# MrOlm/inStrain

Hardware: AMD Instinct MI355X
Metric: Gbp profiled/s (higher is better)
Workload: dtype u32

## Files before the change

include/instrain_amd.h:

```cpp
#ifndef INSTRAIN_AMD_H
#define INSTRAIN_AMD_H

#include <stdint.h>

#ifdef __cplusplus
extern "C" {
#endif

#define ISX_OK 0
#define ISX_ERR_ARG (-1)
#define ISX_ERR_HIP (-2)
#define ISX_ERR_CAPACITY (-3)
#define ISX_ERR_MM_RANGE (-4)
#define ISX_ERR_IO (-5)
#define ISX_ERR_STATE (-6)

#define ISX_ABI_VERSION 5


typedef struct isx_ctx isx_ctx;
typedef struct isx_batch isx_batch;
typedef struct isx_bam isx_bam;
struct isx_bam_params_s;
struct isx_bam_info_s;

typedef struct {
    uint32_t gpos;
    uint16_t mm;
    uint8_t base;
    uint8_t flags;
} isx_obs;

typedef struct {
    int32_t min_cov;
    int32_t min_snp;
    double min_freq;
    int32_t rarefied_coverage;
    int32_t n_mm_bins;
    int32_t enable_linkage;
    int32_t linkage_mode;
    int32_t window;
    uint64_t seed;
    int32_t layout;
    int32_t reserved;
} isx_params;

#define ISX_LAYOUT_WIDE_RECORDS 1
#define ISX_LAYOUT_NO_SHORT_RECORDS 2
#define ISX_LAYOUT_NO_PACKED_COUNTERS 4
#define ISX_LAYOUT_SEG64_RECORDS 8

#define ISX_LAYOUT_MM_ENTRIES 16

#define ISX_LAYOUT_MM_DELTA_RECORDS 32

#define ISX_LAYOUT_NO_STRIPES 64

typedef struct {
    uint32_t gpos;
    uint16_t mm;
    uint16_t flags;
    uint32_t cnt[4];
    float clon;
    float clon_rarefied;
} isx_entry;

typedef struct {
    uint32_t gpos;
    uint16_t mm;
    uint8_t con_base, var_base;
    uint8_t allele_count;
    uint8_t cls;
    uint8_t cryptic;
    uint8_t ref_base;
    uint32_t cnt[4];
} isx_snv;

typedef struct {
    uint32_t gpos_a, gpos_b;
    uint16_t mm;
    uint8_t allele_A, allele_a, allele_B, allele_b;
    uint16_t pad;
    uint32_t total, countAB, countAb, countaB, countab;
    uint32_t pad2;
    double r2, d_prime;
    double r2_normalized, d_prime_normalized;
} isx_ld;

typedef struct {
    int64_t n_entries;
    int64_t n_snv;
    int64_t n_sites;
    int64_t n_allele_obs;
    int64_t n_increments;
    int64_t n_edges;
    int64_t n_ld;
} isx_sizes;

typedef struct {
    float pileup_ms;
    float sites_ms;
    float allele_ms;
    float group_ms;
    float incr_ms;
    float ld_ms;
    float total_ms;
    int32_t pileup_blocks, pileup_threads, pileup_lds_bytes, pileup_window;
    float mfma_ms;
    int32_t dense_tiles;
    int64_t dense_macs;
    int64_t dense_bytes;
    int32_t record_bytes;
    int32_t pad;
} isx_timings;

const char *isx_last_error(void);
int isx_abi_version(void);

int isx_ctx_create(int device_id, isx_ctx **out);
void isx_ctx_destroy(isx_ctx *ctx);
int isx_ctx_reserve_cus(isx_ctx *ctx, int cus_per_xcd);

int isx_set_null_model(isx_ctx *ctx, const int32_t *lut, int64_t n, int32_t fallback);

int isx_batch_create(isx_ctx *ctx, const isx_params *params, int64_t n_pos, const uint8_t *ref,
                     int32_t n_splits, const int64_t *split_bounds, int64_t n_obs,
                     const isx_obs *obs, const uint32_t *pair, isx_batch **out);
void isx_batch_destroy(isx_batch *b);

int isx_batch_run(isx_batch *b);

int isx_batch_launch(isx_batch *b);
int isx_batch_wait(isx_batch *b);
int isx_batch_sizes(const isx_batch *b, isx_sizes *out);
int isx_batch_timings(const isx_batch *b, isx_timings *out);

int isx_batch_fetch_entries(isx_batch *b, isx_entry *out);
int isx_batch_fetch_dense(isx_batch *b, uint32_t *counts , float *clon ,
                          float *clon_rarefied );
// ... 159 lines not shown
    const isx_sat *lev_sat;
    int64_t n_lev, n_lev_clon, n_lev_rare, n_lev_sat;
    int32_t lev_mask_bytes, lev_cov_bytes, lev_window, n_lev_windows, lev_min_cov, pad_lev;
    uint64_t rows_checksum;
} isx_pipe_result;

int isx_levels_expand(const isx_pipe_result *r, int32_t host_threads, uint32_t *gpos, uint32_t *mm_cov, float *clon, float *clon_rarefied);

int isx_pipe_create(isx_ctx *ctx, const isx_params *params, const isx_pipe_params *pp, isx_pipe **out);
void isx_pipe_destroy(isx_pipe *p);
int isx_pipe_submit(isx_pipe *p, int64_t n_pos, const uint8_t *ref, int32_t n_splits, const int64_t *split_bounds,
                    int64_t n_obs, const isx_obs *obs, const uint32_t *pair, int64_t *ticket);
int isx_pipe_submit_bam(isx_pipe *p, isx_bam *bam, const struct isx_bam_params_s *bp, const int32_t *refs, int32_t n_refs,
                        const uint8_t *ref, int32_t n_splits, const int64_t *split_bounds, struct isx_bam_info_s *info,
                        int64_t *ticket);
int isx_pipe_collect(isx_pipe *p, int64_t ticket, isx_pipe_result *out);
int isx_pipe_release(isx_pipe *p, int64_t ticket);
int isx_pipe_fetch_entries(isx_pipe *p, int64_t ticket, isx_entry *out);
int isx_pipe_fetch_entries_shrunk(isx_pipe *p, int64_t ticket, uint32_t *gpos, uint32_t *mm_cov, float *clon, float *clon_rarefied);


#define ISX_SEG_BASES 150
#define ISX_SEG_WORDS 15
#define ISX_SEG_SKIP_WORD 0x24924924u
#define ISX_DREC_WORDS 8
#define ISX_DREC_EXC 6
#define ISX_DREC_EXC_FULL 3
#define ISX_DREC_DUAL 0x80000000u
#define ISX_DREC_NO_EXC 0x3FFFFFFFu

typedef struct {
    int64_t n_seg;
    const uint32_t *gpos;
    const uint8_t *len;
    const uint8_t *mm;
    const uint32_t *pair;
    const uint32_t *bases;
} isx_segs;

int isx_batch_create_reads(isx_ctx *ctx, const isx_params *params, int64_t n_pos, const uint8_t *ref, int32_t n_splits,
                           const int64_t *split_bounds, const isx_segs *segs, isx_batch **out);
int isx_pipe_submit_reads(isx_pipe *p, int64_t n_pos, const uint8_t *ref, int32_t n_splits, const int64_t *split_bounds,
                          const isx_segs *segs, int64_t *ticket);

typedef struct isx_wire isx_wire;
int isx_pipe_stage_reads(isx_pipe *p, int64_t n_pos, const uint8_t *ref, int32_t n_splits, const int64_t *split_bounds,
                         const isx_segs *segs, isx_wire **out);
int isx_pipe_submit_wire(isx_pipe *p, const isx_wire *wire, int64_t *ticket);
int64_t isx_wire_bytes(const isx_wire *wire);
void isx_wire_free(isx_wire *wire);
int isx_wire_keep_reference(isx_pipe *p, isx_wire *wire);

#define ISX_PLANE_WORDS 8
typedef struct {
    int64_t n_seg;
    const uint32_t *gpos;
    const uint8_t *len;
    const uint32_t *pair;
    const uint64_t *planes;
    const uint8_t *mm;
} isx_read_planes;

typedef struct {
    const uint8_t *plane2;
    const uint8_t *nplane;
    uint64_t key;
} isx_ref_planes;

int isx_pack_ref_planes(const uint8_t *ref, int64_t n_pos, int32_t host_threads, uint8_t *plane2, uint8_t *nplane, int32_t *has_n);
int isx_planes_from_segs(const isx_segs *segs, int32_t host_threads, uint64_t *planes);
int isx_pack_read_planes(int64_t n_reads, const int64_t *ref_start, const int64_t *clip_lo, const int64_t *clip_hi,
                         const uint32_t *cigar, const int64_t *cigar_off, const char *seq, const uint8_t *qual, const int64_t *seq_off,
                         const uint32_t *pair, int32_t min_base_quality, int64_t cap_seg, uint32_t *seg_gpos,
                         uint8_t *seg_len, uint32_t *seg_pair, uint64_t *seg_planes, int64_t *n_seg);
int isx_pipe_submit_planes(isx_pipe *p, int64_t n_pos, const isx_ref_planes *ref, int32_t n_splits, const int64_t *split_bounds,
                           const isx_read_planes *reads, int64_t *ticket);
int isx_pipe_stage_planes(isx_pipe *p, int64_t n_pos, const isx_ref_planes *ref, int32_t n_splits, const int64_t *split_bounds,
                          const isx_read_planes *reads, isx_wire **out);
int isx_pipe_set_reference_budget(isx_pipe *p, int64_t mib);
int isx_host_register(const void *ptr, int64_t bytes);
int isx_host_unregister(const void *ptr);
int isx_encode_planes(const isx_read_planes *reads, const isx_ref_planes *ref, int64_t n_pos, int32_t host_threads, int32_t slack_groups,
                      int64_t cap_rec, int64_t ring_records, uint32_t *rec, uint32_t *gbase, int64_t *n_rec, int64_t *need_slack);
int isx_encode_planes_mm(const isx_read_planes *reads, const isx_ref_planes *ref, int64_t n_pos, int32_t n_mm_bins, int32_t host_threads, int32_t slack_groups,
                         int64_t cap_rec, int64_t ring_records, uint32_t *rec, uint32_t *gbase, int64_t *n_rec, int64_t *need_slack);

int isx_count_read_segs(int64_t n_reads, const uint32_t *cigar, const int64_t *cigar_off, const int64_t *ref_start,
                        const int64_t *clip_lo, const int64_t *clip_hi, int64_t *n_seg);
int isx_pack_reads(int64_t n_reads, const int64_t *ref_start, const int64_t *clip_lo, const int64_t *clip_hi,
                   const uint32_t *cigar, const int64_t *cigar_off, const char *seq, const uint8_t *qual, const int64_t *seq_off,
                   const uint8_t *mm, const uint32_t *pair, int32_t min_base_quality, int64_t cap_seg, uint32_t *seg_gpos,
                   uint8_t *seg_len, uint8_t *seg_mm, uint32_t *seg_pair, uint32_t *seg_bases, int64_t *n_seg);

int isx_encode_segs(const isx_segs *segs, int64_t n_pos, int32_t n_mm_bins, int32_t host_threads, int64_t cap_rec, uint32_t *rec,
                    uint32_t *gbase, uint32_t *pair_out, int64_t *n_rec);
int64_t isx_seg_records_needed(const uint32_t *gpos, int64_t n_seg, int32_t host_threads);
int isx_encode_segs_ring(const isx_segs *segs, int64_t n_pos, int32_t n_mm_bins, int32_t host_threads, int64_t cap_rec, int64_t ring_records,
                         uint32_t *rec, uint32_t *gbase, uint32_t *pair_out, int64_t *n_rec);

int isx_encode_delta(const isx_segs *segs, const uint8_t *ref, int64_t n_pos, int32_t n_mm_bins, int32_t host_threads, int32_t slack_groups,
                     int64_t cap_rec, int64_t ring_records, uint32_t *rec, uint32_t *gbase, uint32_t *pair_out, int64_t *n_rec, int64_t *need_slack);
int64_t isx_delta_records_needed(const uint32_t *gpos, int64_t n_seg, int32_t host_threads, int32_t slack_groups);

int isx_encode_obs(const isx_obs *obs, const uint32_t *pair, int64_t n_obs, int64_t n_pos, int32_t record_bytes,
                   int32_t host_threads, double slack, int64_t cap_rec, void *rec, uint32_t *gbase, uint32_t *pair_out,
                   int64_t *n_rec, int32_t *passes);
int isx_encode_obs_ring(const isx_obs *obs, const uint32_t *pair, int64_t n_obs, int64_t n_pos, int32_t record_bytes,
                        int32_t host_threads, double slack, int64_t cap_rec, int64_t ring_records, void *rec,
                        uint32_t *gbase, uint32_t *pair_out, int64_t *n_rec, int32_t *passes);

typedef struct {
    int64_t in_off;
    int32_t in_len;
    int32_t out_len;
    int64_t out_off;
} isx_bgzf_block;
int isx_bgzf_index(const uint8_t *image, int64_t n_bytes, int64_t cap_blocks, isx_bgzf_block *blocks, int64_t *n_blocks, int64_t *out_bytes);
int isx_bgzf_inflate_device(isx_ctx *ctx, const uint8_t *image, int64_t n_bytes, const isx_bgzf_block *blocks, int64_t n_blocks,
                            uint8_t *out, int64_t out_bytes, float *kernel_ms);
int isx_bgzf_inflate_host(const uint8_t *image, int64_t n_bytes, const isx_bgzf_block *blocks, int64_t n_blocks, uint8_t *out, int64_t out_bytes);
int isx_bgzf_inflate_fast(const uint8_t *image, int64_t n_bytes, const isx_bgzf_block *blocks, int64_t n_blocks, uint8_t *out, int64_t out_bytes);

typedef struct isx_bam_params_s {
    double min_read_ani;
    int32_t min_mapq;
    double max_insert_relative;
    int32_t min_insert;
    int32_t min_base_quality;
    int32_t skip_mm;
    int32_t window_length;
    int32_t pairing_filter;
} isx_bam_params;

typedef struct isx_bam_info_s {
    int32_t n_refs;
    int32_t n_splits;
    int64_t n_reads;
    int64_t n_pos;
    int64_t n_obs;
    int64_t n_pairs;
    int64_t unfiltered_pairs, filtered_pairs;
    int64_t filtered_bases;
    double median_insert;
    int32_t max_mm;
    int32_t pad;
    int64_t unfiltered_reads, unfiltered_singletons, filtered_singletons;
    int64_t n_segs;
} isx_bam_info;

int isx_bam_open(const char *path, isx_bam **out);
void isx_bam_close(isx_bam *bam);
void isx_bam_close_wait(isx_bam *bam);
int isx_bam_set_threads(isx_bam *bam, int32_t threads);
int isx_bam_ref(const isx_bam *bam, int32_t i, const char **name, int64_t *length, int64_t *flat_offset);
int isx_bam_set_priority_reads(isx_bam *bam, int64_t n, const char *names, const int64_t *offs);
int isx_bam_scan(isx_bam *bam, isx_bam_info *info );
int isx_bam_scan_part(isx_bam *bam, int32_t part, int32_t n_parts, isx_bam_info *info );
int isx_bam_set_wanted_refs(isx_bam *bam, const int32_t *refs, int32_t n);
int isx_bam_insert_sizes(isx_bam *bam, int64_t *out, int64_t cap, int64_t *n);
int isx_bam_filter(isx_bam *bam, const isx_bam_params *p, double median_insert , isx_bam_info *info);
int isx_bam_pair_keys(isx_bam *bam, uint64_t *h1, uint64_t *h2, int32_t *tid, int64_t *info4, int64_t cap, int64_t *n);
int isx_bam_set_cross_names(isx_bam *bam, int64_t n, const int64_t *entry, const int64_t *occurrences, const int64_t *info4);
int isx_bam_filter_insert_sizes(isx_bam *bam, int64_t *out, int64_t cap, int64_t *n);
int isx_bam_set_r2m(isx_bam *bam, int32_t ref, int64_t n, const char *names, const int64_t *offs, const int32_t *mm );
int isx_bam_set_mm_cap(isx_bam *bam, int32_t cap);
int isx_bam_mm_levels(const isx_bam *bam, int32_t *levels, int32_t cap, int32_t *n);
// ... 20 lines not shown
```

instrain_amd/_lib.py:

```python
import ctypes as C
import os

import numpy as np

_HERE = os.path.dirname(os.path.abspath(__file__))
LIB_PATH = os.path.join(_HERE, "libinstrain_amd.so")
if os.environ.get("ISX_LIB"):
    LIB_PATH = os.path.abspath(os.environ["ISX_LIB"])

BGZF_BLOCK_DT = np.dtype([("in_off", np.int64), ("in_len", np.int32), ("out_len", np.int32), ("out_off", np.int64)])
OBS_DT = np.dtype([("gpos", "<u4"), ("mm", "<u2"), ("base", "u1"), ("flags", "u1")])
ENTRY_DT = np.dtype([("gpos", "<u4"), ("mm", "<u2"), ("flags", "<u2"), ("cnt", "<u4", (4,)), ("clon", "<f4"),
                     ("clon_rarefied", "<f4")])
SNV_DT = np.dtype([("gpos", "<u4"), ("mm", "<u2"), ("con_base", "u1"), ("var_base", "u1"),
                   ("allele_count", "u1"), ("cls", "u1"), ("cryptic", "u1"), ("ref_base", "u1"),
                   ("cnt", "<u4", (4,))])
LD_DT = np.dtype([("gpos_a", "<u4"), ("gpos_b", "<u4"), ("mm", "<u2"), ("allele_A", "u1"), ("allele_a", "u1"),
                  ("allele_B", "u1"), ("allele_b", "u1"), ("pad", "<u2"), ("total", "<u4"), ("countAB", "<u4"),
                  ("countAb", "<u4"), ("countaB", "<u4"), ("countab", "<u4"), ("pad2", "<u4"),
                  ("r2", "<f8"), ("d_prime", "<f8"), ("r2_normalized", "<f8"), ("d_prime_normalized", "<f8")])
AO_DT = np.dtype([("pair", "<u4"), ("gpos", "<u4"), ("order", "<u4"), ("mm", "<u2"), ("base", "u1"), ("pad", "u1")])
assert AO_DT.itemsize == 16
assert OBS_DT.itemsize == 8 and ENTRY_DT.itemsize == 32 and SNV_DT.itemsize == 28 and LD_DT.itemsize == 72


class Params(C.Structure):
    _fields_ = [("min_cov", C.c_int32), ("min_snp", C.c_int32), ("min_freq", C.c_double),
                ("rarefied_coverage", C.c_int32), ("n_mm_bins", C.c_int32), ("enable_linkage", C.c_int32),
                ("linkage_mode", C.c_int32), ("window", C.c_int32), ("seed", C.c_uint64), ("layout", C.c_int32),
                ("reserved", C.c_int32)]


LAYOUT_WIDE_RECORDS, LAYOUT_NO_SHORT_RECORDS, LAYOUT_NO_PACKED_COUNTERS, LAYOUT_SEG64_RECORDS = 1, 2, 4, 8


class PipeParams(C.Structure):
    _fields_ = [("max_pos", C.c_int64), ("max_obs", C.c_int64), ("max_splits", C.c_int32), ("depth", C.c_int32),
                ("host_threads", C.c_int32), ("pin_threads", C.c_int32), ("jump_slack", C.c_double),
                ("want_counts", C.c_int32), ("ring_kib", C.c_int32), ("stage_async", C.c_int32), ("lean_output", C.c_int32),
                ("max_segs", C.c_int64)]


SEG_BASES, SEG_WORDS, SEG_SKIP_WORD = 150, 15, 0x24924924


class Segs(C.Structure):
    _fields_ = [("n_seg", C.c_int64), ("gpos", C.c_void_p), ("len", C.c_void_p), ("mm", C.c_void_p), ("pair", C.c_void_p),
                ("bases", C.c_void_p)]


PLANE_WORDS = 8
LAYOUT_MM_ENTRIES = 16
LAYOUT_MM_DELTA_RECORDS = 32
ABI_VERSION = 5


class ReadPlanes(C.Structure):
    _fields_ = [("n_seg", C.c_int64), ("gpos", C.c_void_p), ("len", C.c_void_p), ("pair", C.c_void_p), ("planes", C.c_void_p), ("mm", C.c_void_p)]


class RefPlanes(C.Structure):
    _fields_ = [("plane2", C.c_void_p), ("nplane", C.c_void_p), ("key", C.c_uint64)]


RARE_DT = np.dtype([("gpos", "<u4"), ("clon_rarefied", "<f4")])
CLON_DT = np.dtype([("gpos", "<u4"), ("clon", "<f4")])
SAT_DT = np.dtype([("gpos", "<u4"), ("coverage", "<u4")])


class Sizes(C.Structure):
    _fields_ = [(n, C.c_int64) for n in ("n_entries", "n_snv", "n_sites", "n_allele_obs", "n_increments",
                                         "n_edges", "n_ld")]


class Timings(C.Structure):
    _fields_ = [(n, C.c_float) for n in ("pileup_ms", "sites_ms", "allele_ms", "group_ms", "incr_ms", "ld_ms",
                                         "total_ms")] + \
               [(n, C.c_int32) for n in ("pileup_blocks", "pileup_threads", "pileup_lds_bytes", "pileup_window")] + \
               [("mfma_ms", C.c_float), ("dense_tiles", C.c_int32), ("dense_macs", C.c_int64), ("dense_bytes", C.c_int64),
                ("record_bytes", C.c_int32), ("pad", C.c_int32)]


class PipeResult(C.Structure):
    _fields_ = [("ticket", C.c_int64), ("n_pos", C.c_int64), ("n_obs", C.c_int64), ("sizes", Sizes),
                ("coverage16", C.c_void_p), ("clon", C.c_void_p), ("rare", C.c_void_p), ("n_rare", C.c_int64),
                ("n_saturated", C.c_int64), ("counts", C.c_void_p), ("clon_rarefied", C.c_void_p), ("snv", C.c_void_p),
                ("batch", C.c_void_p),
                ("encode_ms", C.c_float), ("h2d_ms", C.c_float), ("kernel_ms", C.c_float), ("d2h_ms", C.c_float),
                ("collect_wait_ms", C.c_float), ("record_bytes", C.c_int32), ("encode_passes", C.c_int32),
                ("h2d_bytes", C.c_int64), ("d2h_bytes", C.c_int64), ("ld", C.c_void_p),
                ("coverage8", C.c_void_p), ("clon_sparse", C.c_void_p), ("n_clon", C.c_int64), ("saturated", C.c_void_p),
                ("coverage4", C.c_void_p), ("cov_rows", C.c_void_p), ("cov_row_window", C.c_void_p), ("n_cov_rows", C.c_int64),
                ("cov_window", C.c_int32), ("pad_cov", C.c_int32),
                ("lev_mask", C.c_void_p), ("lev_cov", C.c_void_p), ("lev_win_off", C.c_void_p), ("lev_clon", C.c_void_p), ("lev_rare", C.c_void_p),
                ("lev_sat", C.c_void_p), ("n_lev", C.c_int64), ("n_lev_clon", C.c_int64), ("n_lev_rare", C.c_int64), ("n_lev_sat", C.c_int64),
                ("lev_mask_bytes", C.c_int32), ("lev_cov_bytes", C.c_int32), ("lev_window", C.c_int32), ("n_lev_windows", C.c_int32),
                ("lev_min_cov", C.c_int32), ("pad_lev", C.c_int32), ("rows_checksum", C.c_uint64)]


class BamParams(C.Structure):
    _fields_ = [("min_read_ani", C.c_double), ("min_mapq", C.c_int32), ("max_insert_relative", C.c_double),
                ("min_insert", C.c_int32), ("min_base_quality", C.c_int32), ("skip_mm", C.c_int32),
                ("window_length", C.c_int32), ("pairing_filter", C.c_int32)]


PAIRING_FILTERS = {"paired_only": 0, "non_discordant": 1, "all_reads": 2}


class BamInfo(C.Structure):
    _fields_ = [("n_refs", C.c_int32), ("n_splits", C.c_int32), ("n_reads", C.c_int64), ("n_pos", C.c_int64),
                ("n_obs", C.c_int64), ("n_pairs", C.c_int64), ("unfiltered_pairs", C.c_int64),
                ("filtered_pairs", C.c_int64), ("filtered_bases", C.c_int64), ("median_insert", C.c_double),
                ("max_mm", C.c_int32), ("pad", C.c_int32), ("unfiltered_reads", C.c_int64),
                ("unfiltered_singletons", C.c_int64), ("filtered_singletons", C.c_int64), ("n_segs", C.c_int64)]


SCAFFOLD_LEVEL_DT = np.dtype([("nonzero", "<i8"), ("sum_cov", "<u8"), ("sumsq_cov", "<u8"), ("median_cov", "<f8"),
                              ("counted", "<i8"), ("sum_clon", "<f8"), ("median_clon", "<f8"),
                              ("counted_rarefied", "<i8"), ("sum_clon_rarefied", "<f8"),
                              ("median_clon_rarefied", "<f8"), ("mm", "<i4"), ("present", "<i4")])
assert SCAFFOLD_LEVEL_DT.itemsize == 88
GENOME_LEVEL_DT = np.dtype([("n", "<i8"), ("sum_cov", "<u8"), ("sumsq_cov", "<u8"), ("median_cov", "<f8"), ("mm", "<i4"), ("pad", "<i4")])
assert GENOME_LEVEL_DT.itemsize == 40


COMPARE_LEVEL_DT = np.dtype([("both", "<i8"), ("either", "<i8"), ("mm", "<i4"), ("present_a", "<i4"),
                             ("present_b", "<i4"), ("pad", "<i4"), ("consensus_snps", "<i8"), ("population_snps", "<i8")])
assert COMPARE_LEVEL_DT.itemsize == 48
COMPARE_SNP_DT = np.dtype([("gpos", "<u4"), ("mm", "<u2"), ("consensus_snp", "u1"), ("population_snp", "u1"),
                           ("has_a", "u1"), ("has_b", "u1"), ("con_a", "u1"), ("ref_a", "u1"), ("var_a", "u1"),
                           ("con_b", "u1"), ("ref_b", "u1"), ("var_b", "u1"), ("cnt_a", "<u4", (4,)), ("cnt_b", "<u4", (4,))])
assert COMPARE_SNP_DT.itemsize == 48


GENE_DT = np.dtype([("start", "<i8"), ("end", "<i8"), ("seq_off", "<i8"), ("strand", "<i4"), ("pad", "<i4")])
GENE_COV_DT = np.dtype([("sum_cov", "<u8"), ("nonzero", "<u4"), ("counted", "<u4"), ("sum_clon", "<f8")])
GENE_SNV_COUNT_DT = np.dtype([(n, "<u4") for n in ("divergent", "sns", "sns_n", "sns_s", "snv", "snv_n", "snv_s")])
GENE_MUTATION_DT = np.dtype([("gene", "<i4"), ("k", "<i4"), ("type", "u1"), ("aa_old", "u1"), ("aa_new", "u1"), ("n_genes", "u1"),
                             ("pad", "<u4")])
assert GENE_DT.itemsize == 32 and GENE_COV_DT.itemsize == 24 and GENE_SNV_COUNT_DT.itemsize == 28 and GENE_MUTATION_DT.itemsize == 16
GENE_LEVEL_PRESENT, GENE_COV_ANY, GENE_CLON_ANY = 1, 2, 4


ERR_CAPACITY = -3


class IsxError(RuntimeError):
    def __init__(self, code, msg):
        super().__init__("libinstrain_amd error %d: %s" % (code, msg))
        self.code = code


SYMBOLS = ["isx_last_error", "isx_abi_version", "isx_ctx_create", "isx_ctx_destroy", "isx_ctx_reserve_cus", "isx_set_null_model",
           "isx_batch_create", "isx_batch_create_reads", "isx_batch_destroy", "isx_batch_run", "isx_batch_launch", "isx_batch_wait", "isx_batch_sizes", "isx_batch_timings",
           "isx_batch_fetch_entries", "isx_batch_fetch_dense", "isx_batch_fetch_snv", "isx_batch_fetch_ld", "isx_batch_fetch_allele_obs",
           "isx_batch_summarize", "isx_batch_summarize_genomes", "isx_compare_coverage", "isx_compare_scaffolds", "isx_compare_fetch_snps",
           "isx_genes_create", "isx_genes_destroy", "isx_genes_sites", "isx_batch_profile_genes", "isx_genes_profile_snvs",
           "isx_pipe_create", "isx_pipe_destroy", "isx_pipe_submit", "isx_pipe_submit_reads", "isx_pipe_stage_reads", "isx_pipe_submit_wire", "isx_wire_bytes", "isx_wire_free", "isx_wire_keep_reference", "isx_pipe_submit_bam", "isx_encode_segs", "isx_encode_segs_ring", "isx_seg_records_needed", "isx_encode_delta", "isx_delta_records_needed", "isx_count_read_segs", "isx_pack_reads", "isx_pipe_collect", "isx_pipe_release", "isx_pipe_fetch_entries", "isx_pipe_fetch_entries_shrunk", "isx_levels_expand", "isx_encode_obs", "isx_encode_obs_ring",
           "isx_pack_ref_planes", "isx_planes_from_segs", "isx_pack_read_planes", "isx_pipe_submit_planes", "isx_pipe_stage_planes", "isx_encode_planes", "isx_encode_planes_mm", "isx_pipe_set_reference_budget", "isx_host_register", "isx_host_unregister",
           "isx_bgzf_index", "isx_bgzf_inflate_device", "isx_bgzf_inflate_host", "isx_bgzf_inflate_fast",
           "isx_bam_open", "isx_bam_close", "isx_bam_close_wait", "isx_bam_set_threads", "isx_bam_ref", "isx_bam_set_priority_reads", "isx_bam_scan", "isx_bam_scan_part",
           "isx_bam_insert_sizes", "isx_bam_set_wanted_refs", "isx_bam_pair_keys", "isx_bam_set_cross_names", "isx_bam_filter_insert_sizes", "isx_bam_filter", "isx_bam_set_r2m", "isx_bam_r2m", "isx_bam_drop_names", "isx_bam_batch_pair_names", "isx_bam_set_mm_cap", "isx_bam_mm_levels", "isx_bam_set_mm_levels", "isx_bam_ref_counts",
           "isx_bam_expand_refs", "isx_bam_segment_refs", "isx_bam_copy_segs", "isx_bam_copy_read_planes", "isx_bam_expand_region", "isx_bam_expand", "isx_bam_copy", "isx_bam_view"]

_lib = None


def load():
    global _lib
    if _lib is not None:
        return _lib
    if not os.path.exists(LIB_PATH):
        raise IsxError(-2, "%s not built: run `python -c 'import __graft_entry__ as g; g.build()'` "
                           "(hipcc --offload-arch=gfx950)" % LIB_PATH)
    lib = C.CDLL(LIB_PATH)
    vp, i32, i64 = C.c_void_p, C.c_int32, C.c_int64
    lib.isx_last_error.restype = C.c_char_p
    lib.isx_abi_version.restype = C.c_int
    if lib.isx_abi_version() != ABI_VERSION:
        raise IsxError(-6, "%s has ABI version %d, this package binds version %d: rebuild it (python -c 'import __graft_entry__ as g; g.build()')"
                       % (LIB_PATH, lib.isx_abi_version(), ABI_VERSION))
    lib.isx_ctx_create.argtypes = [C.c_int, C.POINTER(vp)]
    lib.isx_ctx_destroy.argtypes = [vp]
    lib.isx_ctx_reserve_cus.argtypes = [vp, C.c_int]
    lib.isx_bgzf_index.argtypes = [vp, i64, i64, vp, C.POINTER(i64), C.POINTER(i64)]
    lib.isx_bgzf_inflate_device.argtypes = [vp, vp, i64, vp, i64, vp, i64, C.POINTER(C.c_float)]
    lib.isx_bgzf_inflate_host.argtypes = [vp, i64, vp, i64, vp, i64]
    lib.isx_bgzf_inflate_fast.argtypes = [vp, i64, vp, i64, vp, i64]
    lib.isx_ctx_destroy.restype = None
    lib.isx_set_null_model.argtypes = [vp, vp, i64, i32]
    lib.isx_batch_create.argtypes = [vp, C.POINTER(Params), i64, vp, i32, vp, i64, vp, vp, C.POINTER(vp)]
    lib.isx_batch_create_reads.argtypes = [vp, C.POINTER(Params), i64, vp, i32, vp, C.POINTER(Segs), C.POINTER(vp)]
    lib.isx_pipe_submit_reads.argtypes = [vp, i64, vp, i32, vp, C.POINTER(Segs), C.POINTER(i64)]
    lib.isx_pipe_stage_reads.argtypes = [vp, i64, vp, i32, vp, C.POINTER(Segs), C.POINTER(vp)]
    lib.isx_pipe_submit_wire.argtypes = [vp, vp, C.POINTER(i64)]
    lib.isx_wire_bytes.argtypes = [vp]
    lib.isx_wire_bytes.restype = i64
    lib.isx_wire_free.argtypes = [vp]
    lib.isx_wire_keep_reference.argtypes = [vp, vp]
    lib.isx_wire_free.restype = None
    lib.isx_encode_segs.argtypes = [C.POINTER(Segs), i64, i32, i32, i64, vp, vp, vp, C.POINTER(i64)]
    lib.isx_encode_segs_ring.argtypes = [C.POINTER(Segs), i64, i32, i32, i64, i64, vp, vp, vp, C.POINTER(i64)]
    lib.isx_encode_delta.argtypes = [C.POINTER(Segs), vp, i64, i32, i32, i32, i64, i64, vp, vp, vp, C.POINTER(i64), C.POINTER(i64)]
    lib.isx_delta_records_needed.argtypes = [vp, i64, i32, i32]
    lib.isx_delta_records_needed.restype = i64
    lib.isx_seg_records_needed.argtypes = [vp, i64, i32]
    lib.isx_seg_records_needed.restype = i64
    lib.isx_count_read_segs.argtypes = [i64, vp, vp, vp, vp, vp, C.POINTER(i64)]
    lib.isx_pack_reads.argtypes = [i64, vp, vp, vp, vp, vp, vp, vp, vp, vp, vp, i32, i64, vp, vp, vp, vp, vp, C.POINTER(i64)]
    lib.isx_batch_destroy.argtypes = [vp]
    lib.isx_batch_destroy.restype = None
    lib.isx_batch_run.argtypes = [vp]
    lib.isx_batch_launch.argtypes = [vp]
    lib.isx_batch_wait.argtypes = [vp]
    lib.isx_batch_sizes.argtypes = [vp, C.POINTER(Sizes)]
    lib.isx_batch_timings.argtypes = [vp, C.POINTER(Timings)]
    for f in ("isx_batch_fetch_entries", "isx_batch_fetch_snv", "isx_batch_fetch_ld", "isx_batch_fetch_allele_obs"):
        getattr(lib, f).argtypes = [vp, vp]
    lib.isx_batch_fetch_dense.argtypes = [vp, vp, vp, vp]
    lib.isx_batch_summarize.argtypes = [vp, i32, vp, vp, C.POINTER(C.c_float)]
    lib.isx_batch_summarize_genomes.argtypes = [vp, i32, vp, i32, vp, i32, vp, C.POINTER(C.c_float)]
    lib.isx_compare_coverage.argtypes = [vp, vp, i32, vp, i32, vp, C.POINTER(C.c_float)]
    lib.isx_compare_scaffolds.argtypes = [vp, vp, i32, vp, i32, C.c_double, vp, C.POINTER(i64), C.POINTER(C.c_float)]
    lib.isx_compare_fetch_snps.argtypes = [vp, vp]
    lib.isx_genes_create.argtypes = [vp, i64, vp, C.c_char_p, i64, C.POINTER(vp)]
    lib.isx_genes_destroy.argtypes = [vp]
    lib.isx_genes_destroy.restype = None
    lib.isx_genes_sites.argtypes = [vp, vp, C.POINTER(C.c_float)]
    lib.isx_batch_profile_genes.argtypes = [vp, vp, i32, vp, vp, vp, vp, vp, C.POINTER(C.c_float)]
    lib.isx_genes_profile_snvs.argtypes = [vp, i32, vp, vp, vp, i64, vp, i32, vp, vp, C.POINTER(C.c_float)]
    lib.isx_pipe_create.argtypes = [vp, C.POINTER(Params), C.POINTER(PipeParams), C.POINTER(vp)]
    lib.isx_pipe_destroy.argtypes = [vp]
    lib.isx_pipe_destroy.restype = None
    lib.isx_pipe_submit.argtypes = [vp, i64, vp, i32, vp, i64, vp, vp, C.POINTER(i64)]
    lib.isx_pipe_submit_bam.argtypes = [vp, vp, C.POINTER(BamParams), vp, i32, vp, i32, vp, C.POINTER(BamInfo), C.POINTER(i64)]
    lib.isx_pipe_collect.argtypes = [vp, i64, C.POINTER(PipeResult)]
    lib.isx_pipe_release.argtypes = [vp, i64]
    lib.isx_pipe_fetch_entries.argtypes = [vp, i64, vp]
    lib.isx_pipe_fetch_entries_shrunk.argtypes = [vp, i64, vp, vp, vp, vp]
    lib.isx_levels_expand.argtypes = [C.POINTER(PipeResult), i32, vp, vp, vp, vp]
    lib.isx_encode_obs.argtypes = [vp, vp, i64, i64, i32, i32, C.c_double, i64, vp, vp, vp, C.POINTER(i64), C.POINTER(i32)]
    lib.isx_encode_obs_ring.argtypes = [vp, vp, i64, i64, i32, i32, C.c_double, i64, i64, vp, vp, vp, C.POINTER(i64), C.POINTER(i32)]
    lib.isx_bam_open.argtypes = [C.c_char_p, C.POINTER(vp)]
    lib.isx_bam_close.argtypes = [vp]
    lib.isx_bam_close.restype = None
    lib.isx_bam_close_wait.argtypes = [vp]
    lib.isx_bam_close_wait.restype = None
    lib.isx_bam_expand.argtypes = [vp, C.POINTER(BamParams), C.POINTER(BamInfo)]
    lib.isx_bam_set_threads.argtypes = [vp, i32]
    lib.isx_bam_set_priority_reads.argtypes = [vp, i64, C.c_char_p, vp]
    lib.isx_bam_scan.argtypes = [vp, C.POINTER(BamInfo)]
    lib.isx_bam_scan_part.argtypes = [vp, i32, i32, C.POINTER(BamInfo)]
    lib.isx_bam_set_wanted_refs.argtypes = [vp, vp, i32]
    lib.isx_bam_insert_sizes.argtypes = [vp, vp, i64, C.POINTER(i64)]
    lib.isx_bam_filter_insert_sizes.argtypes = [vp, vp, i64, C.POINTER(i64)]
    lib.isx_bam_pair_keys.argtypes = [vp, vp, vp, vp, vp, i64, C.POINTER(i64)]
    lib.isx_bam_set_cross_names.argtypes = [vp, i64, vp, vp, vp]
    lib.isx_bam_filter.argtypes = [vp, C.POINTER(BamParams), C.c_double, C.POINTER(BamInfo)]
    lib.isx_bam_set_r2m.argtypes = [vp, i32, i64, C.c_char_p, vp, vp]
    lib.isx_bam_drop_names.argtypes = [vp]
    lib.isx_bam_r2m.argtypes = [vp, i32, C.POINTER(i64), C.POINTER(i64), vp, vp, vp]
    lib.isx_bam_batch_pair_names.argtypes = [vp, C.POINTER(i64), C.POINTER(i64), vp, vp]
    lib.isx_bam_set_mm_cap.argtypes = [vp, i32]
    lib.isx_bam_mm_levels.argtypes = [vp, vp, i32, vp]
    lib.isx_bam_set_mm_levels.argtypes = [vp, vp, i32]
    lib.isx_bam_ref_counts.argtypes = [vp, vp, vp]
    lib.isx_bam_expand_region.argtypes = [vp, C.POINTER(BamParams), i32, i64, i64, C.POINTER(BamInfo)]
    lib.isx_bam_expand_refs.argtypes = [vp, C.POINTER(BamParams), vp, i32, C.POINTER(BamInfo)]
    lib.isx_bam_segment_refs.argtypes = [vp, C.POINTER(BamParams), vp, i32, C.POINTER(BamInfo), C.POINTER(i64)]
    lib.isx_bam_copy_segs.argtypes = [vp, vp, vp, vp, vp, vp, vp, vp]
    lib.isx_bam_copy_read_planes.argtypes = [vp, vp]
    lib.isx_pack_ref_planes.argtypes = [vp, i64, i32, vp, vp, C.POINTER(i32)]
    lib.isx_planes_from_segs.argtypes = [C.POINTER(Segs), i32, vp]
    lib.isx_pack_read_planes.argtypes = [i64, vp, vp, vp, vp, vp, vp, vp, vp, vp, i32, i64, vp, vp, vp, vp, C.POINTER(i64)]
    lib.isx_pipe_submit_planes.argtypes = [vp, i64, C.POINTER(RefPlanes), i32, vp, C.POINTER(ReadPlanes), C.POINTER(i64)]
    lib.isx_pipe_set_reference_budget.argtypes = [vp, i64]
    lib.isx_host_register.argtypes = [vp, i64]
    lib.isx_host_unregister.argtypes = [vp]
    lib.isx_pipe_stage_planes.argtypes = [vp, i64, C.POINTER(RefPlanes), i32, vp, C.POINTER(ReadPlanes), C.POINTER(vp)]
    lib.isx_encode_planes.argtypes = [C.POINTER(ReadPlanes), C.POINTER(RefPlanes), i64, i32, i32, i64, i64, vp, vp, C.POINTER(i64), C.POINTER(i64)]
    lib.isx_encode_planes_mm.argtypes = [C.POINTER(ReadPlanes), C.POINTER(RefPlanes), i64, i32, i32, i32, i64, i64, vp, vp, C.POINTER(i64), C.POINTER(i64)]
    lib.isx_bam_ref.argtypes = [vp, i32, C.POINTER(C.c_char_p), C.POINTER(i64), C.POINTER(i64)]
    lib.isx_bam_copy.argtypes = [vp, vp, vp, vp, vp]
    lib.isx_bam_view.argtypes = [vp, C.POINTER(vp), C.POINTER(vp)]
    _lib = lib
    return lib


def check(rc):
    if rc != 0:
        raise IsxError(rc, load().isx_last_error().decode(errors="replace"))
```

instrain_amd/csrc/isx_pipe.hip:

```cpp
#include <atomic>
#include <algorithm>
#include <chrono>
#include <cmath>
#include <condition_variable>
#include <cstring>
#include <deque>
#include <mutex>
#include <memory>
#include <string>
#include <thread>
#include <vector>

#include "bam_front.h"
#include "isx_batch.h"
#include "obs_encode.h"
#include "seg_encode.h"
#include "isx_summary.h"
#include <unordered_map>

namespace {

constexpr size_t ALIGN = 256;
inline size_t up(size_t v, size_t a = ALIGN) { return (v + a - 1) / a * a; }

double now_ms()
{
    return std::chrono::duration<double, std::milli>(std::chrono::steady_clock::now().time_since_epoch()).count();
}

int host_block_alloc(void **p, size_t bytes, bool pinned)
{
    *p = nullptr;
    if (pinned) { HIP_TRY(isx_pin_malloc(p, std::max<size_t>(bytes, 1))); return ISX_OK; }
    if (posix_memalign(p, 4096, std::max<size_t>(bytes, 4096)) != 0) { *p = nullptr; isx_set_error("out of host memory"); return ISX_ERR_ARG; }
    return ISX_OK;
}

void host_block_free(void *p, bool pinned)
{
    if (!p) return;
    if (pinned) isx_pin_free(p); else free(p);
}

static const bool pipe_timing = getenv("ISX_PIPE_TIMING") != nullptr;
#define H2D(p, s) ((s).h2d ? (s).h2d : (p)->s_h2d)
struct Slot {
    isx_batch *b = nullptr;
    hipStream_t h2d = nullptr;
    uint8_t *h_in = nullptr, *d_in = nullptr;
    size_t in_bytes = 0;
    size_t off_bounds = 0, off_win = 0, off_ref = 0, off_gbase = 0, off_ridx = 0, off_rec = 0;
    size_t off_pairs = 0;
    isxenc::PairRun *h_runs = nullptr;
    bool runs_pinned = true;
    uint2 *d_runs = nullptr;
    size_t cap_runs = 0;
    hipEvent_t ev_ring[2] = {nullptr, nullptr};
    bool ring_busy[2] = {false, false};
    uint8_t *h_out = nullptr;
    uint8_t *h_small = nullptr;
    size_t small_bytes = 0;
    bool out_pinned = true;
    size_t out_bytes = 0, o_counts = 0, o_clon = 0, o_clonr = 0, o_snv = 0, o_cov16 = 0, o_rare = 0;
    bool rare_dense = false;
    bool cov8 = false, clon_sparse = false;
    bool cov4 = false;
    size_t cov_rows_off = 0;
    int cov_window = 0;
    std::vector<uint32_t> cov_row_win;
    std::vector<isx_sat> sat_rows;
    bool sat_complete = true;
    void *sort_temp = nullptr;
    size_t sort_temp_bytes = 0;
    std::vector<float> clonr_big;
    std::vector<isx_rare> rare_big;
    std::vector<uint32_t> cmin, cmax, dir_pmax, dir_smin;
    std::vector<uint8_t> cany;
    std::vector<uint2> win;
    size_t o_lmask = 0, o_lwin = 0, o_lcov = 0, o_lclon = 0, o_lrare = 0;
    size_t lcov_room = 0, lclon_room = 0, lrare_room = 0;
    std::vector<uint8_t> lcov_big;
    std::vector<isx_rare> lclon_big, lrare_big;
    std::vector<isx_snv> snv_big;
    std::vector<isx_ld> ld_rows;
    uint64_t rows_checksum = 0;
    hipEvent_t ev_h2d0 = nullptr, ev_h2d1 = nullptr, ev_pass = nullptr, ev_d2h0 = nullptr, ev_d2h1 = nullptr;
    hipEvent_t ev_h2da = nullptr, ev_h2db = nullptr;
    bool h2d_split = false;
    int64_t ticket = -1;
    BamBatch *dead_batch = nullptr;
    bool ref_has_n = false;
    int state = 0;
    int rc = 0;
    std::string err;
    float finish_wait_ms = 0.f;
    float encode_ms = 0.f;
    int encode_passes = 0;
    int64_t h2d_bytes = 0, d2h_bytes = 0;
    uint16_t *d_gpos16 = nullptr;
};

static uint64_t bytes_checksum(const void *p, size_t bytes, uint64_t seed)
{
    const uint8_t *b = static_cast<const uint8_t *>(p);
    uint64_t a[4] = {seed ^ 0x9E3779B97F4A7C15ull, seed + 0xC2B2AE3D27D4EB4Full, seed ^ 0x165667B19E3779F9ull, seed + 0x27D4EB2F165667C5ull};
    const size_t n8 = bytes / 8;
    size_t i = 0;
    for (; i + 4 <= n8; i += 4) {
        uint64_t w[4];
        memcpy(w, b + 8 * i, 32);
        for (int k = 0; k < 4; k++) a[k] = a[k] * 0x100000001B3ull + w[k];
    }
    uint64_t h = (uint64_t)bytes;
    for (; i < n8; i++) { uint64_t w; memcpy(&w, b + 8 * i, 8); h = h * 0x100000001B3ull + w; }
    for (size_t j = n8 * 8; j < bytes; j++) h = h * 0x100000001B3ull + b[j];
    for (int k = 0; k < 4; k++) { h ^= a[k]; h *= 0xFF51AFD7ED558CCDull; h ^= h >> 33; }
    return h;
}

static inline size_t ref2_bytes(int64_t n_pos) { return (((size_t)n_pos + 3) / 4 + 15) & ~(size_t)15; }
static inline size_t refn_bytes(int64_t n_pos) { return (((size_t)n_pos + 7) / 8 + 15) & ~(size_t)15; }

static bool copy_ref_planes(isxenc::HostPool &pool, const isx_ref_planes *rp, int64_t n_pos, uint8_t *plane2, uint8_t *nplane)
{
    const size_t b2 = ((size_t)n_pos + 3) / 4, bn = ((size_t)n_pos + 7) / 8;
    const size_t piece = (size_t)1 << 20;
    const int t2 = (int)((b2 + piece - 1) / piece), tn = rp->nplane ? (int)((bn + piece - 1) / piece) : 0;
    std::atomic<int> any{0};
    pool.run(t2 + tn, [&](int t) {
        if (t < t2) { const size_t a = (size_t)t * piece; memcpy(plane2 + a, rp->plane2 + a, std::min(piece, b2 - a)); return; }
        const size_t a = (size_t)(t - t2) * piece, n = std::min(piece, bn - a);
        const uint8_t *src = rp->nplane + a;
        uint8_t acc = 0;
        for (size_t i = 0; i < n; i++) acc |= src[i];
        memcpy(nplane + a, src, n);
        if (acc) any.store(1, std::memory_order_relaxed);
    });
    return any.load() != 0;
}

static bool plane_any(isxenc::HostPool &pool, const uint8_t *pl, size_t bytes)
{
    const size_t piece = (size_t)1 << 20;
    const int nt = (int)((bytes + piece - 1) / piece);
    std::atomic<int> any{0};
    pool.run(nt, [&](int t) {
        const size_t a = (size_t)t * piece, n = std::min(piece, bytes - a);
        uint64_t acc = 0;
        size_t i = 0;
        for (; i + 8 <= n; i += 8) { uint64_t v; memcpy(&v, pl + a + i, 8); acc |= v; }
        for (; i < n; i++) acc |= pl[a + i];
        if (acc) any.store(1, std::memory_order_relaxed);
    });
    return any.load() != 0;
}

static uint64_t ref_plane_checksum(const uint8_t *plane2, int64_t n_pos)
{
    const size_t words = (((size_t)n_pos + 3) / 4) / 8;
    uint64_t h = 0x9E3779B97F4A7C15ull ^ (uint64_t)n_pos;
    if (!words) { for (size_t i = 0; i < ((size_t)n_pos + 3) / 4; i++) h = (h ^ plane2[i]) * 0x100000001B3ull; return h; }
    const size_t n_s = std::min<size_t>(words, 4096), step = words / n_s;
    for (size_t k = 0; k < n_s; k++) {
        uint64_t w;
        memcpy(&w, plane2 + 8 * (k * step), 8);
        h = (h ^ w) * 0x100000001B3ull;
        h ^= h >> 29;
    }
    return h;
}

int cgroup_cpus()
{
    if (FILE *f = fopen("/sys/fs/cgroup/cpu.max", "r")) {
        char q[64] = {0};
        long period = 0;
        const int n = fscanf(f, "%63s %ld", q, &period);
        fclose(f);
        if (n == 2 && period > 0 && strcmp(q, "max") != 0) return (int)std::max<long>(1, atol(q) / period);
    }
    return 0;
}

int gpu_numa_node(int device)
{
    char bus[64] = {0};
    if (hipDeviceGetPCIBusId(bus, sizeof bus, device) != hipSuccess) return -1;
    std::string id(bus);
    std::transform(id.begin(), id.end(), id.begin(), [](unsigned char ch) { return (char)std::tolower(ch); });
    int node = -1;
    if (FILE *f = fopen(("/sys/bus/pci/devices/" + id + "/numa_node").c_str(), "r")) {
        if (fscanf(f, "%d", &node) != 1) node = -1;
        fclose(f);
    }
    return node;
}

}

struct isx_pipe {
    isx_ctx *ctx = nullptr;
    isx_params prm{};
    isx_pipe_params pp{};
    std::unique_ptr<isxenc::HostPool> pool;
    std::vector<Slot> slots;
    hipStream_t s_h2d = nullptr, s_d2h = nullptr;
    hipStream_t s_h2d2 = nullptr;
    hipStream_t s_fin = nullptr;
    hipStream_t s_fin2 = nullptr;
    int64_t next_ticket = 0;
    int64_t cap_rec = 0;
    int64_t ring_half = 0;
    int rb = 2;
    bool segs = false;
    bool drec = false;
    int64_t dslack = 1;
    uint32_t G = ISX_GROUP16;
    size_t snv_prefix = 0;
    size_t rare_prefix = 0, cap_rare = 0;
    double slack = 0.0;
    std::thread finisher;
    std::thread finisher2;
    std::vector<std::thread> more_finishers;
    std::vector<hipStream_t> extra_fin;
    std::mutex bounce_mu;
    std::mutex mu;
    std::condition_variable cv_work, cv_done;
    std::deque<int64_t> work;
    bool stop = false;
    std::mutex launch_mu;
    uint8_t *bounce[2] = {nullptr, nullptr};
    hipEvent_t bounce_ev[2] = {nullptr, nullptr};
    size_t bounce_bytes = 0;
    std::unique_ptr<isxenc::HostPool> fin_pool;
    struct StageJob {
        int64_t ticket, n_pos;
        const uint8_t *ref;
        std::vector<int64_t> bounds;
        isx_segs segs;
        bool planes = false;
        isx_read_planes reads{};
        isx_ref_planes rp{};
    };
    struct RefEntry { uint8_t *d = nullptr; size_t bytes = 0; int64_t n_pos = 0; bool has_n = false; hipEvent_t ready = nullptr; uint64_t sum = 0; };
    std::unordered_map<uint64_t, RefEntry> ref_cache;
    size_t ref_cache_bytes = 0;
    std::atomic<size_t> ref_cache_budget{(size_t)4096 << 20};
    std::thread stager;
    std::deque<StageJob> stage_q;
    std::condition_variable cv_stage;
    int64_t next_promise = 0;
    bool stage_stop = false;
};

static int bounce_d2h(isx_pipe *p, void *hdst, const void *dsrc, size_t bytes, hipStream_t st)
{
    if (!bytes) return ISX_OK;
    std::lock_guard<std::mutex> bounce_lk(p->bounce_mu);
    const size_t piece = p->bounce_bytes;
    const size_t n_pieces = (bytes + piece - 1) / piece;
    auto issue = [&](size_t k) -> hipError_t {
        const size_t off = k * piece, len = std::min(piece, bytes - off);
        hipError_t e = isx_copy_to_host(p->bounce[k & 1], static_cast<const uint8_t *>(dsrc) + off, len, st);
        return e == hipSuccess ? hipEventRecord(p->bounce_ev[k & 1], st) : e;
    };
    HIP_TRY(issue(0));
    for (size_t k = 0; k < n_pieces; k++) {
        if (k + 1 < n_pieces) HIP_TRY(issue(k + 1));
        HIP_TRY(isx_wait_event(p->bounce_ev[k & 1]));
        const size_t off = k * piece, len = std::min(piece, bytes - off);
        const size_t sub = (size_t)1 << 20;
        const uint8_t *src = p->bounce[k & 1];
        uint8_t *dst = static_cast<uint8_t *>(hdst) + off;
        p->fin_pool->run((int)((len + sub - 1) / sub), [&](int t) {
            const size_t a = (size_t)t * sub;
            memcpy(dst + a, src + a, std::min(sub, len - a));
        });
    }
    return ISX_OK;
}

static void pipe_free(isx_pipe *p)
{
    if (!p) return;
    if (p->stager.joinable()) {
        { std::lock_guard<std::mutex> lk(p->mu); p->stage_stop = true; }
        p->cv_stage.notify_all();
        p->stager.join();
    }
    if (p->finisher.joinable()) {
        { std::lock_guard<std::mutex> lk(p->mu); p->stop = true; }
        p->cv_work.notify_all();
        p->finisher.join();
        if (p->finisher2.joinable()) p->finisher2.join();
        for (auto &t : p->more_finishers) if (t.joinable()) t.join();
    }
    (void)hipSetDevice(p->ctx->device);
    if (p->s_h2d) (void)isx_wait_stream(p->s_h2d);
    if (p->s_h2d2) (void)isx_wait_stream(p->s_h2d2);
    if (p->s_d2h) (void)isx_wait_stream(p->s_d2h);
    if (p->s_fin) (void)isx_wait_stream(p->s_fin);
    if (p->s_fin2) (void)isx_wait_stream(p->s_fin2);
    for (hipStream_t st : p->extra_fin) (void)isx_wait_stream(st);
    for (int i = 0; i < 2; i++) if (p->ctx->pstream[i]) (void)isx_wait_stream(p->ctx->pstream[i]);
    const double t_f0 = now_ms();
    double t_batch = 0, t_dev = 0, t_pin = 0;
    for (Slot &s : p->slots) {
        double t_x = now_ms();
        if (s.b) {
            isx_batch *b = s.b;
            b->d_seg = nullptr; b->d_drec = nullptr;
            b->d_rec = nullptr; b->d_rec32 = nullptr; b->d_rec16 = nullptr; b->d_gbase = nullptr; b->d_pair = nullptr;
            b->d_pair_runs = nullptr; b->d_run_index = nullptr;
            b->d_gpos = nullptr; b->d_gpos16 = nullptr; b->d_cbase = nullptr; b->d_ref = nullptr; b->d_win = nullptr;
            b->d_bounds = nullptr;
            isx_batch_destroy(b);
        }
        t_batch += now_ms() - t_x; t_x = now_ms();
        if (s.sort_temp) isx_dev_free(s.sort_temp);
        if (s.d_gpos16) isx_dev_free(s.d_gpos16);
        if (s.d_in) isx_dev_free(s.d_in);
        if (s.d_runs) isx_dev_free(s.d_runs);
        t_dev += now_ms() - t_x; t_x = now_ms();
        if (s.h_in) isx_pin_free(s.h_in);
        host_block_free(s.h_runs, s.runs_pinned);
        for (hipEvent_t e : s.ev_ring) if (e) (void)hipEventDestroy(e);
        host_block_free(s.h_out, s.out_pinned);
        if (s.h_small) isx_pin_free(s.h_small);
        t_pin += now_ms() - t_x;
        for (hipEvent_t e : {s.ev_h2d0, s.ev_h2d1, s.ev_pass, s.ev_d2h0, s.ev_d2h1, s.ev_h2da, s.ev_h2db}) if (e) (void)hipEventDestroy(e);
    }
    if (pipe_timing)
        fprintf(stderr, "[isx_pipe_destroy] device tables %.1f ms, device arena %.1f ms, pinned staging %.1f ms, total %.1f ms\n", t_batch, t_dev, t_pin, now_ms() - t_f0);
    for (auto &kv : p->ref_cache) { if (kv.second.d) isx_dev_free(kv.second.d); if (kv.second.ready) (void)hipEventDestroy(kv.second.ready); }
    for (int i = 0; i < 2; i++) {
        if (p->bounce[i]) isx_pin_free(p->bounce[i]);
        if (p->bounce_ev[i]) (void)hipEventDestroy(p->bounce_ev[i]);
    }
    if (p->s_h2d) (void)hipStreamDestroy(p->s_h2d);
    if (p->s_h2d2) (void)hipStreamDestroy(p->s_h2d2);
    if (p->s_d2h) (void)hipStreamDestroy(p->s_d2h);
    if (p->s_fin) (void)hipStreamDestroy(p->s_fin);
    if (p->s_fin2) (void)hipStreamDestroy(p->s_fin2);
    for (hipStream_t st : p->extra_fin) (void)hipStreamDestroy(st);
    delete p;
}

static int slot_batch_create(isx_pipe *p, Slot &s, int index)
{
    isx_ctx *c = p->ctx;
    const isx_params *prm = &p->prm;
    const double t_s0 = now_ms();
    isx_batch *b = new isx_batch();
    s.b = b;
    b->ctx = c; b->prm = *prm; b->M = prm->n_mm_bins;
    b->ps = getenv("ISX_ONE_PASS_QUEUE") ? 0 : (index & 1);
    b->cap_pos = p->pp.max_pos; b->cap_obs = p->pp.max_obs; b->arena = true; b->ref_packed = 2;
    b->n_pos = p->pp.max_pos; b->n_obs = p->pp.max_obs;
    b->segs = p->segs; b->drec = p->drec;
    b->lean = p->pp.lean_output != 0 && !p->pp.want_counts;
    b->lev_sparse = b->M > 1 && b->M <= 32 && p->segs && !p->pp.want_counts && !(prm->layout & ISX_LAYOUT_MM_ENTRIES);
    b->spin_us = (p->pp.host_threads > 0 && p->pp.host_threads < 8) ? 200 : 2000;
    const bool dense = b->M == 1;
    batch_pick_block(b);
    const int64_t cap_pos = p->pp.max_pos;
    for (auto &e : b->ev) HIP_TRY(hipEventCreate(&e));
    for (auto &e : b->ev_sum) HIP_TRY(hipEventCreate(&e));
    HIP_TRY(isx_dev_malloc(reinterpret_cast<void **>(&b->d_cursors), (CUR_N + 4) * sizeof(uint32_t)));
    b->d_flags = b->d_cursors + CUR_N;
    HIP_TRY(hipHostMalloc(&b->h_state, (CUR_N + 8) * sizeof(uint32_t), hipHostMallocMapped | hipHostMallocCoherent));
    memset(b->h_state, 0, (CUR_N + 8) * sizeof(uint32_t));
    HIP_TRY(hipHostGetDevicePointer(reinterpret_cast<void **>(&b->d_host_state), b->h_state, 0));
    HIP_TRY(hipMemset(b->d_cursors, 0, (CUR_N + 4) * sizeof(uint32_t)));
    {
        std::vector<uint16_t> thr = build_thresholds(c->h_lut, c->fallback, prm->min_freq);
        HIP_TRY(isx_dev_malloc(reinterpret_cast<void **>(&b->d_thr), thr.size() * sizeof(uint16_t)));
        HIP_TRY(hipMemcpy(b->d_thr, thr.data(), thr.size() * sizeof(uint16_t), hipMemcpyHostToDevice));
    }
    const uint64_t npm = (uint64_t)cap_pos * b->M;
    const uint64_t cap_obs = (uint64_t)std::max<int64_t>(p->pp.max_obs, 1);
    if (dense) {
        if (p->pp.want_counts) HIP_TRY(isx_dev_malloc(reinterpret_cast<void **>(&b->d_counts), (size_t)cap_pos * sizeof(uint4)));
        else {
            b->cap_clon = (size_t)cap_pos / 2 + 65536;
            HIP_TRY(isx_dev_malloc(reinterpret_cast<void **>(&b->d_cov8), (size_t)cap_pos));
            if (p->pp.lean_output) {
                b->cap_cov_row_win = (size_t)cap_pos / 64 + 2;
                HIP_TRY(isx_dev_malloc(reinterpret_cast<void **>(&b->d_cov_row_win), b->cap_cov_row_win * sizeof(uint32_t)));
            }
            HIP_TRY(isx_dev_malloc(reinterpret_cast<void **>(&b->d_clon_list), b->cap_clon * sizeof(uint2)));
            HIP_TRY(isx_dev_malloc(reinterpret_cast<void **>(&b->d_clon_sorted), b->cap_clon * sizeof(uint2)));
        }
        b->cap_sat = (size_t)cap_pos / 16 + 65536;
        HIP_TRY(isx_dev_malloc(reinterpret_cast<void **>(&b->d_sat), b->cap_sat * sizeof(uint2)));
        HIP_TRY(isx_dev_malloc(reinterpret_cast<void **>(&b->d_clon), (size_t)cap_pos * sizeof(float)));
        HIP_TRY(isx_dev_malloc(reinterpret_cast<void **>(&b->d_clon_r), (size_t)cap_pos * sizeof(float)));
        HIP_TRY(isx_dev_malloc(reinterpret_cast<void **>(&b->d_cov16), (size_t)cap_pos * sizeof(uint16_t)));
        if (prm->rarefied_coverage > 0) {
            b->cap_rare = p->cap_rare;
            HIP_TRY(isx_dev_malloc(reinterpret_cast<void **>(&b->d_rare), b->cap_rare * sizeof(uint2)));
        }
    } else if (b->lev_sparse) {
        b->lev_mask_bytes = b->M <= 8 ? 1 : (b->M <= 16 ? 2 : 4);
        b->cap_lev = (size_t)std::min<uint64_t>(std::min<uint64_t>(npm, 0xFFFFFFF0ull), std::max<uint64_t>((uint64_t)cap_pos * (uint64_t)std::min(b->M, 4), 1u << 20));
        HIP_TRY(isx_dev_malloc(&b->d_lev_mask, (size_t)cap_pos * b->lev_mask_bytes + 64));
// ... 390 lines not shown
            p->ring_half = (int64_t)(ring / 2 / (size_t)p->rb) / (int64_t)p->G * (int64_t)p->G;
            if (p->ring_half * p->rb < (4096 + 16 * ISX_SEG_GROUP) * 64) { delete p; isx_set_error("isx_pipe_create: ring_kib too small for a read-level pipe (at least 1024)"); return ISX_ERR_ARG; }
        }
    } else {
        const uint64_t want = (uint64_t)((double)pp->max_obs * (1.0 + js)) + 4 * ISX_PAD;
        p->cap_rec = (int64_t)((want + ISX_PAD - 1) / ISX_PAD * ISX_PAD);
        if ((uint64_t)p->cap_rec >= 0xFFFFFFFFull) { delete p; isx_set_error("more than 2^32 records in one batch"); return ISX_ERR_ARG; }
    }
    if (!p->segs) {
        const size_t rec_bytes = (size_t)p->cap_rec * p->rb;
        size_t ring = 0;
        if (pp->ring_kib > 0) ring = (size_t)pp->ring_kib << 10;
        else if (pp->ring_kib == 0 && pp->depth == 1 && rec_bytes > ((size_t)128 << 20)) ring = (size_t)64 << 20;
        else if (pp->ring_kib == 0 && rec_bytes > ((size_t)512 << 20)) ring = (size_t)256 << 20;
        if (ring && ring < rec_bytes) {
            p->ring_half = (int64_t)(ring / 2 / p->rb) / ISX_PAD * ISX_PAD;
            if (p->ring_half < 2 * ISX_PAD) { delete p; isx_set_error("isx_pipe_create: ring_kib too small (at least 32)"); return ISX_ERR_ARG; }
        }
    }
    p->snv_prefix = (size_t)std::min<int64_t>(std::max<int64_t>(pp->max_pos / 64, 1 << 16), 1 << 22);
    p->cap_rare = (size_t)std::max<int64_t>(pp->max_pos, 1 << 16);
    p->rare_prefix = (size_t)std::max<int64_t>(pp->max_pos / 16, 1 << 16);
    int nt = pp->host_threads;
    if (nt <= 0) {
        const int q = cgroup_cpus();
        nt = q > 0 ? q : (int)std::thread::hardware_concurrency();
        nt = std::max(1, std::min(nt, 32));
    }
    c->n_pipes++;
    const double t_c0 = now_ms();
    p->pool.reset(new isxenc::HostPool(nt, gpu_numa_node(c->device), pp->pin_threads != 0));
    const double t_c1 = now_ms();
    int rc = ISX_OK;
    hipError_t e;
    if ((e = isx_side_stream_create(c, &p->s_h2d)) != hipSuccess ||
        (e = isx_side_stream_create(c, &p->s_fin)) != hipSuccess ||
        (e = isx_side_stream_create(c, &p->s_fin2)) != hipSuccess ||
        (e = isx_side_stream_create(c, &p->s_d2h)) != hipSuccess) {
        isx_set_error(std::string("isx_pipe_create: ") + hipGetErrorString(e));
        pipe_free(p);
        return ISX_ERR_HIP;
    }
    p->slots.resize((size_t)pp->depth);
    {
        const char *e2 = getenv("ISX_PIPE_H2D_STREAMS");
        if (e2 && atoi(e2) >= 2 && pp->depth >= 2 && isx_side_stream_create(c, &p->s_h2d2) != hipSuccess) { p->s_h2d2 = nullptr; (void)hipGetLastError(); }
    }
    for (int i = 0; i < pp->depth && rc == ISX_OK; i++) {
        rc = slot_batch_create(p, p->slots[(size_t)i], i);
        if ((i & 1) && p->s_h2d2) p->slots[(size_t)i].h2d = p->s_h2d2;
    }
    if (rc != ISX_OK) { pipe_free(p); return rc; }
    if (!p->slots[0].out_pinned) {
        p->bounce_bytes = (size_t)16 << 20;
        for (int i = 0; i < 2 && rc == ISX_OK; i++) {
            if (isx_pin_malloc(reinterpret_cast<void **>(&p->bounce[i]), p->bounce_bytes) != hipSuccess ||
                hipEventCreateWithFlags(&p->bounce_ev[i], hipEventDisableTiming) != hipSuccess) rc = ISX_ERR_HIP;
        }
        if (rc != ISX_OK) { isx_set_error("isx_pipe_create: bounce buffers"); pipe_free(p); return rc; }
        p->fin_pool.reset(new isxenc::HostPool(std::max(1, std::min(nt, 6)), -1, false));
    }
    p->finisher = std::thread(finisher_main, p, p->s_fin);
    if (pp->depth >= 2) p->finisher2 = std::thread(finisher_main, p, p->s_fin2);
    {
        int want = pp->depth >= 4 ? 4 : 2;
        if (const char *e = getenv("ISX_PIPE_FINISHERS")) want = std::max(1, atoi(e));
        want = std::min(want, pp->depth);
        for (int i = 2; i < want; i++) {
            hipStream_t st = nullptr;
            if (isx_side_stream_create(c, &st) != hipSuccess) break;
            p->extra_fin.push_back(st);
            p->more_finishers.emplace_back(finisher_main, p, st);
        }
    }
    if (pipe_timing)
        fprintf(stderr, "[isx_pipe_create] thread pool %.1f ms, %d slot(s) %.1f ms\n", t_c1 - t_c0, pp->depth, now_ms() - t_c1);
    if (pp->stage_async && p->segs) p->stager = std::thread(stager_main, p);
    *out = p;
    return ISX_OK;
}

void isx_pipe_destroy(isx_pipe *p) { pipe_free(p); }

static int enqueue_pass_impl(isx_pipe *p, Slot &s, int64_t n_pos, int64_t *ticket);

static int enqueue_pass(isx_pipe *p, Slot &s, int64_t n_pos, int64_t *ticket)
{
    const int rc = enqueue_pass_impl(p, s, n_pos, ticket);
    if (rc != ISX_OK) {
        const std::string why(isx_last_error());
        (void)isx_wait_stream(H2D(p, s));
        (void)isx_wait_stream(p->ctx->pstream[s.b->ps]);
        (void)isx_wait_stream(p->s_d2h);
        isx_set_error(why);
    }
    return rc;
}

static int enqueue_pass_impl(isx_pipe *p, Slot &s, int64_t n_pos, int64_t *ticket)
{
    isx_ctx *c = p->ctx;
    isx_batch *b = s.b;
    const bool dense = b->M == 1, linkage = p->prm.enable_linkage != 0;
    hipStream_t ps = c->pstream[b->ps];
    int rc = ISX_OK;
    std::unique_lock<std::mutex> launch_lk(p->launch_mu);
    HIP_TRY(hipStreamWaitEvent(ps, s.ev_h2d1, 0));
    if (dense && p->prm.rarefied_coverage > 0 && b->rare_dense)
        HIP_TRY(hipMemsetD32Async(reinterpret_cast<hipDeviceptr_t>(b->d_clon_r), 0x7FC00000, (size_t)n_pos, ps));
    if (linkage && p->rb == 4)
        launch_extract_gpos(nullptr, b->d_rec32, b->d_gbase, nullptr, b->d_gpos16, b->d_gbase, ISX_GROUP, b->n_rec, ps);
    if ((rc = launch_pass(b)) != ISX_OK) return rc;
    {
        PileupArgs pa{};
        pa.cursors = b->d_cursors; pa.host_state = b->d_host_state;
        launch_publish_state(pa, b->epoch, ps);
        b->publish_enqueued = true;
        if (c->unpublished[b->ps] == b) c->unpublished[b->ps] = nullptr;
    }
    HIP_TRY(hipEventRecord(s.ev_pass, ps));

    HIP_TRY(hipStreamWaitEvent(p->s_d2h, s.ev_pass, 0));
    HIP_TRY(hipEventRecord(s.ev_d2h0, p->s_d2h));
    const size_t snv_rows = std::min(p->snv_prefix, b->cap_snv);
    HIP_TRY(isx_copy_rows_to_host(s.h_small + s.o_snv, b->d_snv, b->d_cursors + CUR_SNV, b->base[CUR_SNV], (uint32_t)sizeof(isx_snv), snv_rows, p->s_d2h));
    s.d2h_bytes = 0;
    if (dense) {
        if (p->prm.rarefied_coverage > 0) {
            const size_t n = std::min(p->rare_prefix, std::min(p->cap_rare, (size_t)n_pos));
            HIP_TRY(isx_copy_rows_to_host(s.h_small + s.o_rare, b->d_rare, b->d_cursors + CUR_RARE, b->base[CUR_RARE], (uint32_t)sizeof(isx_rare), n, p->s_d2h));
        }
        if (!b->sparse_out) s.d2h_bytes += (int64_t)n_pos * 6;
    }
    if (dense && s.out_pinned && !b->sparse_out) {
        HIP_TRY(isx_copy_to_host(s.h_out + s.o_cov16, b->d_cov16, (size_t)n_pos * 2, p->s_d2h));
        HIP_TRY(isx_copy_to_host(s.h_out + s.o_clon, b->d_clon, (size_t)n_pos * 4, p->s_d2h));
        if (p->pp.want_counts) {
            HIP_TRY(isx_copy_to_host(s.h_out + s.o_counts, b->d_counts, (size_t)n_pos * 16, p->s_d2h));
            s.d2h_bytes += (int64_t)n_pos * 16;
            if (p->prm.rarefied_coverage > 0) {
                HIP_TRY(isx_copy_to_host(s.h_out + s.o_clonr, b->d_clon_r, (size_t)n_pos * 4, p->s_d2h));
                s.d2h_bytes += (int64_t)n_pos * 4;
            }
        }
    }
    HIP_TRY(hipEventRecord(s.ev_d2h1, p->s_d2h));
    launch_lk.unlock();
    {
        std::lock_guard<std::mutex> lk(p->mu);
        s.ticket = p->next_ticket++;
        if (p->next_promise < p->next_ticket) p->next_promise = p->next_ticket;
        s.state = 1; s.rc = ISX_OK;
        *ticket = s.ticket;
        p->work.push_back(s.ticket);
    }
    p->cv_work.notify_one();
    return ISX_OK;
}


static int check_capacity(const isx_pipe *p, const char *who, int64_t n_pos, int64_t n_items, int64_t max_items, int32_t n_splits)
{
    if (n_pos > p->pp.max_pos || n_items > max_items || n_splits > p->pp.max_splits) {
        isx_set_error(std::string(who) + ": batch larger than the pipe was created for");
        return ISX_ERR_CAPACITY;
    }
    return ISX_OK;
}

static int slot_acquire(isx_pipe *p, const char *who, Slot **out)
{
    Slot &s = p->slots[(size_t)(p->next_ticket % (int64_t)p->slots.size())];
    {
        std::lock_guard<std::mutex> lk(p->mu);
        if (s.state != 0) { isx_set_error(std::string(who) + ": every slot is in use (collect + release the oldest batch first)"); return ISX_ERR_STATE; }
    }
    HIP_TRY(hipSetDevice(p->ctx->device));
    *out = &s;
    return ISX_OK;
}

static int queue_for_stager(isx_pipe *p, isx_pipe::StageJob &&job, const char *who, int64_t *ticket)
{
    const int rc = check_capacity(p, who, job.n_pos, job.planes ? job.reads.n_seg : job.segs.n_seg, p->pp.max_segs, (int32_t)job.bounds.size() - 1);
    if (rc != ISX_OK) return rc;
    {
        std::lock_guard<std::mutex> lk(p->mu);
        const int64_t t = p->next_promise, n = (int64_t)p->slots.size();
        const Slot &s = p->slots[(size_t)(t % n)];
        if (t - n >= p->next_ticket || s.state != 0) { isx_set_error(std::string(who) + ": every slot is in use (collect + release the oldest batch first)"); return ISX_ERR_STATE; }
        job.ticket = t;
        p->next_promise = t + 1;
        *ticket = t;
        p->stage_q.push_back(std::move(job));
    }
    p->cv_stage.notify_one();
    return ISX_OK;
}

struct RingFeed { hipError_t err = hipSuccess; size_t bytes = 0; };

static int ring_feed_install(isx_pipe *p, Slot &s, RingFeed &r, int64_t &ring_groups, std::function<void(int)> &wave_begin,
                             std::function<void(int, int64_t, int64_t)> &wave_flush)
{
    if (p->ring_half <= 0) return ISX_OK;
    HIP_TRY(hipEventRecord(s.ev_h2d0, H2D(p, s)));
    const size_t half_bytes = (size_t)p->ring_half * (size_t)p->rb, grp_bytes = (size_t)p->G * (size_t)p->rb;
    uint8_t *d_rec = s.d_in + s.off_rec;
    ring_groups = p->ring_half / (int64_t)p->G;
    wave_begin = [&s, &r](int h) {
        if (s.ring_busy[h]) { const hipError_t e = isx_wait_event(s.ev_ring[h]); if (e != hipSuccess && r.err == hipSuccess) r.err = e; s.ring_busy[h] = false; }
    };
    wave_flush = [p, &s, &r, half_bytes, grp_bytes, d_rec](int h, int64_t g0, int64_t g1) {
        const size_t n = (size_t)(g1 - g0) * grp_bytes;
        if (g0 == 0) r.bytes = 0;
        hipError_t e = hipMemcpyAsync(d_rec + (size_t)g0 * grp_bytes, s.h_in + s.off_rec + (size_t)h * half_bytes, n, hipMemcpyHostToDevice, H2D(p, s));
        if (e == hipSuccess) e = hipEventRecord(s.ev_ring[h], H2D(p, s));
        if (e != hipSuccess && r.err == hipSuccess) r.err = e;
        s.ring_busy[h] = true;
        r.bytes += n;
    };
    return ISX_OK;
}

static int slot_choose_windows(isx_pipe *p, Slot &s, uint32_t chunk, bool threads)
{
    isx_batch *b = s.b;
    DirThreads mt{*p->pool, s.dir_pmax, s.dir_smin};
    const ChunkDir dir{s.cmin.data(), s.cmax.data(), s.cany.data(), b->n_rec / chunk, chunk};
    b->W = choose_windows(b, b->n_pos, dir, threads ? &mt : nullptr, s.win, &b->packed);
    b->n_win = (int)s.win.size();
    if (s.win.size() > (size_t)p->pp.max_pos / 64 + 2) { isx_set_error("internal: window directory larger than the arena"); return ISX_ERR_STATE; }
    memcpy(s.h_in + s.off_win, s.win.data(), s.win.size() * sizeof(uint2));
    return ISX_OK;
}

constexpr double COV8_BELOW_DEPTH = 16.0;
constexpr double NIB_BELOW_DEPTH = 6.0;
constexpr double LEV_COV8_BELOW_DEPTH = 64.0;
constexpr double RARE_DENSE_OBS_FACTOR = 4.0;

static int slot_shape_pass(isx_pipe *p, Slot &s)
{
    isx_batch *b = s.b;
    const bool dense = b->M == 1;
    const double n_obs = (double)b->n_obs, n_pos = (double)b->n_pos;
    b->sparse_out = dense && b->d_clon_list != nullptr;
    b->cov8_out = b->sparse_out && n_obs < COV8_BELOW_DEPTH * n_pos;
    b->nib_out = b->cov8_out && b->lean && n_obs < NIB_BELOW_DEPTH * n_pos;
    b->clon_dense = false;
    b->rare_dense = !(b->lean && b->sparse_out) || n_obs * RARE_DENSE_OBS_FACTOR >= (double)p->prm.rarefied_coverage * n_pos;
    if (b->lev_sparse) b->lev_cov_bytes = n_obs < LEV_COV8_BELOW_DEPTH * n_pos ? 1 : 2;
    const int rc = batch_set_geometry(b);
    if (rc != ISX_OK) return rc;
    if (!dense && !b->lev_sparse) {
        const size_t used = (size_t)b->n_win * b->slab;
        if (used > b->slab_region) { isx_set_error("internal: entry slabs larger than the slot's region"); return ISX_ERR_STATE; }
        b->cap_ovf = b->cap_entries - used;
    }
    return ISX_OK;
}

static void slot_bind_inputs(isx_pipe *p, Slot &s, uint8_t *resident_ref)
{
    isx_batch *b = s.b;
    const bool linkage = p->prm.enable_linkage != 0;
    uint8_t *rec = s.d_in + s.off_rec;
    b->d_bounds = reinterpret_cast<int64_t *>(s.d_in + s.off_bounds);
    b->d_win = reinterpret_cast<uint2 *>(s.d_in + s.off_win);
    b->d_ref = resident_ref ? resident_ref : s.d_in + s.off_ref;
    b->d_ref_n = s.ref_has_n ? b->d_ref + ref2_bytes(b->n_pos) : nullptr;
    b->d_gbase = reinterpret_cast<uint32_t *>(s.d_in + s.off_gbase);
    b->d_rec16 = p->rb == 2 ? reinterpret_cast<uint16_t *>(rec) : nullptr;
    b->d_rec32 = p->rb == 4 ? reinterpret_cast<uint32_t *>(rec) : nullptr;
    if (p->segs) {
        b->d_seg = p->drec ? nullptr : reinterpret_cast<uint4 *>(rec);
        b->d_drec = p->drec ? reinterpret_cast<uint4 *>(rec) : nullptr;
        b->d_pair = linkage && !p->drec ? reinterpret_cast<uint32_t *>(s.d_in + s.off_pairs) : nullptr;
        b->d_pair_runs = nullptr; b->d_run_index = nullptr; b->n_runs = 0;
    } else {
        b->d_pair = nullptr;
        b->d_pair_runs = linkage ? s.d_runs : nullptr;
        b->d_run_index = linkage ? reinterpret_cast<uint32_t *>(s.d_in + s.off_ridx) : nullptr;
        b->d_gpos16 = s.d_gpos16; b->gpos16_shift = 5;
    }
}

static void ref_cache_insert(isx_pipe *p, Slot &s, const isx_ref_planes *rp, int64_t n_pos)
{
    const size_t rb_all = ref2_bytes(n_pos) + (s.ref_has_n ? refn_bytes(n_pos) : 0);
    if (p->ref_cache_bytes + rb_all > p->ref_cache_budget.load(std::memory_order_relaxed)) return;
    isx_pipe::RefEntry e;
    bool ok = isx_dev_malloc(reinterpret_cast<void **>(&e.d), rb_all + 64) == hipSuccess && hipEventCreateWithFlags(&e.ready, hipEventDisableTiming) == hipSuccess;
    ok = ok && hipMemcpyAsync(e.d, s.d_in + s.off_ref, rb_all, hipMemcpyDeviceToDevice, H2D(p, s)) == hipSuccess && hipEventRecord(e.ready, H2D(p, s)) == hipSuccess;
    if (ok) {
        e.bytes = rb_all; e.n_pos = n_pos; e.has_n = s.ref_has_n; e.sum = ref_plane_checksum(rp->plane2, n_pos);
        p->ref_cache_bytes += rb_all;
        p->ref_cache.emplace(rp->key, e);
    } else {
        if (e.d) isx_dev_free(e.d);
        if (e.ready) (void)hipEventDestroy(e.ready);
        (void)hipGetLastError();
    }
}

struct RefStage {
    bool early = false;
    uint8_t *resident = nullptr;
    double host_ms = 0.0;
};

static int stage_reference(isx_pipe *p, Slot &s, int64_t n_pos, const uint8_t *ref, const isx_ref_planes *rp, isxenc::SegJob &J, RefStage *out)
{
    const bool ring = p->ring_half > 0;
    const double t_r = now_ms();
    const size_t b2 = ((size_t)n_pos + 3) / 4, bn = ((size_t)n_pos + 7) / 8;
    hipStream_t st = H2D(p, s);

    const auto hit = rp && rp->key ? p->ref_cache.find(rp->key) : p->ref_cache.end();
    if (hit != p->ref_cache.end()) {
        const isx_pipe::RefEntry &e = hit->second;
        if (e.n_pos != n_pos || e.has_n != (rp->nplane != nullptr && e.has_n) || e.sum != ref_plane_checksum(rp->plane2, n_pos)) {
            isx_set_error("isx_pipe_submit_planes: the reference key stands for other planes (positions / non-ACGT plane / content differ)");
            return ISX_ERR_ARG;
        }
        s.ref_has_n = e.has_n;
        J.ref2 = rp->plane2; J.refn = e.has_n ? rp->nplane : nullptr;
        out->resident = e.d;
        HIP_TRY(hipStreamWaitEvent(st, e.ready, 0));
        if (!ring) HIP_TRY(hipEventRecord(s.ev_h2d0, st));
        HIP_TRY(hipEventRecord(s.ev_h2da, st));
        out->early = true;
        out->host_ms = now_ms() - t_r;
        return ISX_OK;
    }

    const bool first_trip = rp && rp->key && p->ref_cache_budget.load(std::memory_order_relaxed) > 0;
    if (rp && !first_trip && isx_host_is_registered(rp->plane2, b2) && (!rp->nplane || isx_host_is_registered(rp->nplane, bn))) {
        const bool any_n = rp->nplane && plane_any(*p->pool, rp->nplane, bn);
        s.ref_has_n = any_n;
        J.ref2 = rp->plane2; J.refn = any_n ? rp->nplane : nullptr;
        out->host_ms = now_ms() - t_r;
        if (!ring) HIP_TRY(hipEventRecord(s.ev_h2d0, st));
        HIP_TRY(hipMemcpyAsync(s.d_in + s.off_ref, rp->plane2, b2, hipMemcpyHostToDevice, st));
        if (any_n) HIP_TRY(hipMemcpyAsync(s.d_in + s.off_ref + ref2_bytes(n_pos), rp->nplane, bn, hipMemcpyHostToDevice, st));
        if (!ring) HIP_TRY(hipEventRecord(s.ev_h2da, st));
        out->early = true;
        return ISX_OK;
    }

    uint8_t *h2 = s.h_in + s.off_ref, *hn = h2 + ref2_bytes(n_pos);
    s.ref_has_n = rp ? copy_ref_planes(*p->pool, rp, n_pos, h2, hn) : isxenc::pack_ref_planes(*p->pool, ref, n_pos, h2, hn);
    J.ref2 = h2; J.refn = s.ref_has_n ? hn : nullptr;
    out->host_ms = now_ms() - t_r;
    static const bool late_dma = getenv("ISX_PIPE_LATE_DMA") != nullptr;
    if (late_dma) return ISX_OK;
    if (!ring) HIP_TRY(hipEventRecord(s.ev_h2d0, st));
    HIP_TRY(hipMemcpyAsync(s.d_in + s.off_ref, h2, ref2_bytes(n_pos) + (s.ref_has_n ? refn_bytes(n_pos) : 0), hipMemcpyHostToDevice, st));
    if (!ring) HIP_TRY(hipEventRecord(s.ev_h2da, st));
    out->early = true;
    if (rp && rp->key) ref_cache_insert(p, s, rp, n_pos);
    return ISX_OK;
}

static int submit_common(isx_pipe *p, int64_t n_pos, const uint8_t *ref, int32_t n_splits, const int64_t *split_bounds,
                         int64_t n_obs, isxenc::EncodeJob &J, int64_t *ticket)
{
    static const char who[] = "isx_pipe_submit";
    int rc;
    if ((rc = check_capacity(p, who, n_pos, n_obs, p->pp.max_obs, n_splits)) != ISX_OK) return rc;
    if ((rc = check_split_bounds(n_pos, n_splits, split_bounds)) != ISX_OK) return rc;
    Slot *slot = nullptr;
    if ((rc = slot_acquire(p, who, &slot)) != ISX_OK) return rc;
    Slot &s = *slot;
    isx_batch *b = s.b;
    const bool linkage = p->prm.enable_linkage != 0;

    const double t0 = now_ms();
    const bool ring = p->ring_half > 0;
    uint8_t *d_rec = s.d_in + s.off_rec;
    RingFeed feed;
    J.n_obs = n_obs; J.n_pos = n_pos; J.record_bytes = p->rb;
    J.rec = s.h_in + s.off_rec; J.gbase = reinterpret_cast<uint32_t *>(s.h_in + s.off_gbase);
    J.pair_out = nullptr;
    J.cmin = s.cmin.data(); J.cmax = s.cmax.data(); J.cany = s.cany.data();
    J.cap_rec = p->cap_rec;
    if ((rc = ring_feed_install(p, s, feed, J.ring_groups, J.wave_begin, J.wave_flush)) != ISX_OK) return rc;
    int erc = 0;
    for (int attempt = 0;; attempt++) {
        if (linkage) {
            J.runs_out = s.h_runs; J.cap_runs = s.cap_runs;
            J.run_index_out = reinterpret_cast<uint32_t *>(s.h_in + s.off_ridx);
        }
        J.slack = p->slack;
        feed.bytes = 0;
        erc = isxenc::encode_obs(*p->pool, J);
        if (erc != isxenc::ENC_OK || !linkage || J.n_runs <= s.cap_runs || attempt == 1) break;
        HIP_TRY(isx_wait_stream(H2D(p, s)));
        host_block_free(s.h_runs, s.runs_pinned); s.h_runs = nullptr;
        isx_dev_free(s.d_runs); s.d_runs = nullptr;
        s.cap_runs = J.n_runs + J.n_runs / 4 + 4096;
        { const int hrc = host_block_alloc(reinterpret_cast<void **>(&s.h_runs), s.cap_runs * sizeof(isxenc::PairRun), s.runs_pinned); if (hrc != ISX_OK) return hrc; }
        HIP_TRY(isx_dev_malloc(reinterpret_cast<void **>(&s.d_runs), s.cap_runs * sizeof(uint2)));
    }
    const double t_enc = now_ms();
    if (feed.err != hipSuccess) { isx_set_error(std::string("isx_pipe_submit: staging ring: ") + hipGetErrorString(feed.err)); return ISX_ERR_HIP; }
    if (erc == isxenc::ENC_CAPACITY) { isx_set_error("isx_pipe_submit: the stream jumps too often for the pipe's record capacity (raise jump_slack)"); return ISX_ERR_CAPACITY; }
    if (erc == isxenc::ENC_MM_RANGE) { isx_set_error("an observation has mm >= 256"); return ISX_ERR_MM_RANGE; }
    if (erc == isxenc::ENC_BAD_POS) { isx_set_error("observation gpos >= n_pos"); return ISX_ERR_ARG; }
    if (linkage) {
        if (J.n_runs > s.cap_runs) { isx_set_error("isx_pipe_submit: internal: pair-id run table did not fit after growing it"); return ISX_ERR_STATE; }
        b->n_runs = (uint32_t)J.n_runs;
    }
    if (J.passes > 1 && J.n_groups_in > 0)
        p->slack = std::max(p->slack, 1.25 * ((double)J.n_groups_real / (double)J.n_groups_in - 1.0) + 0.01);
    s.ref_has_n = isxenc::pack_ref_planes(*p->pool, ref, n_pos, s.h_in + s.off_ref, s.h_in + s.off_ref + ref2_bytes(n_pos));
    memcpy(s.h_in + s.off_bounds, split_bounds, (size_t)(n_splits + 1) * sizeof(int64_t));

    b->n_pos = n_pos; b->n_obs = n_obs; b->n_splits = n_splits; b->n_rec = (uint64_t)J.n_rec;
    b->n_pairs = (uint64_t)J.max_pair + 1;
    if ((rc = slot_choose_windows(p, s, ISX_CHUNK, false)) != ISX_OK) return rc;
    if ((rc = slot_shape_pass(p, s)) != ISX_OK) return rc;
    slot_bind_inputs(p, s, nullptr);
    s.encode_ms = (float)(now_ms() - t0);
    s.encode_passes = J.passes;
    if (pipe_timing)
        fprintf(stderr, "[isx_pipe_submit] records %.2f ms (%d pass), reference + bounds + windows %.2f ms; %lld obs, %lld runs\n",
                t_enc - t0, J.passes, now_ms() - t_enc, (long long)n_obs, (long long)J.n_runs);

    if (!ring) HIP_TRY(hipEventRecord(s.ev_h2d0, H2D(p, s)));
    const size_t ref_bytes = ref2_bytes(n_pos) + (s.ref_has_n ? refn_bytes(n_pos) : 0);
    const size_t head = (size_t)(n_splits + 1) * sizeof(int64_t) + s.win.size() * sizeof(uint2) + ref_bytes;
    memset(s.h_in + s.off_gbase + (size_t)(b->n_rec / p->G) * sizeof(uint32_t), 0, ISX_TAIL_GROUPS * sizeof(uint32_t));
    const size_t gb_bytes = ((size_t)(b->n_rec / p->G) + ISX_TAIL_GROUPS) * sizeof(uint32_t), rec_bytes = (size_t)b->n_rec * p->rb + ISX_TAIL_BYTES;
    HIP_TRY(hipMemcpyAsync(s.d_in + s.off_bounds, s.h_in + s.off_bounds, (size_t)(n_splits + 1) * sizeof(int64_t), hipMemcpyHostToDevice, H2D(p, s)));
    HIP_TRY(hipMemcpyAsync(s.d_in + s.off_win, s.h_in + s.off_win, s.win.size() * sizeof(uint2), hipMemcpyHostToDevice, H2D(p, s)));
    HIP_TRY(hipMemcpyAsync(s.d_in + s.off_ref, s.h_in + s.off_ref, ref_bytes, hipMemcpyHostToDevice, H2D(p, s)));
    HIP_TRY(hipMemcpyAsync(s.d_in + s.off_gbase, s.h_in + s.off_gbase, gb_bytes, hipMemcpyHostToDevice, H2D(p, s)));
    if (ring) {
        if (p->rb == 2) HIP_TRY(hipMemsetD8Async(reinterpret_cast<hipDeviceptr_t>(d_rec + (size_t)b->n_rec * 2), 0xFF, ISX_TAIL_BYTES, H2D(p, s)));
        else HIP_TRY(hipMemsetD32Async(reinterpret_cast<hipDeviceptr_t>(d_rec + (size_t)b->n_rec * 4), (int)ISX_PAD32, ISX_TAIL_BYTES / 4, H2D(p, s)));
        if (feed.bytes != (size_t)b->n_rec * p->rb) { isx_set_error("internal: the staging ring did not carry the whole stream"); return ISX_ERR_STATE; }
    } else {
        if (p->rb == 2) memset(s.h_in + s.off_rec + (size_t)b->n_rec * 2, 0xFF, ISX_TAIL_BYTES);
        else std::fill_n(reinterpret_cast<uint32_t *>(s.h_in + s.off_rec + (size_t)b->n_rec * 4), ISX_TAIL_BYTES / 4, (uint32_t)ISX_PAD32);
        HIP_TRY(hipMemcpyAsync(d_rec, s.h_in + s.off_rec, rec_bytes, hipMemcpyHostToDevice, H2D(p, s)));
    }
    s.h2d_bytes = (int64_t)(head + gb_bytes + rec_bytes);
    if (linkage) {
        const size_t rb = (size_t)b->n_runs * sizeof(isxenc::PairRun), ib = (size_t)(b->n_rec / ISX_CHUNK) * sizeof(uint32_t);
        HIP_TRY(hipMemcpyAsync(s.d_runs, s.h_runs, rb, hipMemcpyHostToDevice, H2D(p, s)));
        HIP_TRY(hipMemcpyAsync(s.d_in + s.off_ridx, s.h_in + s.off_ridx, ib, hipMemcpyHostToDevice, H2D(p, s)));
        s.h2d_bytes += (int64_t)(rb + ib);
    }
    HIP_TRY(hipEventRecord(s.ev_h2d1, H2D(p, s)));
    s.h2d_split = false;

    return enqueue_pass(p, s, n_pos, ticket);
}

static int encode_reads(isx_pipe *p, Slot &s, isxenc::SegJob &J, bool planes_in, RingFeed &feed)
{
    s.encode_passes = 1;
    if (!p->drec) return isxenc::encode_segs(*p->pool, J);
    std::vector<int64_t> exact;
    for (int attempt = 0;; attempt++) {
        J.slack_groups = p->dslack;
        J.task_groups = exact.empty() ? nullptr : exact.data();
        feed.bytes = 0;
        const int erc = planes_in ? isxenc::encode_planes(*p->pool, J) : isxenc::encode_delta(*p->pool, J);
        if (erc != isxenc::SEG_CAPACITY || J.need_slack <= p->dslack || attempt != 0) return erc;
        exact = J.task_need;
        int64_t tot = 0;
        for (int64_t v : exact) tot += v;
        const int64_t n_t = (int64_t)exact.size(), base_tot = J.n_rec / ISX_DREC_GROUP - n_t * p->dslack;
        p->dslack = std::max<int64_t>(p->dslack, 1 + (tot - base_tot + n_t - 1) / std::max<int64_t>(n_t, 1));
        s.encode_passes = 2;
    }
}

static int submit_segs_common(isx_pipe *p, int64_t n_pos, const uint8_t *ref, int32_t n_splits, const int64_t *split_bounds,
                              isxenc::SegJob &J, int64_t *ticket, const isx_ref_planes *rp)
{
    static const char who[] = "isx_pipe_submit_reads";
    const bool planes_in = J.in2.planes != nullptr || (bool)J.produce_planes || (J.n_seg == 0 && rp != nullptr);
    int rc;
    if ((rc = check_capacity(p, who, n_pos, J.n_seg, p->pp.max_segs, n_splits)) != ISX_OK) return rc;
    if ((rc = check_split_bounds(n_pos, n_splits, split_bounds)) != ISX_OK) return rc;
    Slot *slot = nullptr;
    if ((rc = slot_acquire(p, who, &slot)) != ISX_OK) return rc;
    Slot &s = *slot;
    isx_batch *b = s.b;
    const bool linkage = p->prm.enable_linkage != 0;

    const double t0 = now_ms();
    J.n_pos = n_pos; J.n_mm_bins = b->M;
    J.rec = reinterpret_cast<uint32_t *>(s.h_in + s.off_rec);
    J.gbase = reinterpret_cast<uint32_t *>(s.h_in + s.off_gbase);
    J.pair_out = linkage && !p->drec ? reinterpret_cast<uint32_t *>(s.h_in + s.off_pairs) : nullptr;
    J.cmin = s.cmin.data(); J.cmax = s.cmax.data(); J.cany = s.cany.data();
    J.cap_rec = p->cap_rec;
    const bool ring = p->ring_half > 0;
    RingFeed feed;
    if ((rc = ring_feed_install(p, s, feed, J.ring_groups, J.wave_begin, J.wave_flush)) != ISX_OK) return rc;
    RefStage rs;
    if (planes_in) {
        if (!p->drec) { isx_set_error("bit-plane reads need a pipe whose batches travel as reference-delta records (one mm bin, or ISX_LAYOUT_MM_DELTA_RECORDS)"); return ISX_ERR_STATE; }
        if ((rc = stage_reference(p, s, n_pos, ref, rp, J, &rs)) != ISX_OK) return rc;
    }
    if (p->drec) J.ref = ref;
    const int erc = encode_reads(p, s, J, planes_in, feed);
    const double t_enc = now_ms();
    if (feed.err != hipSuccess) { isx_set_error(std::string("isx_pipe_submit_reads: staging ring: ") + hipGetErrorString(feed.err)); return ISX_ERR_HIP; }
    if ((rc = seg_status_error(erc, "isx_pipe_submit_reads: the stream jumps too often for the pipe's record capacity (raise jump_slack)", ISX_ERR_CAPACITY)) != ISX_OK) return rc;
    if (J.n_bases > p->pp.max_obs) { isx_set_error("isx_pipe_submit_reads: more bases than the pipe's max_obs"); return ISX_ERR_CAPACITY; }
    bool early_rec = false;
    if (rs.early && !ring) {
        const size_t gb_bytes0 = (size_t)(J.n_rec / (int64_t)p->G) * sizeof(uint32_t), rec_bytes0 = (size_t)J.n_rec * (size_t)p->rb;
        HIP_TRY(hipEventRecord(s.ev_h2db, H2D(p, s)));
        if (s.off_pairs == s.off_rec && s.off_ridx == s.off_rec && s.off_rec - s.off_gbase < ((size_t)2 << 20)) {
            HIP_TRY(hipMemcpyAsync(s.d_in + s.off_gbase, s.h_in + s.off_gbase, (s.off_rec - s.off_gbase) + rec_bytes0, hipMemcpyHostToDevice, H2D(p, s)));
        } else {
            HIP_TRY(hipMemcpyAsync(s.d_in + s.off_gbase, s.h_in + s.off_gbase, gb_bytes0, hipMemcpyHostToDevice, H2D(p, s)));
            HIP_TRY(hipMemcpyAsync(s.d_in + s.off_rec, s.h_in + s.off_rec, rec_bytes0, hipMemcpyHostToDevice, H2D(p, s)));
        }
        early_rec = true;
    }
    if (!planes_in) s.ref_has_n = isxenc::pack_ref_planes(*p->pool, ref, n_pos, s.h_in + s.off_ref, s.h_in + s.off_ref + ref2_bytes(n_pos));
    const double t_ref = now_ms();
    memcpy(s.h_in + s.off_bounds, split_bounds, (size_t)(n_splits + 1) * sizeof(int64_t));

    b->n_pos = n_pos; b->n_obs = J.n_bases; b->n_splits = n_splits; b->n_rec = (uint64_t)J.n_rec;
    b->n_pairs = (uint64_t)J.max_pair + 1;
    if ((rc = slot_choose_windows(p, s, p->G, true)) != ISX_OK) return rc;
    if ((rc = slot_shape_pass(p, s)) != ISX_OK) return rc;
    slot_bind_inputs(p, s, rs.resident);
    s.encode_ms = (float)(now_ms() - t0);
    if (pipe_timing)
        fprintf(stderr, "[isx_pipe_submit_reads] records %.2f ms, reference %.2f ms, bounds + windows %.2f ms; %lld segments, %lld records%s\n",
                t_enc - t0 - rs.host_ms, t_ref - t_enc + rs.host_ms, now_ms() - t_ref, (long long)J.n_seg, (long long)J.n_rec, planes_in ? " (bit planes)" : "");
    const double t_q0 = now_ms();

    if (!ring && !rs.early) HIP_TRY(hipEventRecord(s.ev_h2d0, H2D(p, s)));
    const size_t ref_bytes = ref2_bytes(n_pos) + (s.ref_has_n ? refn_bytes(n_pos) : 0);
    const size_t head = (size_t)(n_splits + 1) * sizeof(int64_t) + s.win.size() * sizeof(uint2) + ref_bytes;
    const size_t gb_bytes = (size_t)(b->n_rec / p->G) * sizeof(uint32_t), rec_bytes = (size_t)b->n_rec * (size_t)p->rb;
    if (s.off_win - s.off_bounds < ((size_t)1 << 20)) {
        HIP_TRY(hipMemcpyAsync(s.d_in + s.off_bounds, s.h_in + s.off_bounds, (s.off_win - s.off_bounds) + s.win.size() * sizeof(uint2), hipMemcpyHostToDevice, H2D(p, s)));
    } else {
        HIP_TRY(hipMemcpyAsync(s.d_in + s.off_bounds, s.h_in + s.off_bounds, (size_t)(n_splits + 1) * sizeof(int64_t), hipMemcpyHostToDevice, H2D(p, s)));
        HIP_TRY(hipMemcpyAsync(s.d_in + s.off_win, s.h_in + s.off_win, s.win.size() * sizeof(uint2), hipMemcpyHostToDevice, H2D(p, s)));
    }
    if (!rs.early) HIP_TRY(hipMemcpyAsync(s.d_in + s.off_ref, s.h_in + s.off_ref, ref_bytes, hipMemcpyHostToDevice, H2D(p, s)));
    if (!early_rec) HIP_TRY(hipMemcpyAsync(s.d_in + s.off_gbase, s.h_in + s.off_gbase, gb_bytes, hipMemcpyHostToDevice, H2D(p, s)));
    if (ring) { if (feed.bytes != rec_bytes) { isx_set_error("internal: the staging ring did not carry the whole stream"); return ISX_ERR_STATE; } }
    else if (!early_rec) HIP_TRY(hipMemcpyAsync(s.d_in + s.off_rec, s.h_in + s.off_rec, rec_bytes, hipMemcpyHostToDevice, H2D(p, s)));
    s.h2d_bytes = (int64_t)(head + gb_bytes + rec_bytes) - (rs.resident ? (int64_t)ref_bytes : 0);
    if (linkage && !p->drec) {
        HIP_TRY(hipMemcpyAsync(s.d_in + s.off_pairs, s.h_in + s.off_pairs, (size_t)b->n_rec * sizeof(uint32_t), hipMemcpyHostToDevice, H2D(p, s)));
        s.h2d_bytes += (int64_t)b->n_rec * 4;
    }
    HIP_TRY(hipEventRecord(s.ev_h2d1, H2D(p, s)));
    s.h2d_split = early_rec;
    const double t_q1 = now_ms();
    rc = enqueue_pass(p, s, n_pos, ticket);
    if (pipe_timing) fprintf(stderr, "[isx_pipe_submit_reads] copy-in queue %.2f ms, pass + copy-out queue %.2f ms\n", t_q1 - t_q0, now_ms() - t_q1);
    return rc;
}

struct isx_wire {
    isx_pipe *pipe = nullptr;
    uint8_t *h = nullptr;
    size_t bytes = 0;
    size_t o_bounds = 0, o_win = 0, o_ref = 0, o_gbase = 0, o_pairs = 0, o_rec = 0;
    size_t bounds_bytes = 0, win_bytes = 0, ref_bytes = 0, gbase_bytes = 0, pairs_bytes = 0, rec_bytes = 0;
    int64_t n_pos = 0, n_bases = 0, n_rec = 0, n_seg = 0;
    int32_t n_splits = 0;
    uint64_t n_pairs = 0;
    int W = 0, packed = 0;
    bool ref_has_n = false;
    float stage_ms = 0.f;
    int encode_passes = 1;
    uint8_t *d_ref = nullptr;
    int device = 0;
};

static int stage_common(isx_pipe *p, int64_t n_pos, const uint8_t *ref, const isx_ref_planes *rp, int32_t n_splits, const int64_t *split_bounds,
                        const isx_segs *segs, const isx_read_planes *reads, isx_wire **out)
{
    isx_segs as_segs{};
    if (reads) { as_segs.n_seg = reads->n_seg; as_segs.gpos = reads->gpos; as_segs.len = reads->len; as_segs.pair = reads->pair; segs = &as_segs; }
    *out = nullptr;
    if (!p->segs) { isx_set_error("isx_pipe_stage_reads: not a read-level pipe (isx_pipe_params.max_segs == 0)"); return ISX_ERR_STATE; }
    const bool linkage = p->prm.enable_linkage != 0;
    if (linkage && segs->n_seg && !segs->pair) { isx_set_error("linkage needs the pair array"); return ISX_ERR_ARG; }
    int rc;
    if ((rc = check_capacity(p, "isx_pipe_stage_reads", n_pos, segs->n_seg, p->pp.max_segs, n_splits)) != ISX_OK) return rc;
    if ((rc = check_split_bounds(n_pos, n_splits, split_bounds)) != ISX_OK) return rc;
    HIP_TRY(hipSetDevice(p->ctx->device));
    const double t0 = now_ms();
    std::unique_ptr<isx_wire, void (*)(isx_wire *)> w(new isx_wire(), isx_wire_free);
    w->pipe = p; w->n_pos = n_pos; w->n_splits = n_splits; w->n_seg = segs->n_seg;
    const isx_batch *b0 = p->slots[0].b;
    const int M = b0->M;
    const size_t G = p->G, rb = (size_t)p->rb;
    auto up = [](size_t v) { return (v + 255) & ~(size_t)255; };
    isxenc::SegJob J;
    std::vector<uint32_t> cmin, cmax;
    std::vector<uint8_t> cany;
    std::vector<int64_t> exact;
    for (int attempt = 0;; attempt++) {
        int64_t cap = p->drec ? isxenc::delta_groups_needed(*p->pool, segs->gpos, segs->n_seg, p->dslack) * ISX_DREC_GROUP
                              : isxenc::seg_groups_needed(*p->pool, segs->gpos, segs->n_seg) * ISX_SEG_GROUP;
        if (!exact.empty()) { cap = 0; for (int64_t v : exact) cap += std::max<int64_t>(v, 1) * ISX_DREC_GROUP; }
        if (cap > p->cap_rec) { isx_set_error("isx_pipe_stage_reads: the stream needs more records than the pipe's capacity (raise jump_slack)"); return ISX_ERR_CAPACITY; }
        const size_t n_groups = (size_t)cap / G;
        w->bounds_bytes = (size_t)(n_splits + 1) * sizeof(int64_t);
        w->ref_bytes = ref2_bytes(n_pos) + refn_bytes(n_pos);
        const size_t win_cap = ((size_t)n_pos / 64 + 2) * sizeof(uint2);
        size_t o = 0;
        w->o_bounds = o; o = up(o + w->bounds_bytes);
        w->o_win = o; o = up(o + win_cap);
        w->o_ref = o; o = up(o + w->ref_bytes);
        w->o_gbase = o; o = up(o + n_groups * sizeof(uint32_t));
        w->o_pairs = o; if (linkage && !p->drec) o = up(o + (size_t)cap * sizeof(uint32_t));
        w->o_rec = o; o = up(o + (size_t)cap * rb);
        if (w->h) { isx_pin_free(w->h); w->h = nullptr; }
        HIP_TRY(isx_pin_malloc(reinterpret_cast<void **>(&w->h), o));
        w->bytes = o;
        cmin.assign(n_groups + 2, 0xFFFFFFFFu); cmax.assign(n_groups + 2, 0u); cany.assign(n_groups + 2, 0);
        J = isxenc::SegJob();
        J.n_seg = segs->n_seg; J.n_pos = n_pos; J.n_mm_bins = M;
        if (reads) { J.in2 = *reads; if (!linkage) J.in2.pair = nullptr; }
        else { J.in = *segs; if (!linkage) J.in.pair = nullptr; }
        J.rec = reinterpret_cast<uint32_t *>(w->h + w->o_rec);
        J.gbase = reinterpret_cast<uint32_t *>(w->h + w->o_gbase);
        J.pair_out = linkage && !p->drec ? reinterpret_cast<uint32_t *>(w->h + w->o_pairs) : nullptr;
        J.cmin = cmin.data(); J.cmax = cmax.data(); J.cany = cany.data();
        J.cap_rec = cap;
        int erc;
// ... 79 lines not shown
}

int64_t isx_wire_bytes(const isx_wire *w) { return w ? (int64_t)(w->bounds_bytes + w->win_bytes + (w->d_ref ? 0 : w->ref_bytes) + w->gbase_bytes + w->pairs_bytes + w->rec_bytes) : 0; }

int isx_pipe_submit_wire(isx_pipe *p, const isx_wire *w, int64_t *ticket)
{
    if (!p || !w || !ticket) { isx_set_error("isx_pipe_submit_wire: bad argument"); return ISX_ERR_ARG; }
    if (w->pipe != p) { isx_set_error("isx_pipe_submit_wire: the batch was staged for another pipe"); return ISX_ERR_ARG; }
    drain_stager(p);
    Slot *slot = nullptr;
    int rc = slot_acquire(p, "isx_pipe_submit_wire", &slot);
    if (rc != ISX_OK) return rc;
    Slot &s = *slot;
    isx_batch *b = s.b;
    const double t0 = now_ms();
    b->n_pos = w->n_pos; b->n_obs = w->n_bases; b->n_splits = w->n_splits; b->n_rec = (uint64_t)w->n_rec;
    b->n_pairs = w->n_pairs;
    s.ref_has_n = w->ref_has_n;
    b->packed = w->packed; b->W = w->W;
    b->n_win = (int)(w->win_bytes / sizeof(uint2));
    if ((rc = slot_shape_pass(p, s)) != ISX_OK) return rc;
    slot_bind_inputs(p, s, w->d_ref);
    HIP_TRY(hipEventRecord(s.ev_h2d0, H2D(p, s)));
    HIP_TRY(hipMemcpyAsync(s.d_in + s.off_bounds, w->h + w->o_bounds, w->bounds_bytes, hipMemcpyHostToDevice, H2D(p, s)));
    HIP_TRY(hipMemcpyAsync(s.d_in + s.off_win, w->h + w->o_win, w->win_bytes, hipMemcpyHostToDevice, H2D(p, s)));
    if (!w->d_ref) HIP_TRY(hipMemcpyAsync(s.d_in + s.off_ref, w->h + w->o_ref, w->ref_bytes, hipMemcpyHostToDevice, H2D(p, s)));
    HIP_TRY(hipMemcpyAsync(s.d_in + s.off_gbase, w->h + w->o_gbase, w->gbase_bytes, hipMemcpyHostToDevice, H2D(p, s)));
    if (w->pairs_bytes) HIP_TRY(hipMemcpyAsync(s.d_in + s.off_pairs, w->h + w->o_pairs, w->pairs_bytes, hipMemcpyHostToDevice, H2D(p, s)));
    HIP_TRY(hipMemcpyAsync(s.d_in + s.off_rec, w->h + w->o_rec, w->rec_bytes, hipMemcpyHostToDevice, H2D(p, s)));
    HIP_TRY(hipEventRecord(s.ev_h2d1, H2D(p, s)));
    s.h2d_split = false;
    s.h2d_bytes = isx_wire_bytes(w);
    s.encode_ms = (float)(now_ms() - t0);
    s.encode_passes = 0;
    return enqueue_pass(p, s, w->n_pos, ticket);
}

int isx_pipe_submit_reads(isx_pipe *p, int64_t n_pos, const uint8_t *ref, int32_t n_splits, const int64_t *split_bounds,
                          const isx_segs *segs, int64_t *ticket)
{
    if (!p || !ref || !split_bounds || !ticket || n_pos <= 0 || n_splits <= 0 || !segs || segs->n_seg < 0 ||
        (segs->n_seg && (!segs->gpos || !segs->len || !segs->bases))) {
        isx_set_error("isx_pipe_submit_reads: bad argument");
        return ISX_ERR_ARG;
    }
    if (!p->segs) { isx_set_error("isx_pipe_submit_reads: not a read-level pipe (isx_pipe_params.max_segs == 0)"); return ISX_ERR_STATE; }
    if (p->prm.enable_linkage && segs->n_seg && !segs->pair) { isx_set_error("linkage needs the pair array"); return ISX_ERR_ARG; }
    if (p->stager.joinable()) {
        isx_pipe::StageJob job;
        job.n_pos = n_pos; job.ref = ref; job.segs = *segs;
        if (!p->prm.enable_linkage) job.segs.pair = nullptr;
        job.bounds.assign(split_bounds, split_bounds + n_splits + 1);
        return queue_for_stager(p, std::move(job), "isx_pipe_submit_reads", ticket);
    }
    isxenc::SegJob J;
    J.in = *segs; J.n_seg = segs->n_seg;
    if (!p->prm.enable_linkage) J.in.pair = nullptr;
    return submit_segs_common(p, n_pos, ref, n_splits, split_bounds, J, ticket);
}

int isx_pipe_submit_planes(isx_pipe *p, int64_t n_pos, const isx_ref_planes *ref, int32_t n_splits, const int64_t *split_bounds,
                           const isx_read_planes *reads, int64_t *ticket)
{
    if (!p || !ref || !ref->plane2 || !split_bounds || !ticket || n_pos <= 0 || n_splits <= 0 || !reads || reads->n_seg < 0 ||
        (reads->n_seg && (!reads->gpos || !reads->len || !reads->planes))) {
        isx_set_error("isx_pipe_submit_planes: bad argument");
        return ISX_ERR_ARG;
    }
    if (!p->segs || !p->drec) { isx_set_error("isx_pipe_submit_planes: bit-plane reads need a read-level pipe (max_segs > 0) with one mm bin (n_mm_bins == 1) or ISX_LAYOUT_MM_DELTA_RECORDS"); return ISX_ERR_STATE; }
    if (p->prm.enable_linkage && reads->n_seg && !reads->pair) { isx_set_error("linkage needs the pair array"); return ISX_ERR_ARG; }
    if (p->stager.joinable()) {
        isx_pipe::StageJob job;
        job.n_pos = n_pos; job.ref = nullptr; job.planes = true; job.reads = *reads; job.rp = *ref;
        if (!p->prm.enable_linkage) job.reads.pair = nullptr;
        job.bounds.assign(split_bounds, split_bounds + n_splits + 1);
        return queue_for_stager(p, std::move(job), "isx_pipe_submit_planes", ticket);
    }
    isxenc::SegJob J;
    J.in2 = *reads; J.n_seg = reads->n_seg;
    if (!p->prm.enable_linkage) J.in2.pair = nullptr;
    return submit_segs_common(p, n_pos, nullptr, n_splits, split_bounds, J, ticket, ref);
}

int isx_pipe_set_reference_budget(isx_pipe *p, int64_t mib)
{
    if (!p) { isx_set_error("isx_pipe_set_reference_budget: bad argument"); return ISX_ERR_ARG; }
    p->ref_cache_budget.store(mib < 0 ? 0 : (size_t)(mib ? mib : 4096) << 20, std::memory_order_relaxed);
    return ISX_OK;
}

int isx_pipe_submit(isx_pipe *p, int64_t n_pos, const uint8_t *ref, int32_t n_splits, const int64_t *split_bounds,
                    int64_t n_obs, const isx_obs *obs, const uint32_t *pair, int64_t *ticket)
{
    if (!p || !ref || !split_bounds || !ticket || n_pos <= 0 || n_splits <= 0 || n_obs < 0 || (n_obs && !obs)) {
        isx_set_error("isx_pipe_submit: bad argument");
        return ISX_ERR_ARG;
    }
    if (p->prm.enable_linkage && n_obs && !pair) { isx_set_error("linkage needs the pair array"); return ISX_ERR_ARG; }
    if (p->segs) { isx_set_error("isx_pipe_submit: a read-level pipe takes isx_pipe_submit_reads / isx_pipe_submit_bam"); return ISX_ERR_STATE; }
    isxenc::EncodeJob J;
    J.obs = obs; J.pair = p->prm.enable_linkage ? pair : nullptr;
    static const isx_obs none{};
    if (!n_obs) J.obs = &none;
    return submit_common(p, n_pos, ref, n_splits, split_bounds, n_obs, J, ticket);
}

int isx_pipe_submit_bam(isx_pipe *p, isx_bam *bam, const struct isx_bam_params_s *bp, const int32_t *refs, int32_t n_refs,
                        const uint8_t *ref, int32_t n_splits, const int64_t *split_bounds, struct isx_bam_info_s *info, int64_t *ticket)
{
    if (!p || !bam || !bp || !refs || n_refs <= 0 || !ref || !ticket) { isx_set_error("isx_pipe_submit_bam: bad argument"); return ISX_ERR_ARG; }
    BamBatch *q = nullptr;
    const double t_in = now_ms();
    drain_stager(p);
    int rc = bam_batch_prepare(bam, bp, refs, n_refs, &q, 0, -1, p->segs);
    if (rc != ISX_OK) return rc;
    const double t_prep = now_ms();
    std::unique_ptr<BamBatch, void (*)(BamBatch *)> Q(q, bam_batch_free);
    const int64_t n_pos = bam_batch_n_pos(q), n_obs = p->segs ? bam_batch_seg_bases(q) : bam_batch_n_obs(q);
    const std::vector<int64_t> &own = bam_batch_bounds(q);
    if (!split_bounds) { split_bounds = own.data(); n_splits = (int32_t)own.size() - 1; }
    if (n_splits <= 0) { isx_set_error("isx_pipe_submit_bam: no splits"); return ISX_ERR_ARG; }
    if (info) bam_batch_info(q, n_refs, info);
    if (p->segs) {
        isxenc::SegJob J;
        J.n_seg = bam_batch_n_segs(q);
        J.gpos_all = bam_batch_seg_gpos(q);
        J.want_pairs = p->prm.enable_linkage != 0;
        if (p->drec && !getenv("ISX_BAM_SEG_WORDS")) J.produce_planes = [q](int64_t first, int64_t count, uint32_t *g, uint8_t *l, uint8_t *m, uint32_t *pr, uint64_t *pl) { bam_batch_emit_planes(q, first, count, g, l, m, pr, pl); };
        else J.produce = [q](int64_t first, int64_t count, uint32_t *g, uint8_t *l, uint8_t *m, uint32_t *pr, uint32_t *b) { bam_batch_emit_segs(q, first, count, g, l, m, pr, b); };
        rc = submit_segs_common(p, n_pos, ref, n_splits, split_bounds, J, ticket);
    } else {
        isxenc::EncodeJob J;
        J.obs = nullptr;
        J.want_pairs = p->prm.enable_linkage != 0;
        J.produce = [q](int64_t first, uint32_t count, isx_obs *o, uint32_t *pr) { bam_batch_emit(q, first, count, o, pr); };
        rc = submit_common(p, n_pos, ref, n_splits, split_bounds, n_obs, J, ticket);
    }
    const double t_sub = now_ms();
    if (rc == ISX_OK) {
        std::lock_guard<std::mutex> lk(p->mu);
        Slot &s = p->slots[(size_t)(*ticket % (int64_t)p->slots.size())];
        if (s.ticket == *ticket && s.state == 1) s.dead_batch = Q.release();
    }
    if (Q) bam_batch_retire(Q.release());
    if (pipe_timing)
        fprintf(stderr, "[isx_pipe_submit_bam] prepare %.1f ms, encode + enqueue %.1f ms, free %.1f ms\n", t_prep - t_in, t_sub - t_prep, now_ms() - t_sub);
    return rc;
}

int isx_pipe_collect(isx_pipe *p, int64_t ticket, isx_pipe_result *out)
{
    if (!p || !out || ticket < 0) { isx_set_error("isx_pipe_collect: bad argument"); return ISX_ERR_ARG; }
    Slot &s = p->slots[(size_t)(ticket % (int64_t)p->slots.size())];
    isx_ctx *c = p->ctx;
    isx_batch *b = s.b;
    const bool dense = b->M == 1;
    *out = isx_pipe_result{};
    {
        const double t0 = now_ms();
        std::unique_lock<std::mutex> lk(p->mu);
        if (ticket < p->next_promise) p->cv_done.wait(lk, [&] { return p->next_ticket > ticket; });
        if (s.ticket != ticket || s.state == 0) { isx_set_error("isx_pipe_collect: unknown or already released ticket"); return ISX_ERR_STATE; }
        p->cv_done.wait(lk, [&] { return s.state == 2; });
        out->collect_wait_ms = (float)(now_ms() - t0);
        if (s.rc != ISX_OK) { isx_set_error(s.err); return s.rc; }
    }
// ... 191 lines not shown
```

instrain_amd/csrc/seg_encode.cpp:

```cpp
#include "seg_encode.h"

#include <immintrin.h>

#include <algorithm>
#include <atomic>
#include <cstdlib>
#include <cstring>
#include <string>
#include <vector>

void isx_set_error(const std::string &msg);

namespace isxenc {

namespace {

constexpr int64_t TASK = 4096;
constexpr uint32_t SPAN = 65535u;

inline int64_t count_groups(const uint32_t *gpos, int64_t a, int64_t e, int64_t group = ISX_SEG_GROUP)
{
    int64_t n = 0;
    for (int64_t i = a; i < e;) {
        uint32_t lo = gpos[i], hi = gpos[i];
// ... 467 lines not shown
    }
    J.need_slack = fits ? slack : std::max<int64_t>(worst, slack + 1);
    if (!fits) return SEG_CAPACITY;
    return SEG_OK;
}


namespace {

struct LenMasks {
    alignas(32) uint64_t m[ISX_SEG_BASES + 1][4];
    LenMasks()
    {
        for (uint32_t L = 0; L <= ISX_SEG_BASES; L++)
            for (uint32_t k = 0; k < 4; k++) {
                const uint32_t from = 64 * k;
                m[L][k] = L <= from ? 0 : (L - from >= 64 ? ~(uint64_t)0 : (((uint64_t)1 << (L - from)) - 1));
            }
    }
};

inline bool cpu_has_bmi2()
{
    static const bool v = __builtin_cpu_supports("bmi2") && !getenv("ISX_NO_BMI2");
    return v;
}

inline uint64_t even_bits_portable(uint64_t x)
{
    x &= 0x5555555555555555ull;
    x = (x | (x >> 1)) & 0x3333333333333333ull;
    x = (x | (x >> 2)) & 0x0F0F0F0F0F0F0F0Full;
    x = (x | (x >> 4)) & 0x00FF00FF00FF00FFull;
    x = (x | (x >> 8)) & 0x0000FFFF0000FFFFull;
    x = (x | (x >> 16)) & 0x00000000FFFFFFFFull;
    return x;
}

inline void bits160(const uint8_t *q, uint32_t sh, uint64_t d[3])
{
    uint64_t w[4];
    memcpy(w, q, 32);
    for (int i = 0; i < 3; i++) d[i] = (w[i] >> sh) | ((w[i + 1] << 1) << (63 - sh));
}

struct PlaneTask {
    int64_t a, e;
    const uint32_t *gp, *pr, *gpos_all;
    const uint8_t *ln;
    const uint8_t *mm = nullptr;
    const uint64_t *pl;
    uint32_t *rec0;
    int64_t g0, ga, ge;
    bool fast_store;
    int64_t used = 0, np = 0, nb = 0;
    uint32_t maxp = 0;
};

inline void put_empty_drec(uint32_t *o)
{
    o[0] = o[1] = o[2] = o[4] = o[5] = o[6] = o[7] = 0;
    o[3] = ISX_DREC_NO_EXC;
}

#ifndef ISX_PLANES_PREFETCH
#define ISX_PLANES_PREFETCH 16
#endif
constexpr int64_t PLANES_PREFETCH = ISX_PLANES_PREFETCH;
struct PlaneGroup {
    alignas(64) uint32_t rec[ISX_DREC_GROUP][ISX_DREC_WORDS];
    int n = 0, open = -1;
    uint32_t lo = 0, hi = 0, last = 0;
    int64_t g = 0, used = 0;
};
__attribute__((noinline)) void rebase_drecs(PlaneGroup &G, uint32_t new_lo)
{
    const uint32_t up = G.lo - new_lo;
    for (int r = 0; r < G.n; r++) {
        uint32_t *o = G.rec[r];
        if ((o[0] >> 16) & 0xFFu) o[0] += up;
        if ((o[0] & ISX_DREC_DUAL) && ((o[4] >> 16) & 0xFFu)) o[4] += up;
    }
    G.lo = new_lo;
}

struct PlaneScratch {
    std::vector<uint32_t> gpos, pair;
    std::vector<uint8_t> len, mm;
    std::vector<uint64_t> planes;
    uint64_t *pl = nullptr;
};

#define ISX_PLANES_FN planes_task_portable
#define ISX_CLOSE_FN close_group_portable
#define ISX_DIFFERS_FN differs160_portable
#define ISX_PLANES_VARIANT 0
#include "seg_planes.inc"
#undef ISX_PLANES_FN
#undef ISX_CLOSE_FN
#undef ISX_DIFFERS_FN
#undef ISX_PLANES_VARIANT
#pragma GCC push_options
#pragma GCC target("bmi,bmi2,popcnt,lzcnt")
#define ISX_PLANES_FN planes_task_bmi2
#define ISX_CLOSE_FN close_group_bmi2
#define ISX_DIFFERS_FN differs160_bmi2
#define ISX_PLANES_VARIANT 1
#include "seg_planes.inc"
#undef ISX_PLANES_FN
#undef ISX_CLOSE_FN
#undef ISX_DIFFERS_FN
#undef ISX_PLANES_VARIANT
#pragma GCC pop_options
#pragma GCC push_options
#pragma GCC target("bmi,bmi2,popcnt,lzcnt,avx512f,avx512bw,avx512vl,avx512vbmi2,gfni")
#define ISX_PLANES_FN planes_task_avx512
#define ISX_CLOSE_FN close_group_avx512
#define ISX_DIFFERS_FN differs160_avx512
#define ISX_PLANES_VARIANT 2
#include "seg_planes.inc"
#undef ISX_PLANES_FN
#undef ISX_CLOSE_FN
#undef ISX_DIFFERS_FN
#undef ISX_PLANES_VARIANT
#pragma GCC pop_options

inline int planes_variant()
{
    static const int v = [] {
        if (const char *e = getenv("ISX_PLANES_VARIANT")) return std::max(0, std::min(2, atoi(e)));
        if (!cpu_has_bmi2()) return 0;
        return cpu_has_avx512() && __builtin_cpu_supports("avx512vbmi2") && __builtin_cpu_supports("gfni") ? 2 : 1;
    }();
    if (v == 2 && !(cpu_has_avx512() && __builtin_cpu_supports("avx512vbmi2") && __builtin_cpu_supports("gfni") && __builtin_cpu_supports("bmi2"))) return __builtin_cpu_supports("bmi2") ? 1 : 0;
    if (v == 1 && !__builtin_cpu_supports("bmi2")) return 0;
    return v;
}

}

int encode_planes(HostPool &pool, SegJob &J)
{
    const int64_t n = J.n_seg;
    const bool producer = (bool)J.produce_planes;
    const uint32_t *gpos_all = producer ? J.gpos_all : J.in2.gpos;
    const int n_tasks = (int)((n + TASK - 1) / TASK);
    const int64_t slack = std::max<int64_t>(J.slack_groups, 1);
    std::vector<int64_t> g_at((size_t)n_tasks + 1, 0);
    if (J.task_groups) for (int t = 0; t < n_tasks; t++) g_at[(size_t)t + 1] = std::max<int64_t>(J.task_groups[t], 1);
    else pool.run(n_tasks, [&](int t) {
        const int64_t a = (int64_t)t * TASK, e = std::min<int64_t>(n, a + TASK);
        g_at[(size_t)t + 1] = count_groups(gpos_all, a, e, 2 * ISX_DREC_GROUP) + slack;
    });
    for (int t = 0; t < n_tasks; t++) g_at[(size_t)t + 1] += g_at[(size_t)t];
    const int64_t n_groups = std::max<int64_t>(g_at[(size_t)n_tasks], 1);
    J.n_rec = n_groups * ISX_DREC_GROUP;
    J.need_slack = slack;
    if (J.n_rec > J.cap_rec) return SEG_CAPACITY;
    std::atomic<int> err{SEG_OK};
    std::vector<int64_t> bases_of((size_t)std::max(n_tasks, 1), 0), need_of((size_t)std::max(n_tasks, 1), 0), pieces_of((size_t)std::max(n_tasks, 1), 0);
    std::vector<uint32_t> maxp_of((size_t)std::max(n_tasks, 1), 0);
    const bool pairs = producer ? J.want_pairs : J.in2.pair != nullptr;
    const int64_t RG = J.ring_groups;
    constexpr size_t group_words = (size_t)ISX_DREC_GROUP * ISX_DREC_WORDS;
    const bool fast_store = cpu_has_avx512() && (reinterpret_cast<uintptr_t>(J.rec) & 63) == 0;
    const int variant = planes_variant();
    if (n == 0) {
        if (RG) J.wave_begin(0);
        for (int r = 0; r < ISX_DREC_GROUP; r++) put_empty_drec(J.rec + (size_t)r * ISX_DREC_WORDS);
        J.gbase[0] = 0; J.cmin[0] = 0xFFFFFFFFu; J.cmax[0] = 0; J.cany[0] = 0;
        J.n_bases = 0; J.max_pair = 0; J.n_pieces = 0;
        if (RG) J.wave_flush(0, 0, 1);
        return SEG_OK;
    }
    auto run_task = [&](int t, int64_t wave_g0, int half) {
        if (err.load(std::memory_order_relaxed) != SEG_OK) return;
        const int64_t a = (int64_t)t * TASK, e = std::min<int64_t>(n, a + TASK);
        const uint32_t *gp, *pr;
        const uint8_t *ln, *mmv = nullptr;
        const uint64_t *pl;
        if (producer) {
            thread_local PlaneScratch S;
            if (S.gpos.size() < (size_t)TASK) {
                S.gpos.resize((size_t)TASK); S.pair.resize((size_t)TASK); S.len.resize((size_t)TASK); S.mm.resize((size_t)TASK);
                S.planes.resize((size_t)TASK * ISX_PLANE_WORDS + 8);
                S.pl = reinterpret_cast<uint64_t *>((reinterpret_cast<uintptr_t>(S.planes.data()) + 63) & ~(uintptr_t)63);
            }
            J.produce_planes(a, e - a, S.gpos.data(), S.len.data(), J.n_mm_bins > 1 ? S.mm.data() : nullptr, pairs ? S.pair.data() : nullptr, S.pl);
            gp = S.gpos.data() - a; ln = S.len.data() - a; pr = pairs ? S.pair.data() - a : nullptr;
            if (J.n_mm_bins > 1) mmv = S.mm.data() - a;
            pl = S.pl - (size_t)a * ISX_PLANE_WORDS;
        } else {
            gp = J.in2.gpos; ln = J.in2.len; pr = pairs ? J.in2.pair : nullptr; pl = J.in2.planes;
            if (J.n_mm_bins > 1) mmv = J.in2.mm;
        }
        PlaneTask K;
        K.a = a; K.e = e; K.gp = gp; K.ln = ln; K.mm = mmv; K.pr = pr; K.pl = pl; K.gpos_all = gpos_all;
        K.rec0 = RG ? J.rec + (size_t)((int64_t)half * RG) * group_words : J.rec;
        K.g0 = RG ? wave_g0 : 0; K.ga = g_at[(size_t)t]; K.ge = g_at[(size_t)t + 1]; K.fast_store = fast_store;
        if (variant == 2) planes_task_avx512(J, err, K);
        else if (variant == 1) planes_task_bmi2(J, err, K);
        else planes_task_portable(J, err, K);
        if (err.load(std::memory_order_relaxed) != SEG_OK) return;
        need_of[(size_t)t] = K.used;
        bases_of[(size_t)t] = K.nb; maxp_of[(size_t)t] = K.maxp; pieces_of[(size_t)t] = K.np;
    };
    if (!RG) pool.run(n_tasks, [&](int t) { run_task(t, 0, 0); });
    else {
        int half = 0;
        for (int t0 = 0; t0 < n_tasks && err.load() == SEG_OK;) {
            int t1 = t0 + 1;
            while (t1 < n_tasks && g_at[(size_t)t1 + 1] - g_at[(size_t)t0] <= RG) t1++;
            if (g_at[(size_t)t1] - g_at[(size_t)t0] > RG) return SEG_CAPACITY;
            J.wave_begin(half);
            const int64_t wg0 = g_at[(size_t)t0];
            pool.run(t1 - t0, [&](int k) { run_task(t0 + k, wg0, half); });
            if (err.load() == SEG_OK) J.wave_flush(half, wg0, g_at[(size_t)t1]);
            t0 = t1; half ^= 1;
        }
    }
    if (err.load() != SEG_OK) return err.load();
    J.n_bases = 0; J.max_pair = 0; J.n_pieces = 0;
    int64_t worst = 0;
    bool fits = true;
    J.task_need.assign(need_of.begin(), need_of.begin() + n_tasks);
    for (int t = 0; t < n_tasks; t++) {
        J.n_bases += bases_of[(size_t)t]; J.max_pair = std::max(J.max_pair, maxp_of[(size_t)t]); J.n_pieces += pieces_of[(size_t)t];
        const int64_t region = g_at[(size_t)t + 1] - g_at[(size_t)t];
        if (need_of[(size_t)t] > region) fits = false;
        worst = std::max(worst, need_of[(size_t)t] - (region - (J.task_groups ? 0 : slack)));
    }
    J.need_slack = fits ? slack : std::max<int64_t>(worst, slack + 1);
    if (!fits) return SEG_CAPACITY;
    return SEG_OK;
}


namespace {
__attribute__((target("bmi2")))
inline void pack_ref_piece_bmi2(const uint8_t *r, int64_t n, uint8_t *o2, uint8_t *on, bool &seen)
{
    int64_t i = 0;
    uint64_t any = 0;
    for (; i + 8 <= n; i += 8) {
        uint64_t x;
        memcpy(&x, r + i, 8);
        const uint64_t bad = x & 0xFCFCFCFCFCFCFCFCull;
        if (__builtin_expect(bad == 0, 1)) {
            const uint16_t v = (uint16_t)_pext_u64(x, 0x0303030303030303ull);
            memcpy(o2 + (i >> 2), &v, 2);
            on[i >> 3] = 0;
            continue;
        }
        uint64_t t = bad | (bad >> 4);
        t |= t >> 2; t |= t >> 1;
        const uint64_t nb = t & 0x0101010101010101ull;
        const uint64_t keep = ~(nb * 0xFFull);
        const uint16_t v = (uint16_t)_pext_u64(x & keep, 0x0303030303030303ull);
        memcpy(o2 + (i >> 2), &v, 2);
        on[i >> 3] = (uint8_t)_pext_u64(nb, 0x0101010101010101ull);
        any |= nb;
    }
    for (; i < n; i += 8) {
        uint32_t lo = 0, hi = 0, nbits = 0;
        const int64_t m = std::min<int64_t>(8, n - i);
        for (int64_t k = 0; k < m; k++) {
            const uint32_t c = r[i + k];
            const uint32_t b = c > 3u;
            nbits |= b << k;
            const uint32_t v = b ? 0u : c;
            if (k < 4) lo |= v << (2 * k); else hi |= v << (2 * (k - 4));
        }
        o2[i >> 2] = (uint8_t)lo;
        if (m > 4) o2[(i >> 2) + 1] = (uint8_t)hi;
        on[i >> 3] = (uint8_t)nbits;
        any |= nbits;
    }
    seen = any != 0;
}

inline void pack_ref_piece_scalar(const uint8_t *r, int64_t n, uint8_t *o2, uint8_t *on, bool &seen)
{
    seen = false;
    for (int64_t i = 0; i < n; i += 8) {
        uint32_t lo = 0, hi = 0, nb = 0;
        const int64_t m = std::min<int64_t>(8, n - i);
        for (int64_t k = 0; k < m; k++) {
            const uint32_t c = r[i + k];
            const uint32_t bad = c > 3u;
            nb |= bad << k;
            const uint32_t v = bad ? 0u : c;
            if (k < 4) lo |= v << (2 * k); else hi |= v << (2 * (k - 4));
        }
        o2[i >> 2] = (uint8_t)lo;
        if (m > 4) o2[(i >> 2) + 1] = (uint8_t)hi;
        on[i >> 3] = (uint8_t)nb;
        seen |= nb != 0;
    }
}
}

bool pack_ref_planes(HostPool &pool, const uint8_t *ref, int64_t n_pos, uint8_t *plane2, uint8_t *nplane)
{
    const int64_t piece = (int64_t)256 << 10;
    const int n_tasks = (int)((n_pos + piece - 1) / piece);
    std::atomic<int> any{0};
    const bool bmi2 = cpu_has_bmi2();
    auto cp = [&](int t) {
        const int64_t a = (int64_t)t * piece, e = std::min<int64_t>(n_pos, a + piece);
        bool seen = false;
        if (bmi2) pack_ref_piece_bmi2(ref + a, e - a, plane2 + (a >> 2), nplane + (a >> 3), seen);
        else pack_ref_piece_scalar(ref + a, e - a, plane2 + (a >> 2), nplane + (a >> 3), seen);
        if (seen) any.store(1, std::memory_order_relaxed);
    };
    if (n_tasks > 1) pool.run(n_tasks, cp); else if (n_tasks == 1) cp(0);
    return any.load() != 0;
// ... 165 lines not shown
                                 [&](int64_t, int64_t, int64_t cols) { n += (cols + ISX_SEG_BASES - 1) / ISX_SEG_BASES; });
        if (!ok) { isx_set_error("isx_count_read_segs: unknown CIGAR operator"); return ISX_ERR_ARG; }
    }
    *n_seg = n;
    return ISX_OK;
}

int isx_pack_reads(int64_t n_reads, const int64_t *ref_start, const int64_t *clip_lo, const int64_t *clip_hi,
                   const uint32_t *cigar, const int64_t *cigar_off, const char *seq, const uint8_t *qual, const int64_t *seq_off,
                   const uint8_t *mm, const uint32_t *pair, int32_t min_base_quality, int64_t cap_seg, uint32_t *seg_gpos,
                   uint8_t *seg_len, uint8_t *seg_mm, uint32_t *seg_pair, uint32_t *seg_bases, int64_t *n_seg)
{
    if (n_reads < 0 || !n_seg || cap_seg < 0 || (n_reads && (!ref_start || !clip_lo || !clip_hi || !cigar || !cigar_off || !seq || !qual || !seq_off)) ||
        (cap_seg && (!seg_gpos || !seg_len || !seg_bases)) || (pair && cap_seg && !seg_pair)) {
        isx_set_error("isx_pack_reads: bad argument");
        return ISX_ERR_ARG;
    }
    int64_t n = 0;
    bool full = false, bad = false;
    for (int64_t r = 0; r < n_reads && !full && !bad; r++) {
        const char *sq = seq + seq_off[r];
        const uint8_t *ql = qual + seq_off[r];
        const int64_t q_len = seq_off[r + 1] - seq_off[r];
        const bool ok = for_runs(cigar + cigar_off[r], cigar_off[r + 1] - cigar_off[r], ref_start[r], clip_lo[r], clip_hi[r],
                                 [&](int64_t pos, int64_t q0, int64_t cols) {
            if (q0 + cols > q_len || pos < 0 || pos + cols > (int64_t)0xFFFFFFFFll) { bad = true; return; }
            for (int64_t c0 = 0; c0 < cols && !full; c0 += ISX_SEG_BASES) {
                const int L = (int)std::min<int64_t>(ISX_SEG_BASES, cols - c0);
                if (n >= cap_seg) { full = true; return; }
                uint32_t *w = seg_bases + (size_t)n * ISX_SEG_WORDS;
                for (int k = 0; k < ISX_SEG_WORDS; k++) w[k] = ISX_SEG_SKIP_WORD;
                for (int j = 0; j < L; j++) {
                    const int64_t qi = q0 + c0 + j;
                    const uint32_t code = (int)ql[qi] >= min_base_quality ? ascii_code(sq[qi]) : 4u;
                    w[j / 10] = (w[j / 10] & ~(7u << (3 * (j % 10)))) | (code << (3 * (j % 10)));
                }
                seg_gpos[n] = (uint32_t)(pos + c0); seg_len[n] = (uint8_t)L;
                if (seg_mm) seg_mm[n] = mm ? mm[r] : (uint8_t)0;
                if (seg_pair) seg_pair[n] = pair ? pair[r] : 0u;
                n++;
            }
        });
        if (!ok) { isx_set_error("isx_pack_reads: unknown CIGAR operator"); return ISX_ERR_ARG; }
    }
    if (bad) { isx_set_error("isx_pack_reads: a CIGAR reaches beyond its read's bases or the flat space"); return ISX_ERR_ARG; }
    if (full) { isx_set_error("isx_pack_reads: more segments than cap_seg (isx_count_read_segs gives the number)"); return ISX_ERR_CAPACITY; }
    *n_seg = n;
    return ISX_OK;
}

int isx_pack_ref_planes(const uint8_t *ref, int64_t n_pos, int32_t host_threads, uint8_t *plane2, uint8_t *nplane, int32_t *has_n)
{
    if (!ref || n_pos <= 0 || !plane2 || !nplane) { isx_set_error("isx_pack_ref_planes: bad argument"); return ISX_ERR_ARG; }
    isxenc::HostPool pool(std::max(1, host_threads), -1, false);
    const bool any = isxenc::pack_ref_planes(pool, ref, n_pos, plane2, nplane);
    if (has_n) *has_n = any ? 1 : 0;
    return ISX_OK;
}

int isx_planes_from_segs(const isx_segs *segs, int32_t host_threads, uint64_t *planes)
{
    if (!segs || segs->n_seg < 0 || (segs->n_seg && (!segs->len || !segs->bases || !planes))) { isx_set_error("isx_planes_from_segs: bad argument"); return ISX_ERR_ARG; }
    const int64_t n = segs->n_seg, piece = 8192;
    std::atomic<bool> bad{false};
    isxenc::HostPool pool(std::max(1, host_threads), -1, false);
    pool.run((int)((n + piece - 1) / piece), [&](int t) {
        const int64_t a = (int64_t)t * piece, e = std::min<int64_t>(n, a + piece);
        for (int64_t i = a; i < e; i++) {
            const uint32_t L = segs->len[i];
            if (L == 0 || L > ISX_SEG_BASES) { bad.store(true); return; }
            isxenc::planes_from_words(segs->bases + (size_t)i * ISX_SEG_WORDS, L, planes + (size_t)i * ISX_PLANE_WORDS);
        }
    });
    if (bad.load()) { isx_set_error("a segment's length is not in [1, 150]"); return ISX_ERR_ARG; }
    return ISX_OK;
}

int isx_encode_planes(const isx_read_planes *reads, const isx_ref_planes *ref, int64_t n_pos, int32_t host_threads, int32_t slack_groups,
                      int64_t cap_rec, int64_t ring_records, uint32_t *rec, uint32_t *gbase, int64_t *n_rec, int64_t *need_slack)
{
    return isx_encode_planes_mm(reads, ref, n_pos, 1, host_threads, slack_groups, cap_rec, ring_records, rec, gbase, n_rec, need_slack);
}

int isx_encode_planes_mm(const isx_read_planes *reads, const isx_ref_planes *ref, int64_t n_pos, int32_t n_mm_bins, int32_t host_threads, int32_t slack_groups,
                         int64_t cap_rec, int64_t ring_records, uint32_t *rec, uint32_t *gbase, int64_t *n_rec, int64_t *need_slack)
{
    if (n_mm_bins < 1 || n_mm_bins > 128) { isx_set_error("isx_encode_planes: n_mm_bins must be in [1, 128]"); return ISX_ERR_ARG; }
    if (!reads || !ref || !ref->plane2 || !rec || !gbase || !n_rec || reads->n_seg < 0 || cap_rec < ISX_DREC_GROUP || (cap_rec % ISX_DREC_GROUP) || n_pos <= 0 ||
        (reads->n_seg && (!reads->gpos || !reads->len || !reads->planes)) || ring_records < 0 ||
        (ring_records % (2 * ISX_DREC_GROUP)) || slack_groups < 0) {
        isx_set_error("isx_encode_planes: bad argument");
        return ISX_ERR_ARG;
    }
    std::vector<uint32_t> ring;
    isxenc::HostPool pool(std::max(1, host_threads), -1, false);
    std::vector<uint32_t> cmin((size_t)(cap_rec / ISX_DREC_GROUP)), cmax(cmin.size());
    std::vector<uint8_t> cany(cmin.size());
    isxenc::SegJob J;
    J.in2 = *reads; J.n_seg = reads->n_seg; J.n_pos = n_pos; J.n_mm_bins = n_mm_bins;
    J.ref2 = ref->plane2; J.refn = ref->nplane; J.slack_groups = std::max(1, slack_groups);
    J.rec = rec; J.gbase = gbase; J.pair_out = nullptr;
    J.cmin = cmin.data(); J.cmax = cmax.data(); J.cany = cany.data(); J.cap_rec = cap_rec;
    if (ring_records) {
        const int64_t half = ring_records / 2;
        ring.assign((size_t)ring_records * ISX_DREC_WORDS + 16, 0xABABABABu);
        uint32_t *r0 = reinterpret_cast<uint32_t *>((reinterpret_cast<uintptr_t>(ring.data()) + 63) & ~(uintptr_t)63);
        J.rec = r0;
        J.ring_groups = half / ISX_DREC_GROUP;
        J.wave_begin = [](int) {};
        J.wave_flush = [&, r0](int h, int64_t g0, int64_t g1) {
            const size_t gw = (size_t)ISX_DREC_GROUP * ISX_DREC_WORDS;
            memcpy(rec + (size_t)g0 * gw, r0 + (size_t)h * half * ISX_DREC_WORDS, (size_t)(g1 - g0) * gw * 4);
            std::fill_n(r0 + (size_t)h * half * ISX_DREC_WORDS, (size_t)half * ISX_DREC_WORDS, 0xABABABABu);
        };
    }
    const int rc = isxenc::encode_planes(pool, J);
    if (need_slack) *need_slack = J.need_slack;
    *n_rec = J.n_rec;
    if (rc == isxenc::SEG_CAPACITY) {
        isx_set_error(J.need_slack > J.slack_groups ? "isx_encode_planes: a task needs more spare groups than slack_groups (see *need_slack)"
                                                    : "isx_encode_planes: the stream does not fit cap_rec records");
        return ISX_ERR_CAPACITY;
    }
    if (rc == isxenc::SEG_BAD_POS) { isx_set_error("a segment reaches beyond n_pos"); return ISX_ERR_ARG; }
    if (rc == isxenc::SEG_BAD_LEN) { isx_set_error("a segment's length is not in [1, 150]"); return ISX_ERR_ARG; }
    if (rc == isxenc::SEG_MM_RANGE) { isx_set_error("a segment has mm >= n_mm_bins"); return ISX_ERR_MM_RANGE; }
    return ISX_OK;
}

int isx_pack_read_planes(int64_t n_reads, const int64_t *ref_start, const int64_t *clip_lo, const int64_t *clip_hi,
                         const uint32_t *cigar, const int64_t *cigar_off, const char *seq, const uint8_t *qual, const int64_t *seq_off,
                         const uint32_t *pair, int32_t min_base_quality, int64_t cap_seg, uint32_t *seg_gpos,
                         uint8_t *seg_len, uint32_t *seg_pair, uint64_t *seg_planes, int64_t *n_seg)
{
    if (n_reads < 0 || !n_seg || cap_seg < 0 || (n_reads && (!ref_start || !clip_lo || !clip_hi || !cigar || !cigar_off || !seq || !qual || !seq_off)) ||
        (cap_seg && (!seg_gpos || !seg_len || !seg_planes)) || (pair && cap_seg && !seg_pair)) {
        isx_set_error("isx_pack_read_planes: bad argument");
        return ISX_ERR_ARG;
    }
    int64_t n = 0;
    bool full = false, bad = false;
    for (int64_t r = 0; r < n_reads && !full && !bad; r++) {
        const char *sq = seq + seq_off[r];
        const uint8_t *ql = qual + seq_off[r];
        const int64_t q_len = seq_off[r + 1] - seq_off[r];
        const bool ok = for_runs(cigar + cigar_off[r], cigar_off[r + 1] - cigar_off[r], ref_start[r], clip_lo[r], clip_hi[r],
                                 [&](int64_t pos, int64_t q0, int64_t cols) {
            if (q0 + cols > q_len || pos < 0 || pos + cols > (int64_t)0xFFFFFFFFll) { bad = true; return; }
            for (int64_t c0 = 0; c0 < cols && !full; c0 += ISX_SEG_BASES) {
                const int L = (int)std::min<int64_t>(ISX_SEG_BASES, cols - c0);
                if (n >= cap_seg) { full = true; return; }
                uint64_t *P = seg_planes + (size_t)n * ISX_PLANE_WORDS;
                for (int k = 0; k < ISX_PLANE_WORDS; k++) P[k] = 0;
                for (int j = 0; j < L; j++) {
                    const int64_t qi = q0 + c0 + j;
                    const uint32_t code = (int)ql[qi] >= min_base_quality ? ascii_code(sq[qi]) : 4u;
                    if (code >= 4) {
                        P[5 + (j >> 6)] |= (uint64_t)1 << (j & 63);
                        if (code == 5) { P[j >> 5] |= (uint64_t)1 << (2 * (j & 31)); P[7] |= (uint64_t)1 << 63; }
                    } else P[j >> 5] |= (uint64_t)code << (2 * (j & 31));
                }
                seg_gpos[n] = (uint32_t)(pos + c0); seg_len[n] = (uint8_t)L;
                if (seg_pair) seg_pair[n] = pair ? pair[r] : 0u;
                n++;
            }
        });
        if (!ok) { isx_set_error("isx_pack_read_planes: unknown CIGAR operator"); return ISX_ERR_ARG; }
    }
    if (bad) { isx_set_error("isx_pack_read_planes: a CIGAR reaches beyond its read's bases or the flat space"); return ISX_ERR_ARG; }
    if (full) { isx_set_error("isx_pack_read_planes: more segments than cap_seg (isx_count_read_segs gives the number)"); return ISX_ERR_CAPACITY; }
    *n_seg = n;
    return ISX_OK;
}

}
```

instrain_amd/csrc/seg_encode.h:

```cpp
#pragma once
#include <stdint.h>

#include <functional>
#include <vector>

#include "../../include/instrain_amd.h"
#include "obs_encode.h"

#define ISX_SEG_GROUP 16
#define ISX_SEG_REC_WORDS 16
#define ISX_DREC_GROUP 32

namespace isxenc {

struct SegJob {
    isx_segs in{};
    std::function<void(int64_t first, int64_t count, uint32_t *gpos, uint8_t *len, uint8_t *mm, uint32_t *pair, uint32_t *bases)> produce;
    const uint32_t *gpos_all = nullptr;
    isx_read_planes in2{};
    std::function<void(int64_t first, int64_t count, uint32_t *gpos, uint8_t *len, uint8_t *mm, uint32_t *pair, uint64_t *planes)> produce_planes;
    const uint8_t *ref2 = nullptr, *refn = nullptr;
    int64_t n_seg = 0, n_pos = 0;
    int n_mm_bins = 1;
    bool want_pairs = false;
    uint32_t *rec = nullptr;
    uint32_t *gbase = nullptr;
    uint32_t *pair_out = nullptr;
    uint32_t *cmin = nullptr, *cmax = nullptr;
    uint8_t *cany = nullptr;
    int64_t cap_rec = 0;
    int64_t ring_groups = 0;
    std::function<void(int half)> wave_begin;
    std::function<void(int half, int64_t g0, int64_t g1)> wave_flush;
    const uint8_t *ref = nullptr;
    int64_t slack_groups = 1;
    int64_t need_slack = 0;
    std::vector<int64_t> task_need;
    const int64_t *task_groups = nullptr;
    int64_t n_pieces = 0;
    int64_t n_rec = 0;
    int64_t n_bases = 0;
    uint32_t max_pair = 0;
};

enum { SEG_OK = 0, SEG_CAPACITY = 1, SEG_MM_RANGE = 2, SEG_BAD_POS = 3, SEG_BAD_LEN = 4 };

int encode_segs(HostPool &pool, SegJob &job);
int encode_delta(HostPool &pool, SegJob &job);
int encode_planes(HostPool &pool, SegJob &job);
int64_t delta_groups_needed(HostPool &pool, const uint32_t *gpos, int64_t n, int64_t slack_groups);
int64_t seg_groups_needed(HostPool &pool, const uint32_t *gpos, int64_t n);
bool pack_ref_planes(HostPool &pool, const uint8_t *ref, int64_t n_pos, uint8_t *plane2, uint8_t *nplane);
void planes_from_words(const uint32_t *words, uint32_t len, uint64_t *planes);

}
```

instrain_amd/csrc/seg_planes.inc:

```

#if ISX_PLANES_VARIANT == 2
static inline __attribute__((always_inline)) __m256i ISX_DIFFERS_FN(const uint8_t *q, uint32_t sh, __m512i P)
{
    const __m512i lo = _mm512_maskz_loadu_epi64((__mmask8)0x1F, q), hi = _mm512_maskz_loadu_epi64((__mmask8)0x1F, q + 8);
    const __m512i r = _mm512_shrdv_epi64(lo, hi, _mm512_set1_epi64((long long)sh));
    const __m512i x = _mm512_xor_si512(r, P);
    const __m512i m = _mm512_or_si512(x, _mm512_srli_epi64(x, 1));
    const __m512i nib = _mm512_gf2p8affine_epi64_epi8(m, _mm512_set1_epi64((long long)0x0104104000000000ull), 0);
    const __m512i t = _mm512_or_si512(nib, _mm512_srli_epi16(nib, 4));
    return _mm512_cvtepi16_epi8(t);
}
#else
static inline __attribute__((always_inline)) void ISX_DIFFERS_FN(const uint8_t *q, uint32_t sh, const uint64_t *P, uint64_t d[3])
{
    uint64_t w[6];
    memcpy(w, q, 48);
    uint64_t e[5];
    for (int i = 0; i < 5; i++) {
        const uint64_t r = (w[i] >> sh) | ((w[i + 1] << 1) << (63 - sh));
        const uint64_t x = r ^ P[i];
        const uint64_t m = x | (x >> 1);
#if ISX_PLANES_VARIANT == 1
        e[i] = _pext_u64(m, 0x5555555555555555ull);
#else
        e[i] = even_bits_portable(m);
#endif
    }
    d[0] = e[0] | (e[1] << 32);
    d[1] = e[2] | (e[3] << 32);
    d[2] = e[4];
}
#endif

static __attribute__((noinline)) void ISX_CLOSE_FN(SegJob &J, const PlaneTask &K, PlaneGroup &G)
{
    if (!G.n) return;
    if (G.g < K.ge) {
        for (int r = G.n; r < ISX_DREC_GROUP; r++) put_empty_drec(G.rec[r]);
        uint32_t *o = K.rec0 + (size_t)(G.g - K.g0) * (size_t)ISX_DREC_GROUP * ISX_DREC_WORDS;
        if (!K.fast_store) memcpy(o, G.rec, sizeof G.rec);
        else {
#if ISX_PLANES_VARIANT == 2
            for (int r = 0; r < ISX_DREC_GROUP; r += 2) _mm512_stream_si512(reinterpret_cast<__m512i *>(o + (size_t)r * ISX_DREC_WORDS), _mm512_load_si512(G.rec[r]));
#else
            const __m128i *src = reinterpret_cast<const __m128i *>(G.rec);
            __m128i *dst = reinterpret_cast<__m128i *>(o);
            for (int i = 0; i < ISX_DREC_GROUP * ISX_DREC_WORDS / 4; i++) _mm_stream_si128(dst + i, _mm_load_si128(src + i));
#endif
        }
        J.gbase[G.g] = G.lo; J.cmin[G.g] = G.lo; J.cmax[G.g] = G.last; J.cany[G.g] = 1;
        G.g++;
    }
    G.used++;
    G.n = 0; G.open = -1;
}

#if ISX_PLANES_VARIANT == 0
#define ISX_TZ64(x) ((x) ? (uint32_t)__builtin_ctzll(x) : 64u)
#else
#define ISX_TZ64(x) ((uint32_t)_tzcnt_u64(x))
#endif
static void ISX_PLANES_FN(SegJob &J, std::atomic<int> &err, PlaneTask &K)
{
    static const LenMasks LM;
    PlaneGroup G;
    G.g = K.ga;
    const uint8_t *const ref2 = J.ref2, *const refn = J.refn;
    const int64_t n_pos = J.n_pos;
    const int64_t safe_pos = n_pos - 200;
    const uint32_t *const gp = K.gp, *const pr = K.pr, *const ga = K.gpos_all;
    const uint8_t *const ln = K.ln;
    int64_t nb = 0, np = 0;
    uint32_t maxp = 0;
    auto place = [&](uint32_t start, uint32_t len, bool plain, bool &fill) __attribute__((always_inline)) -> uint32_t * {
        fill = plain && G.open >= 0;
        if (G.n) {
            const uint32_t nlo = std::min(G.lo, start), nhi = std::max(G.hi, start);
            if (__builtin_expect(nhi - nlo > SPAN || (!fill && G.n == ISX_DREC_GROUP), 0)) { ISX_CLOSE_FN(J, K, G); fill = false; }
        }
        if (!G.n) { G.lo = G.hi = start; G.last = start + len - 1; }
        else {
            if (__builtin_expect(start < G.lo, 0)) rebase_drecs(G, start);
            G.hi = std::max(G.hi, start); G.last = std::max(G.last, start + len - 1);
        }
        np++;
        if (fill) { uint32_t *o = G.rec[G.open] + 4; G.open = -1; return o; }
        uint32_t *o = G.rec[G.n];
        G.open = plain ? G.n : -1;
        G.n++;
        return o;
    };
    uint32_t hdr_hi = 0;
    auto add_full = [&](uint32_t start, uint32_t len, uint32_t pid, uint64_t s0, uint64_t s1, uint64_t s2, uint32_t exc) __attribute__((always_inline)) {
        bool fill;
        uint32_t *o = place(start, len, false, fill);
        const uint64_t v0 = (uint64_t)((start - G.lo) | (len << 16) | hdr_hi) | (s0 << 32), v1 = (s0 >> 32) | ((uint64_t)exc << 32);
        const uint64_t v3 = (s2 & 0xFFFFFFFFull) | ((uint64_t)pid << 32);
        memcpy(o, &v0, 8); memcpy(o + 2, &v1, 8); memcpy(o + 4, &s1, 8); memcpy(o + 6, &v3, 8);
    };
    auto add_plain = [&](uint32_t start, uint32_t len, uint32_t pid, uint32_t exc0, uint32_t exc1) __attribute__((always_inline)) {
        bool fill;
        uint32_t *o = place(start, len, true, fill);
        const uint64_t v0 = (uint64_t)((start - G.lo) | (len << 16) | hdr_hi | ISX_DREC_DUAL) | ((uint64_t)pid << 32), v1 = (uint64_t)exc0 | ((uint64_t)exc1 << 32);
        memcpy(o, &v0, 8); memcpy(o + 2, &v1, 8);
        if (!fill) {
            const uint64_t v2 = (uint64_t)ISX_DREC_DUAL, v3 = (uint64_t)ISX_DREC_NO_EXC | ((uint64_t)ISX_DREC_NO_EXC << 32);
            memcpy(o + 4, &v2, 8); memcpy(o + 6, &v3, 8);
        }
    };
#if ISX_PLANES_VARIANT == 2
    const __m256i rec_idx = _mm256_setr_epi32(8, 0, 1, 8, 2, 3, 4, 8);
#endif
    const bool mm_on = J.n_mm_bins > 1;
    const int64_t pf_end = K.e - PLANES_PREFETCH;
    for (int64_t s = K.a; s < K.e; s++) {
        const uint32_t L = ln[s], p = gp[s];
        const uint64_t *P = K.pl + (size_t)s * ISX_PLANE_WORDS;
        if (s < pf_end) {
            _mm_prefetch(reinterpret_cast<const char *>(P + (size_t)PLANES_PREFETCH * ISX_PLANE_WORDS), _MM_HINT_T0);
            _mm_prefetch(reinterpret_cast<const char *>(ref2 + (gp[s + PLANES_PREFETCH] >> 2) + 40), _MM_HINT_T0);
        }
        if (__builtin_expect(L == 0 || L > ISX_SEG_BASES, 0)) { err.store(SEG_BAD_LEN); return; }
        if (__builtin_expect((int64_t)p + (int64_t)L > n_pos || p != ga[s], 0)) { err.store(SEG_BAD_POS); return; }
        const uint32_t pid = pr ? pr[s] : 0u;
        maxp = pid > maxp ? pid : maxp;
        nb += L;
        const uint64_t *lm = LM.m[L];
        uint64_t s0, s1, s2, ex[3];
        bool n_marked = false;
        if (mm_on) {
            const uint32_t mv = K.mm ? K.mm[s] : 0u;
            if (__builtin_expect((int)mv >= J.n_mm_bins || mv > 127u, 0)) { err.store(SEG_MM_RANGE); return; }
            hdr_hi = mv << 24;
            n_marked = (P[7] >> 63) != 0;
        }
#if ISX_PLANES_VARIANT == 2
        __m256i skv = _mm256_setzero_si256();
        const bool in_regs = (int64_t)p < safe_pos && !refn && !n_marked;
        if (__builtin_expect(in_regs, 1)) {
            const __m512i Pv = _mm512_loadu_si512(P);
            const __m256i lmv = _mm256_loadu_si256(reinterpret_cast<const __m256i *>(lm));
            skv = _mm256_and_si256(_mm256_maskz_loadu_epi64((__mmask8)0x7, P + 5), lmv);
            const __m256i dv = ISX_DIFFERS_FN(ref2 + (p >> 2), (p & 3u) * 2u, Pv);
            const __m256i exv = _mm256_and_si256(dv, _mm256_xor_si256(skv, lmv));
            alignas(32) uint64_t t[8];
            _mm256_store_si256(reinterpret_cast<__m256i *>(t), skv);
            _mm256_store_si256(reinterpret_cast<__m256i *>(t + 4), exv);
            s0 = t[0]; s1 = t[1]; s2 = t[2];
            ex[0] = t[4]; ex[1] = t[5]; ex[2] = t[6];
        } else
#endif
        {
            s0 = P[5] & lm[0]; s1 = P[6] & lm[1]; s2 = P[7] & lm[2];
            uint64_t d[3];
#if ISX_PLANES_VARIANT == 2
            alignas(32) uint64_t dq[4];
#define ISX_DIFFERS_AT(q_, sh_) do { _mm256_store_si256(reinterpret_cast<__m256i *>(dq), ISX_DIFFERS_FN((q_), (sh_), _mm512_loadu_si512(P))); d[0] = dq[0]; d[1] = dq[1]; d[2] = dq[2]; } while (0)
#else
#define ISX_DIFFERS_AT(q_, sh_) ISX_DIFFERS_FN((q_), (sh_), P, d)
#endif
            if (__builtin_expect((int64_t)p < safe_pos, 1)) {
                ISX_DIFFERS_AT(ref2 + (p >> 2), (p & 3u) * 2u);
                if (refn) {
                    uint64_t nn[3];
                    if (__builtin_expect((int64_t)p + 264 <= n_pos, 1)) bits160(refn + (p >> 3), p & 7u, nn);
                    else {
                        uint8_t bn[32] = {0};
                        const int64_t haven = (n_pos + 7) / 8 - (int64_t)(p >> 3);
                        memcpy(bn, refn + (p >> 3), (size_t)std::min<int64_t>(32, haven));
                        bits160(bn, p & 7u, nn);
                    }
                    d[0] |= nn[0]; d[1] |= nn[1]; d[2] |= nn[2];
                }
            } else {
                alignas(64) uint8_t buf[64] = {0};
                const int64_t have2 = (n_pos + 3) / 4 - (int64_t)(p >> 2);
                memcpy(buf, ref2 + (p >> 2), (size_t)std::min<int64_t>(48, have2));
                ISX_DIFFERS_AT(buf, (p & 3u) * 2u);
                if (refn) {
                    uint8_t bn[32] = {0};
                    const int64_t haven = (n_pos + 7) / 8 - (int64_t)(p >> 3);
                    memcpy(bn, refn + (p >> 3), (size_t)std::min<int64_t>(32, haven));
                    uint64_t nn[3];
                    bits160(bn, p & 7u, nn);
                    d[0] |= nn[0]; d[1] |= nn[1]; d[2] |= nn[2];
                }
            }
#undef ISX_DIFFERS_AT
            ex[0] = d[0] & (lm[0] ^ s0); ex[1] = d[1] & (lm[1] ^ s1); ex[2] = d[2] & (lm[2] ^ s2);
            if (__builtin_expect(n_marked, 0)) {
                ex[0] |= (even_bits_portable(P[0]) | (even_bits_portable(P[1]) << 32)) & s0;
                ex[1] |= (even_bits_portable(P[2]) | (even_bits_portable(P[3]) << 32)) & s1;
                ex[2] |= even_bits_portable(P[4]) & s2;
            }
        }
        const bool plain = (s0 | s1 | s2) == 0;
        const uint32_t n_exc = (uint32_t)(__builtin_popcountll(ex[0]) + __builtin_popcountll(ex[1]) + __builtin_popcountll(ex[2]));
        if (__builtin_expect(n_exc <= 1, 1)) {
            const uint32_t t0 = ISX_TZ64(ex[0]), t1 = ISX_TZ64(ex[1]), t2 = ISX_TZ64(ex[2] | ((uint64_t)1 << 63));
            const uint32_t m0 = 0u - (uint32_t)(ex[0] == 0), m01 = m0 & (0u - (uint32_t)(ex[1] == 0));
            const uint32_t col = t0 + (t1 & m0) + (t2 & m01);
            const uint32_t code = (uint32_t)(P[col >> 5] >> (2 * (col & 31u))) & 3u;
            const uint32_t w0 = 0x3FFFFC00u | ((col | (code << 8) | (0u - (uint32_t)(n_exc == 0))) & 0x3FFu);
            if (__builtin_expect(plain, 0)) { add_plain(p, L, pid, w0, ISX_DREC_NO_EXC); continue; }
#if ISX_PLANES_VARIANT == 2
            if (__builtin_expect(in_regs, 1)) {
                bool fill;
                uint32_t *o = place(p, L, false, fill);
                __m256i v = _mm256_permutex2var_epi32(skv, rec_idx, _mm256_set1_epi32((int)w0));
                v = _mm256_mask_set1_epi32(v, (__mmask8)0x01, (int)((p - G.lo) | (L << 16) | hdr_hi));
                v = _mm256_mask_set1_epi32(v, (__mmask8)0x80, (int)pid);
                _mm256_store_si256(reinterpret_cast<__m256i *>(o), v);
                continue;
            }
#endif
            add_full(p, L, pid, s0, s1, s2, w0);
            continue;
        }
        const uint32_t max_exc = plain ? ISX_DREC_EXC : ISX_DREC_EXC_FULL;
        if (__builtin_expect(n_exc <= max_exc, 1)) {
            uint64_t fields = 0;
            for (uint32_t i = 0; i < n_exc; i++) {
                const int k = ex[0] ? 0 : (ex[1] ? 1 : 2);
                const uint32_t col = (uint32_t)(64 * k + __builtin_ctzll(ex[k]));
                ex[k] &= ex[k] - 1;
                const uint64_t code = (P[col >> 5] >> (2 * (col & 31u))) & 3u;
                fields |= ((uint64_t)col | (code << 8)) << (10 * i);
            }
            const uint64_t all = (fields | (0x0FFFFFFFFFFFFFFFull << (10 * n_exc))) & 0x0FFFFFFFFFFFFFFFull;
            const uint32_t w0 = (uint32_t)all & ISX_DREC_NO_EXC, w1 = (uint32_t)(all >> 30) & ISX_DREC_NO_EXC;
            if (plain) add_plain(p, L, pid, w0, w1);
            else add_full(p, L, pid, s0, s1, s2, w0);
            continue;
        }
        const uint64_t sk[3] = {s0, s1, s2};
        uint32_t b = 0;
        while (b < L) {
            uint32_t w[2] = {ISX_DREC_NO_EXC, ISX_DREC_NO_EXC};
            uint32_t nf = 0, end = L;
            for (int k = 0; k < 3; k++) {
                while (ex[k]) {
                    const uint32_t col = (uint32_t)(64 * k + __builtin_ctzll(ex[k]));
                    if (nf == max_exc) { end = col; goto cut; }
                    ex[k] &= ex[k] - 1;
                    const uint32_t code = (uint32_t)(P[col >> 5] >> (2 * (col & 31u))) & 3u;
                    const uint32_t f = ((col - b) & 0xFFu) | (code << 8);
                    const int wi = (int)(nf / 3), shf = 10 * (int)(nf % 3);
                    w[wi] = (w[wi] & ~(0x3FFu << shf)) | (f << shf);
                    nf++;
                }
            }
        cut:
            if (plain) add_plain(p + b, end - b, pid, w[0], w[1]);
            else if (b == 0 && end == L) add_full(p, L, pid, s0, s1, s2, w[0]);
            else {
                uint64_t msk[3];
                window160(sk, b, end - b, msk);
                add_full(p + b, end - b, pid, msk[0], msk[1], msk[2], w[0]);
            }
            b = end;
        }
    }
    ISX_CLOSE_FN(J, K, G);
    for (; G.g < K.ge; G.g++) {
        uint32_t *o = K.rec0 + (size_t)(G.g - K.g0) * (size_t)ISX_DREC_GROUP * ISX_DREC_WORDS;
        for (int r = 0; r < ISX_DREC_GROUP; r++) put_empty_drec(o + (size_t)r * ISX_DREC_WORDS);
        J.gbase[G.g] = 0; J.cmin[G.g] = 0xFFFFFFFFu; J.cmax[G.g] = 0; J.cany[G.g] = 0;
    }
    if (K.fast_store) _mm_sfence();
    K.used = G.used; K.np = np; K.nb = nb; K.maxp = maxp;
}
#undef ISX_TZ64
```

instrain_amd/engine.py:

```python
import ctypes as C
import os

import numpy as np

from . import _lib
from ._lib import (ENTRY_DT, LD_DT, OBS_DT, SNV_DT, BamInfo, BamParams, IsxError, Params, Sizes,
                   Timings, check)


def pack_obs(gpos, base, mm):
    o = np.empty(len(gpos), dtype=OBS_DT)
    o["gpos"] = gpos
    o["mm"] = mm
    o["base"] = base
    o["flags"] = 0
    return o


class SegBatch:

    def __init__(self, gpos, length, bases, mm=None, pair=None):
        self.gpos = np.ascontiguousarray(gpos, dtype=np.uint32)
        self.len = np.ascontiguousarray(length, dtype=np.uint8)
        self.bases = np.ascontiguousarray(bases, dtype=np.uint32).reshape(-1, _lib.SEG_WORDS)
# ... 367 lines not shown
            pass


class _SlotBatch(Batch):

    def __init__(self, ctx, handle, n_pos, n_obs, n_mm_bins):
        self.ctx, self.lib, self.h = ctx, ctx.lib, C.c_void_p(handle)
        self.n_pos, self.n_obs, self.n_mm_bins = int(n_pos), int(n_obs), int(n_mm_bins)

    def close(self):
        self.h = None


class Pipe:

    def __init__(self, ctx, max_pos, max_obs, max_splits, depth=4, host_threads=0, pin_threads=True, jump_slack=0.0,
                 min_cov=5, min_freq=0.05, min_snp=20, rarefied_coverage=50, n_mm_bins=1, enable_linkage=False,
                 linkage_mode=0, window=0, seed=0, layout=0, want_counts=False, ring_kib=0, max_segs=0, stage_async=False, lean_output=False):
        self.ctx, self.lib = ctx, ctx.lib
        self._held = {}
        self._wires = []
        self.stage_async = bool(stage_async) and max_segs > 0
        self.n_mm_bins = int(n_mm_bins)
        self.min_cov = int(min_cov)
        self.want_counts = bool(want_counts)
        self.enable_linkage = bool(enable_linkage)
        p = Params(int(min_cov), int(min_snp), float(min_freq), int(rarefied_coverage), int(n_mm_bins),
                   1 if enable_linkage else 0, int(linkage_mode), int(window), int(seed), int(layout), 0)
        pp = _lib.PipeParams(int(max_pos), int(max_obs), int(max_splits), int(depth), int(host_threads),
                             1 if pin_threads else 0, float(jump_slack), 1 if want_counts else 0, int(ring_kib),
                             1 if self.stage_async else 0, 1 if lean_output else 0, int(max_segs))
        self.read_level = max_segs > 0
        h = C.c_void_p()
        check(self.lib.isx_pipe_create(ctx.h, C.byref(p), C.byref(pp), C.byref(h)))
        self.h = h
        ctx._adopt(self)

    def submit(self, ref_codes, split_bounds, obs, pair=None):
        ref_codes = np.ascontiguousarray(ref_codes, dtype=np.uint8)
        split_bounds = np.ascontiguousarray(split_bounds, dtype=np.int64)
        obs = np.ascontiguousarray(obs, dtype=OBS_DT)
        if pair is not None:
            pair = np.ascontiguousarray(pair, dtype=np.uint32)
        t = C.c_int64(-1)
        check(self.lib.isx_pipe_submit(self.h, len(ref_codes), ref_codes.ctypes.data, len(split_bounds) - 1,
                                       split_bounds.ctypes.data, len(obs), obs.ctypes.data if len(obs) else None,
                                       pair.ctypes.data if pair is not None and len(obs) else None, C.byref(t)))
        return t.value

    def submit_reads(self, ref_codes, split_bounds, segs):
        ref_codes = np.ascontiguousarray(ref_codes, dtype=np.uint8)
        split_bounds = np.ascontiguousarray(split_bounds, dtype=np.int64)
        cs = segs.c(with_pair=self.enable_linkage)
        t = C.c_int64(-1)
        check(self.lib.isx_pipe_submit_reads(self.h, len(ref_codes), ref_codes.ctypes.data, len(split_bounds) - 1,
                                             split_bounds.ctypes.data, C.byref(cs), C.byref(t)))
        if self.stage_async:
            self._held[t.value] = (ref_codes, segs, cs)
        return t.value

    def stage_reads(self, ref_codes, split_bounds, segs):
        ref_codes = np.ascontiguousarray(ref_codes, dtype=np.uint8)
        split_bounds = np.ascontiguousarray(split_bounds, dtype=np.int64)
        cs = segs.c(with_pair=self.enable_linkage)
        h = C.c_void_p()
        check(self.lib.isx_pipe_stage_reads(self.h, len(ref_codes), ref_codes.ctypes.data, len(split_bounds) - 1, split_bounds.ctypes.data,
                                            C.byref(cs), C.byref(h)))
        w = Wire(self, h)
        self._wires.append(w)
        return w

    def submit_planes(self, ref_planes, split_bounds, reads, keyed=True):
        split_bounds = np.ascontiguousarray(split_bounds, dtype=np.int64)
        cr, cf = reads.c(with_pair=self.enable_linkage), ref_planes.c(keyed)
        t = C.c_int64(-1)
        check(self.lib.isx_pipe_submit_planes(self.h, ref_planes.n_pos, C.byref(cf), len(split_bounds) - 1, split_bounds.ctypes.data,
                                              C.byref(cr), C.byref(t)))
        if self.stage_async:
            self._held[t.value] = (ref_planes, reads, cr, cf)
        return t.value

    def set_reference_budget(self, mib):
        check(self.lib.isx_pipe_set_reference_budget(self.h, int(mib)))

    def stage_planes(self, ref_planes, split_bounds, reads):
        split_bounds = np.ascontiguousarray(split_bounds, dtype=np.int64)
        cr, cf = reads.c(with_pair=self.enable_linkage), ref_planes.c()
        h = C.c_void_p()
        check(self.lib.isx_pipe_stage_planes(self.h, ref_planes.n_pos, C.byref(cf), len(split_bounds) - 1, split_bounds.ctypes.data,
                                             C.byref(cr), C.byref(h)))
        w = Wire(self, h)
        self._wires.append(w)
        return w

    def submit_wire(self, wire):
        t = C.c_int64(-1)
        check(self.lib.isx_pipe_submit_wire(self.h, wire.h, C.byref(t)))
        return t.value

    def submit_bam(self, bamfile, refs, ref_codes, split_bounds=None, **kw):
        refs = np.ascontiguousarray(refs, dtype=np.int32)
        ref_codes = np.ascontiguousarray(ref_codes, dtype=np.uint8)
        sb = None if split_bounds is None else np.ascontiguousarray(split_bounds, dtype=np.int64)
        p = BamFile._params(**kw)
        info = BamInfo()
        t = C.c_int64(-1)
        rc = self.lib.isx_pipe_submit_bam(self.h, bamfile.h, C.byref(p), refs.ctypes.data, len(refs), ref_codes.ctypes.data,
                                          0 if sb is None else len(sb) - 1, None if sb is None else sb.ctypes.data,
                                          C.byref(info), C.byref(t))
        bamfile._info(info)
        check(rc)
        return t.value

    def collect(self, ticket, want_ld=True, rare_list=True, densify=True, shrunk_entries=False):
        r = _lib.PipeResult()
        check(self.lib.isx_pipe_collect(self.h, int(ticket), C.byref(r)))
        sz = {n: getattr(r.sizes, n) for n, _ in Sizes._fields_}
        out = {"sizes": sz, "ticket": r.ticket, "rows_checksum": int(r.rows_checksum),
               "stats": {k: getattr(r, k) for k in ("encode_ms", "h2d_ms", "kernel_ms", "d2h_ms", "collect_wait_ms",
                                                    "record_bytes", "encode_passes", "h2d_bytes", "d2h_bytes")}}
        n_pos = int(r.n_pos)

        def view(addr, dtype, n):
            if not n:
                return np.empty(0, dtype=dtype)
            return np.frombuffer((C.c_uint8 * (n * np.dtype(dtype).itemsize)).from_address(addr), dtype=dtype)

        slot = _SlotBatch(self.ctx, r.batch, n_pos, r.n_obs, self.n_mm_bins)
        if self.n_mm_bins == 1:
            if r.coverage16:
                out["cov16"] = view(r.coverage16, np.uint16, n_pos)
            elif r.coverage4:
                out["cov4"] = view(r.coverage4, np.uint8, (n_pos + 1) // 2)
                out["cov_window"] = int(r.cov_window)
                out["cov_row_win"] = view(r.cov_row_window, np.uint32, int(r.n_cov_rows)).copy()
                out["cov_rows"] = view(r.cov_rows, np.uint16, int(r.n_cov_rows) * int(r.cov_window)).reshape(-1, int(r.cov_window))
            else:
                out["cov8"] = view(r.coverage8, np.uint8, n_pos)
            if r.clon:
                out["clon"] = view(r.clon, np.float32, n_pos)
            else:
                out["clon_sparse"] = view(r.clon_sparse, _lib.CLON_DT, int(r.n_clon))
            if r.n_saturated and r.saturated:
                out["saturated"] = view(r.saturated, _lib.SAT_DT, int(r.n_saturated)).copy()
            if densify and ("cov8" in out or "cov4" in out):
                out["cov16"] = dense_cov(out, n_pos)
                for k in ("cov8", "cov4", "cov_rows", "cov_row_win", "cov_window"):
                    out.pop(k, None)
            if densify and "clon_sparse" in out:
                out["clon"] = dense_clon(out["cov16"], out.pop("clon_sparse"), self.min_cov)
            if r.clon_rarefied:
                out["clon_r"] = view(r.clon_rarefied, np.float32, n_pos)
            if r.rare:
                out["rare"] = view(r.rare, _lib.RARE_DT, int(r.n_rare))
            elif r.clon_rarefied and not rare_list:
                pass
            elif r.clon_rarefied:
                k = np.flatnonzero(~np.isnan(out["clon_r"]))
                out["rare"] = np.empty(len(k), dtype=_lib.RARE_DT)
                out["rare"]["gpos"] = k
                out["rare"]["clon_rarefied"] = out["clon_r"][k]
            else:
                out["rare"] = np.empty(0, dtype=_lib.RARE_DT)
            out["n_saturated"] = int(r.n_saturated)
            if r.counts:
                out["counts"] = view(r.counts, np.uint32, n_pos * 4).reshape(n_pos, 4)
# ... 144 lines not shown
        pass


def encode_obs(obs, pair=None, n_pos=None, record_bytes=2, threads=1, slack=0.0, cap_rec=None, ring_records=0):
    lib = _lib.load()
    obs = np.ascontiguousarray(obs, dtype=OBS_DT)
    G = 512 if record_bytes == 2 else 256
    if cap_rec is None:
        cap_rec = (int(len(obs) * 1.5) + 4 * 2048 + 2047) // 2048 * 2048
    if n_pos is None:
        n_pos = int(obs["gpos"].max()) + 1 if len(obs) else 1
    rec = np.empty(cap_rec, dtype=np.uint16 if record_bytes == 2 else np.uint32)
    gbase = np.empty(cap_rec // G, dtype=np.uint32)
    pout = np.empty(cap_rec, dtype=np.uint32) if pair is not None else None
    if pair is not None:
        pair = np.ascontiguousarray(pair, dtype=np.uint32)
    n_rec, passes = C.c_int64(0), C.c_int32(0)
    check(lib.isx_encode_obs_ring(obs.ctypes.data if len(obs) else None, pair.ctypes.data if pair is not None else None, len(obs),
                                  int(n_pos), int(record_bytes), int(threads), float(slack), int(cap_rec), int(ring_records),
                                  rec.ctypes.data, gbase.ctypes.data, pout.ctypes.data if pout is not None else None,
                                  C.byref(n_rec), C.byref(passes)))
    n = n_rec.value
    return rec[:n], gbase[:n // G], (pout[:n] if pout is not None else None), passes.value


def dense_clon(cov, clon_sparse, min_cov):
    out = np.where(np.asarray(cov) >= min_cov, np.float32(1.0), np.float32(np.nan)).astype(np.float32)
    out[clon_sparse["gpos"]] = clon_sparse["clon"]
    return out


def encode_segs(segs, n_pos, n_mm_bins=1, threads=1, cap_rec=None, ring_records=0):
    lib = _lib.load()
    if cap_rec is None:
        cap_rec = int(lib.isx_seg_records_needed(segs.gpos.ctypes.data if segs.n_seg else None, segs.n_seg, int(threads)))
    rec = np.empty((cap_rec, 16), dtype=np.uint32)
    gbase = np.empty(cap_rec // 16, dtype=np.uint32)
    pout = np.empty(cap_rec, dtype=np.uint32) if segs.pair is not None else None
    n_rec = C.c_int64(0)
    cs = segs.c()
    check(lib.isx_encode_segs_ring(C.byref(cs), int(n_pos), int(n_mm_bins), int(threads), int(cap_rec), int(ring_records), rec.ctypes.data,
                                   gbase.ctypes.data, pout.ctypes.data if pout is not None else None, C.byref(n_rec)))
    n = n_rec.value
    return rec[:n], gbase[:n // 16], (pout[:n] if pout is not None else None)


def encode_delta(segs, ref_codes, n_mm_bins=1, threads=1, slack_groups=1, cap_rec=None, ring_records=0, retry=True):
    lib = _lib.load()
    ref = np.ascontiguousarray(ref_codes, dtype=np.uint8)
    while True:
        cap = cap_rec if cap_rec is not None else int(lib.isx_delta_records_needed(segs.gpos.ctypes.data if segs.n_seg else None, segs.n_seg, int(threads), int(slack_groups)))
        rec = np.empty((cap, 8), dtype=np.uint32)
        gbase = np.empty(cap // 32, dtype=np.uint32)
        n_rec, need = C.c_int64(0), C.c_int64(0)
        cs = segs.c()
        rc = lib.isx_encode_delta(C.byref(cs), ref.ctypes.data, len(ref), int(n_mm_bins), int(threads), int(slack_groups), cap, int(ring_records),
                                  rec.ctypes.data, gbase.ctypes.data, None, C.byref(n_rec), C.byref(need))
        if rc == _lib.ERR_CAPACITY and retry and need.value > slack_groups and cap_rec is None:
            slack_groups = int(need.value)
            continue
        check(rc)
        n = n_rec.value
        return rec[:n], gbase[:n // 32], None, slack_groups


def encode_planes(reads, ref_planes, threads=1, slack_groups=1, cap_rec=None, ring_records=0, retry=True, n_mm_bins=1):
    lib = _lib.load()
    while True:
        cap = cap_rec if cap_rec is not None else int(lib.isx_delta_records_needed(reads.gpos.ctypes.data if reads.n_seg else None, reads.n_seg, int(threads), int(slack_groups)))
        rec = _aligned((cap, 8), np.uint32)
        gbase = np.empty(cap // 32, dtype=np.uint32)
        n_rec, need = C.c_int64(0), C.c_int64(0)
        cr, cf = reads.c(), ref_planes.c()
        rc = lib.isx_encode_planes_mm(C.byref(cr), C.byref(cf), ref_planes.n_pos, int(n_mm_bins), int(threads), int(slack_groups), cap, int(ring_records),
                                      rec.ctypes.data, gbase.ctypes.data, C.byref(n_rec), C.byref(need))
        if rc == _lib.ERR_CAPACITY and retry and need.value > slack_groups and cap_rec is None:
            slack_groups = int(need.value)
            continue
        check(rc)
        n = n_rec.value
        return rec[:n], gbase[:n // 32], None, slack_groups


def dense_cov(res, n_pos=None):
    if "cov16" in res:
        return res["cov16"]
    if "cov8" in res:
        cov = res["cov8"].astype(np.uint16)
    else:
        nib = res["cov4"]
        n_pos = 2 * len(nib) if n_pos is None else int(n_pos)
        cov = np.empty(2 * len(nib), dtype=np.uint16)
        cov[0::2] = nib & 15
        cov[1::2] = nib >> 4
        cov = cov[:n_pos]
        W = int(res["cov_window"])
        for k, w in enumerate(res["cov_row_win"].tolist()):
            lo = w * W
            hi = min(lo + W, n_pos)
            cov[lo:hi] = res["cov_rows"][k, :hi - lo]
    if "saturated" in res:
        cov[res["saturated"]["gpos"]] = np.minimum(res["saturated"]["coverage"], 65535)
    return cov


DREC_DUAL = 0x80000000
DREC_NO_EXC = 0x3FFFFFFF


def decode_delta(rec, gbase, ref_codes):
    rec = np.asarray(rec, dtype=np.uint32).reshape(-1, 8)
    ref = np.asarray(ref_codes, dtype=np.uint8)
    n = len(rec)
    dual = (rec[:, 0] >> 31) == 1
    assert ((rec[dual, 4] >> 31) == 1).all(), "a dual record's second half carries the flag too"
    zero = np.zeros(n, dtype=np.uint32)
    none = np.full(n, DREC_NO_EXC, dtype=np.uint32)
    hdr = np.stack([rec[:, 0], np.where(dual, rec[:, 4], zero)], axis=1)
    pair = np.stack([np.where(dual, rec[:, 1], rec[:, 7]), np.where(dual, rec[:, 5], zero)], axis=1)
    e0 = np.stack([np.where(dual, rec[:, 2], rec[:, 3]), np.where(dual, rec[:, 6], none)], axis=1)
    e1 = np.stack([np.where(dual, rec[:, 3], none), np.where(dual, rec[:, 7], none)], axis=1)
    skw = [np.stack([np.where(dual, zero, rec[:, k]), zero], axis=1) for k in (1, 2, 4, 5, 6)]
    gb = np.repeat(np.asarray(gbase, dtype=np.uint32), 32)[:n]
    start = (gb[:, None] + (hdr & 0xFFFF)).astype(np.int64)
    ln = ((hdr >> 16) & 0xFF).astype(np.int64)
    lvl = ((hdr >> 24) & 0x7F).astype(np.uint8)
    full = np.stack([~dual, np.zeros(n, dtype=bool)], axis=1)
    real = (ln > 0).reshape(-1)
    flat = lambda x: x.reshape(-1)[real]
    st, ln, pr, e0, e1, fl, lvl = flat(start), flat(ln), flat(pair), flat(e0), flat(e1), flat(full), flat(lvl)
    words = np.stack([flat(w) for w in skw], axis=1)
    m = len(st)
    j = np.arange(160, dtype=np.int64)[None, :]
    skip = ((words[:, :, None] >> np.arange(32, dtype=np.uint32)[None, None, :]) & 1).reshape(m, 160).astype(bool)
    assert not (skip & (j >= ln[:, None])).any(), "skip bits beyond a piece's length"
    assert skip[fl].any(axis=1).all() or True
    inside = j < ln[:, None]
    pos = np.minimum(st[:, None] + j, len(ref) - 1)
    codes = np.where(inside & ~skip, ref[pos], 4).astype(np.uint8)
    for e in (e0, e1):
        for k in range(3):
            f = (e >> (10 * k)) & 0x3FF
            has = f != 0x3FF
            off, base = (f & 0xFF).astype(np.int64), ((f >> 8) & 3).astype(np.uint8)
            rows = np.flatnonzero(has)
            assert (off[rows] < ln[rows]).all()
            mark = skip[rows, off[rows]]
            assert fl[rows[mark]].all(), "a non-ACGT marker in a dual half"
            codes[rows[mark], off[rows[mark]]] = 5
            rows = rows[~mark]
            assert (base[rows] != ref[st[rows] + off[rows]]).all(), "an exception that equals the reference"
            codes[rows, off[rows]] = base[rows]
        assert ((e >> 30) == 0).all()
    return st.astype(np.uint32), ln.astype(np.uint8), lvl, codes[:, :150], pr, fl


def decode_segs(rec, gbase):
    rec = np.asarray(rec, dtype=np.uint32).reshape(-1, 16)
    hdr = rec[:, 0]
    ln = (hdr >> 16) & 0xFF
    real = ln > 0
    start = np.repeat(np.asarray(gbase, dtype=np.uint32), 16)[:len(rec)] + (hdr & 0xFFFF)
    return start[real], ln[real].astype(np.uint8), (hdr[real] >> 24).astype(np.uint8), unpack_codes(rec[real, 1:])


def pack_reads(ref_start, clip_lo, clip_hi, cigars, seqs, quals, mm=None, pair=None, min_base_quality=30):
# ... 316 lines not shown
```

Measured before the change: 136.1.

## Send only reference words touched by mismatching reads instead of full planes

During host encoding, the 32-position reference word indices hit by mismatch exceptions are recorded, and the matching 2-bit and N-plane words are packed into chunks. Those sparse chunks are copied to the device, which zero-fills the reference region and scatters the words back in with a new kernel. This avoids the full reference host-to-device transfer on non-cached batches. In exchange it adds host marking work in the encode inner loop, a memset plus scatter kernel, and a fallback to the whole reference when the mark buffer overflows. Reference transfer statistics are also exposed.

Measured after the change: 106.4. -21.9%, worse.

```diff
diff --git a/include/instrain_amd.h b/include/instrain_amd.h
--- a/include/instrain_amd.h
+++ b/include/instrain_amd.h
@@ -55,6 +55,8 @@
 #define ISX_LAYOUT_MM_DELTA_RECORDS 32
 
 #define ISX_LAYOUT_NO_STRIPES 64
+
+#define ISX_LAYOUT_FULL_REFERENCE 128
 
 typedef struct {
     uint32_t gpos;
@@ -380,6 +382,17 @@
 int isx_host_unregister(const void *ptr);
 int isx_encode_planes(const isx_read_planes *reads, const isx_ref_planes *ref, int64_t n_pos, int32_t host_threads, int32_t slack_groups,
                       int64_t cap_rec, int64_t ring_records, uint32_t *rec, uint32_t *gbase, int64_t *n_rec, int64_t *need_slack);
+int isx_encode_planes_marked(const isx_read_planes *reads, const isx_ref_planes *ref, int64_t n_pos, int32_t host_threads, int32_t slack_groups,
+                             int64_t cap_rec, int64_t ring_records, uint32_t *rec, uint32_t *gbase, int64_t *n_rec, int64_t *need_slack,
+                             int64_t cap_entries, uint32_t *word_idx, uint64_t *word2, uint32_t *wordn, int64_t *n_entries, int32_t *whole);
+typedef struct {
+    int64_t batches_sparse;
+    int64_t batches_whole;
+    int64_t batches_fallback;
+    int64_t entries;
+    int64_t ref_bytes;
+} isx_ref_stats;
+int isx_pipe_reference_stats(isx_pipe *p, isx_ref_stats *out);
 int isx_encode_planes_mm(const isx_read_planes *reads, const isx_ref_planes *ref, int64_t n_pos, int32_t n_mm_bins, int32_t host_threads, int32_t slack_groups,
                          int64_t cap_rec, int64_t ring_records, uint32_t *rec, uint32_t *gbase, int64_t *n_rec, int64_t *need_slack);
 
diff --git a/instrain_amd/_lib.py b/instrain_amd/_lib.py
--- a/instrain_amd/_lib.py
+++ b/instrain_amd/_lib.py
@@ -52,6 +52,7 @@
 PLANE_WORDS = 8
 LAYOUT_MM_ENTRIES = 16
 LAYOUT_MM_DELTA_RECORDS = 32
+LAYOUT_FULL_REFERENCE = 128
 ABI_VERSION = 5
 
 
@@ -61,6 +62,10 @@
 
 class RefPlanes(C.Structure):
     _fields_ = [("plane2", C.c_void_p), ("nplane", C.c_void_p), ("key", C.c_uint64)]
+
+
+class RefStats(C.Structure):
+    _fields_ = [("batches_sparse", C.c_int64), ("batches_whole", C.c_int64), ("batches_fallback", C.c_int64), ("entries", C.c_int64), ("ref_bytes", C.c_int64)]
 
 
 RARE_DT = np.dtype([("gpos", "<u4"), ("clon_rarefied", "<f4")])
@@ -157,7 +162,7 @@
            "isx_batch_summarize", "isx_batch_summarize_genomes", "isx_compare_coverage", "isx_compare_scaffolds", "isx_compare_fetch_snps",
            "isx_genes_create", "isx_genes_destroy", "isx_genes_sites", "isx_batch_profile_genes", "isx_genes_profile_snvs",
            "isx_pipe_create", "isx_pipe_destroy", "isx_pipe_submit", "isx_pipe_submit_reads", "isx_pipe_stage_reads", "isx_pipe_submit_wire", "isx_wire_bytes", "isx_wire_free", "isx_wire_keep_reference", "isx_pipe_submit_bam", "isx_encode_segs", "isx_encode_segs_ring", "isx_seg_records_needed", "isx_encode_delta", "isx_delta_records_needed", "isx_count_read_segs", "isx_pack_reads", "isx_pipe_collect", "isx_pipe_release", "isx_pipe_fetch_entries", "isx_pipe_fetch_entries_shrunk", "isx_levels_expand", "isx_encode_obs", "isx_encode_obs_ring",
-           "isx_pack_ref_planes", "isx_planes_from_segs", "isx_pack_read_planes", "isx_pipe_submit_planes", "isx_pipe_stage_planes", "isx_encode_planes", "isx_encode_planes_mm", "isx_pipe_set_reference_budget", "isx_host_register", "isx_host_unregister",
+           "isx_pack_ref_planes", "isx_planes_from_segs", "isx_pack_read_planes", "isx_pipe_submit_planes", "isx_pipe_stage_planes", "isx_encode_planes", "isx_encode_planes_mm", "isx_encode_planes_marked", "isx_pipe_reference_stats", "isx_pipe_set_reference_budget", "isx_host_register", "isx_host_unregister",
            "isx_bgzf_index", "isx_bgzf_inflate_device", "isx_bgzf_inflate_host", "isx_bgzf_inflate_fast",
            "isx_bam_open", "isx_bam_close", "isx_bam_close_wait", "isx_bam_set_threads", "isx_bam_ref", "isx_bam_set_priority_reads", "isx_bam_scan", "isx_bam_scan_part",
            "isx_bam_insert_sizes", "isx_bam_set_wanted_refs", "isx_bam_pair_keys", "isx_bam_set_cross_names", "isx_bam_filter_insert_sizes", "isx_bam_filter", "isx_bam_set_r2m", "isx_bam_r2m", "isx_bam_drop_names", "isx_bam_batch_pair_names", "isx_bam_set_mm_cap", "isx_bam_mm_levels", "isx_bam_set_mm_levels", "isx_bam_ref_counts",
@@ -280,6 +285,9 @@
     lib.isx_pipe_stage_planes.argtypes = [vp, i64, C.POINTER(RefPlanes), i32, vp, C.POINTER(ReadPlanes), C.POINTER(vp)]
     lib.isx_encode_planes.argtypes = [C.POINTER(ReadPlanes), C.POINTER(RefPlanes), i64, i32, i32, i64, i64, vp, vp, C.POINTER(i64), C.POINTER(i64)]
     lib.isx_encode_planes_mm.argtypes = [C.POINTER(ReadPlanes), C.POINTER(RefPlanes), i64, i32, i32, i32, i64, i64, vp, vp, C.POINTER(i64), C.POINTER(i64)]
+    lib.isx_encode_planes_marked.argtypes = [C.POINTER(ReadPlanes), C.POINTER(RefPlanes), i64, i32, i32, i64, i64, vp, vp, C.POINTER(i64), C.POINTER(i64),
+                                             i64, vp, vp, vp, C.POINTER(i64), C.POINTER(i32)]
+    lib.isx_pipe_reference_stats.argtypes = [vp, C.POINTER(RefStats)]
     lib.isx_bam_ref.argtypes = [vp, i32, C.POINTER(C.c_char_p), C.POINTER(i64), C.POINTER(i64)]
     lib.isx_bam_copy.argtypes = [vp, vp, vp, vp, vp]
     lib.isx_bam_view.argtypes = [vp, C.POINTER(vp), C.POINTER(vp)]
diff --git a/instrain_amd/csrc/isx_pipe.hip b/instrain_amd/csrc/isx_pipe.hip
--- a/instrain_amd/csrc/isx_pipe.hip
+++ b/instrain_amd/csrc/isx_pipe.hip
@@ -90,6 +90,10 @@
     int64_t ticket = -1;
     BamBatch *dead_batch = nullptr;
     bool ref_has_n = false;
+    std::unique_ptr<isxenc::RefMarks> marks;
+    uint8_t *d_words = nullptr;
+    size_t words_bytes = 0;
+    bool words_pending = false, words_with_n = false;
     int state = 0;
     int rc = 0;
     std::string err;
@@ -245,6 +249,7 @@
     struct RefEntry { uint8_t *d = nullptr; size_t bytes = 0; int64_t n_pos = 0; bool has_n = false; hipEvent_t ready = nullptr; uint64_t sum = 0; };
     std::unordered_map<uint64_t, RefEntry> ref_cache;
     size_t ref_cache_bytes = 0;
+    std::atomic<int64_t> ref_stat[5] = {};
     std::atomic<size_t> ref_cache_budget{(size_t)4096 << 20};
     std::thread stager;
     std::deque<StageJob> stage_q;
@@ -321,6 +326,7 @@
         if (s.d_gpos16) isx_dev_free(s.d_gpos16);
         if (s.d_in) isx_dev_free(s.d_in);
         if (s.d_runs) isx_dev_free(s.d_runs);
+        if (s.d_words) isx_dev_free(s.d_words);
         t_dev += now_ms() - t_x; t_x = now_ms();
         if (s.h_in) isx_pin_free(s.h_in);
         host_block_free(s.h_runs, s.runs_pinned);
@@ -877,6 +883,19 @@
 
 void isx_pipe_destroy(isx_pipe *p) { pipe_free(p); }
 
+__global__ void __launch_bounds__(256) k_scatter_ref_words(const uint8_t *__restrict__ words, uint64_t n_slots, uint32_t with_n, uint64_t *__restrict__ ref2,
+                                                           uint32_t *__restrict__ refn, uint32_t n_words2, uint32_t n_wordsn)
+{
+    const uint64_t i = (uint64_t)blockIdx.x * 256u + threadIdx.x;
+    if (i >= n_slots) return;
+    const uint8_t *c = words + (i / ISX_RMARK_CHUNK) * (uint64_t)(with_n ? ISX_RMARK_CHUNK * 16 : ISX_RMARK_CHUNK * 12);
+    const uint32_t k = (uint32_t)(i % ISX_RMARK_CHUNK);
+    const uint32_t wi = reinterpret_cast<const uint32_t *>(c)[k];
+    if (wi >= n_words2) return;
+    ref2[wi] = reinterpret_cast<const uint64_t *>(c + ISX_RMARK_CHUNK * 4)[k];
+    if (with_n && wi < n_wordsn) refn[wi] = reinterpret_cast<const uint32_t *>(c + ISX_RMARK_CHUNK * 12)[k];
+}
+
 static int enqueue_pass_impl(isx_pipe *p, Slot &s, int64_t n_pos, int64_t *ticket);
 
 static int enqueue_pass(isx_pipe *p, Slot &s, int64_t n_pos, int64_t *ticket)
@@ -901,6 +920,16 @@
     int rc = ISX_OK;
     std::unique_lock<std::mutex> launch_lk(p->launch_mu);
     HIP_TRY(hipStreamWaitEvent(ps, s.ev_h2d1, 0));
+    if (s.words_pending) {
+        const size_t r2 = ref2_bytes(n_pos), rn = s.words_with_n ? refn_bytes(n_pos) : 0;
+        HIP_TRY(hipMemsetAsync(s.d_in + s.off_ref, 0, r2 + rn, ps));
+        const uint64_t n_slots = (uint64_t)(s.words_bytes / ISX_RMARK_BYTES(s.words_with_n)) * ISX_RMARK_CHUNK;
+        if (n_slots)
+            hipLaunchKernelGGL(k_scatter_ref_words, dim3((unsigned)((n_slots + 255) / 256)), dim3(256), 0, ps, s.d_words, n_slots, s.words_with_n ? 1u : 0u,
+                               reinterpret_cast<uint64_t *>(s.d_in + s.off_ref), reinterpret_cast<uint32_t *>(s.d_in + s.off_ref + r2),
+                               (uint32_t)(r2 / 8), (uint32_t)(rn / 4));
+        s.words_pending = false;
+    }
     if (dense && p->prm.rarefied_coverage > 0 && b->rare_dense)
         HIP_TRY(hipMemsetD32Async(reinterpret_cast<hipDeviceptr_t>(b->d_clon_r), 0x7FC00000, (size_t)n_pos, ps));
     if (linkage && p->rb == 4)
@@ -971,6 +1000,7 @@
         if (s.state != 0) { isx_set_error(std::string(who) + ": every slot is in use (collect + release the oldest batch first)"); return ISX_ERR_STATE; }
     }
     HIP_TRY(hipSetDevice(p->ctx->device));
+    s.words_pending = false;
     *out = &s;
     return ISX_OK;
 }
@@ -1102,6 +1132,7 @@
 struct RefStage {
     bool early = false;
     uint8_t *resident = nullptr;
+    bool words = false;
     double host_ms = 0.0;
 };
 
@@ -1131,6 +1162,23 @@
     }
 
     const bool first_trip = rp && rp->key && p->ref_cache_budget.load(std::memory_order_relaxed) > 0;
+    if (rp && !first_trip && p->drec && s.b->M == 1 && !p->pp.want_counts && !s.b->d_counts && !(p->prm.layout & ISX_LAYOUT_FULL_REFERENCE)) {
+        const bool any_n = rp->nplane && plane_any(*p->pool, rp->nplane, bn);
+        s.ref_has_n = any_n;
+        J.ref2 = rp->plane2; J.refn = any_n ? rp->nplane : nullptr;
+        const size_t region = ref2_bytes(p->pp.max_pos) + refn_bytes(p->pp.max_pos);
+        if (!s.d_words) HIP_TRY(isx_dev_malloc(reinterpret_cast<void **>(&s.d_words), region + 64));
+        if (!s.marks) s.marks.reset(new isxenc::RefMarks);
+        s.marks->buf = s.h_in + s.off_ref;
+        s.marks->cap_chunks = (int64_t)(region / ISX_RMARK_BYTES(any_n));
+        J.marks = s.marks.get();
+        if (!ring) HIP_TRY(hipEventRecord(s.ev_h2d0, st));
+        HIP_TRY(hipEventRecord(s.ev_h2da, st));
+        out->early = true; out->words = true;
+        out->host_ms = now_ms() - t_r;
+        return ISX_OK;
+    }
+
     if (rp && !first_trip && isx_host_is_registered(rp->plane2, b2) && (!rp->nplane || isx_host_is_registered(rp->nplane, bn))) {
         const bool any_n = rp->nplane && plane_any(*p->pool, rp->nplane, bn);
         s.ref_has_n = any_n;
@@ -1141,6 +1189,7 @@
         if (any_n) HIP_TRY(hipMemcpyAsync(s.d_in + s.off_ref + ref2_bytes(n_pos), rp->nplane, bn, hipMemcpyHostToDevice, st));
         if (!ring) HIP_TRY(hipEventRecord(s.ev_h2da, st));
         out->early = true;
+        p->ref_stat[1]++; p->ref_stat[4] += (int64_t)(ref2_bytes(n_pos) + (any_n ? refn_bytes(n_pos) : 0));
         return ISX_OK;
     }
 
@@ -1148,6 +1197,7 @@
     s.ref_has_n = rp ? copy_ref_planes(*p->pool, rp, n_pos, h2, hn) : isxenc::pack_ref_planes(*p->pool, ref, n_pos, h2, hn);
     J.ref2 = h2; J.refn = s.ref_has_n ? hn : nullptr;
     out->host_ms = now_ms() - t_r;
+    p->ref_stat[1]++; p->ref_stat[4] += (int64_t)(ref2_bytes(n_pos) + (s.ref_has_n ? refn_bytes(n_pos) : 0));
     static const bool late_dma = getenv("ISX_PIPE_LATE_DMA") != nullptr;
     if (late_dma) return ISX_OK;
     if (!ring) HIP_TRY(hipEventRecord(s.ev_h2d0, st));
@@ -1155,6 +1205,34 @@
     if (!ring) HIP_TRY(hipEventRecord(s.ev_h2da, st));
     out->early = true;
     if (rp && rp->key) ref_cache_insert(p, s, rp, n_pos);
+    return ISX_OK;
+}
+
+static int send_reference_words(isx_pipe *p, Slot &s, int64_t n_pos, const isx_ref_planes *rp, size_t *sent)
+{
+    hipStream_t st = H2D(p, s);
+    const isxenc::RefMarks &M = *s.marks;
+    const size_t b2 = ((size_t)n_pos + 3) / 4, bn = ((size_t)n_pos + 7) / 8;
+    s.words_pending = false; s.words_bytes = 0;
+    if (!M.whole) {
+        s.words_bytes = (size_t)M.n_chunks * ISX_RMARK_BYTES(s.ref_has_n);
+        s.words_with_n = s.ref_has_n;
+        s.words_pending = true;
+        if (s.words_bytes) HIP_TRY(hipMemcpyAsync(s.d_words, s.h_in + s.off_ref, s.words_bytes, hipMemcpyHostToDevice, st));
+        *sent = s.words_bytes;
+        p->ref_stat[0]++; p->ref_stat[3] += M.entries; p->ref_stat[4] += (int64_t)s.words_bytes;
+        return ISX_OK;
+    }
+    *sent = ref2_bytes(n_pos) + (s.ref_has_n ? refn_bytes(n_pos) : 0);
+    if (isx_host_is_registered(rp->plane2, b2) && (!s.ref_has_n || isx_host_is_registered(rp->nplane, bn))) {
+        HIP_TRY(hipMemcpyAsync(s.d_in + s.off_ref, rp->plane2, b2, hipMemcpyHostToDevice, st));
+        if (s.ref_has_n) HIP_TRY(hipMemcpyAsync(s.d_in + s.off_ref + ref2_bytes(n_pos), rp->nplane, bn, hipMemcpyHostToDevice, st));
+    } else {
+        uint8_t *h2 = s.h_in + s.off_ref;
+        (void)copy_ref_planes(*p->pool, rp, n_pos, h2, h2 + ref2_bytes(n_pos));
+        HIP_TRY(hipMemcpyAsync(s.d_in + s.off_ref, h2, *sent, hipMemcpyHostToDevice, st));
+    }
+    p->ref_stat[1]++; p->ref_stat[2]++; p->ref_stat[4] += (int64_t)*sent;
     return ISX_OK;
 }
 
@@ -1321,6 +1399,8 @@
         }
         early_rec = true;
     }
+    size_t ref_sent = 0;
+    if (rs.words && (rc = send_reference_words(p, s, n_pos, rp, &ref_sent)) != ISX_OK) return rc;
     if (!planes_in) s.ref_has_n = isxenc::pack_ref_planes(*p->pool, ref, n_pos, s.h_in + s.off_ref, s.h_in + s.off_ref + ref2_bytes(n_pos));
     const double t_ref = now_ms();
     memcpy(s.h_in + s.off_bounds, split_bounds, (size_t)(n_splits + 1) * sizeof(int64_t));
@@ -1351,6 +1431,7 @@
     if (ring) { if (feed.bytes != rec_bytes) { isx_set_error("internal: the staging ring did not carry the whole stream"); return ISX_ERR_STATE; } }
     else if (!early_rec) HIP_TRY(hipMemcpyAsync(s.d_in + s.off_rec, s.h_in + s.off_rec, rec_bytes, hipMemcpyHostToDevice, H2D(p, s)));
     s.h2d_bytes = (int64_t)(head + gb_bytes + rec_bytes) - (rs.resident ? (int64_t)ref_bytes : 0);
+    if (rs.words) s.h2d_bytes += (int64_t)ref_sent - (int64_t)ref_bytes;
     if (linkage && !p->drec) {
         HIP_TRY(hipMemcpyAsync(s.d_in + s.off_pairs, s.h_in + s.off_pairs, (size_t)b->n_rec * sizeof(uint32_t), hipMemcpyHostToDevice, H2D(p, s)));
         s.h2d_bytes += (int64_t)b->n_rec * 4;
@@ -1596,6 +1677,14 @@
     return submit_segs_common(p, n_pos, nullptr, n_splits, split_bounds, J, ticket, ref);
 }
 
+int isx_pipe_reference_stats(isx_pipe *p, isx_ref_stats *out)
+{
+    if (!p || !out) { isx_set_error("isx_pipe_reference_stats: bad argument"); return ISX_ERR_ARG; }
+    out->batches_sparse = p->ref_stat[0].load(); out->batches_whole = p->ref_stat[1].load(); out->batches_fallback = p->ref_stat[2].load();
+    out->entries = p->ref_stat[3].load(); out->ref_bytes = p->ref_stat[4].load();
+    return ISX_OK;
+}
+
 int isx_pipe_set_reference_budget(isx_pipe *p, int64_t mib)
 {
     if (!p) { isx_set_error("isx_pipe_set_reference_budget: bad argument"); return ISX_ERR_ARG; }
diff --git a/instrain_amd/csrc/seg_encode.cpp b/instrain_amd/csrc/seg_encode.cpp
--- a/instrain_amd/csrc/seg_encode.cpp
+++ b/instrain_amd/csrc/seg_encode.cpp
@@ -573,6 +573,44 @@
         if ((o[0] & ISX_DREC_DUAL) && ((o[4] >> 16) & 0xFFu)) o[4] += up;
     }
     G.lo = new_lo;
+}
+
+constexpr int MARK_WORDS_PER_SEG = 6;
+__attribute__((noinline)) void marks_flush(RefMarks &M, const uint8_t *ref2, const uint8_t *refn, int64_t n_pos, const uint32_t *hw, uint32_t nh)
+{
+    if (!nh || M.overflow.load(std::memory_order_relaxed)) return;
+    const bool with_n = refn != nullptr;
+    const int64_t b2 = (n_pos + 3) / 4, bn = (n_pos + 7) / 8;
+    const uint32_t safe = (uint32_t)std::min<int64_t>(b2 / 8, with_n ? bn / 4 : b2 / 8);
+    uint8_t *c = nullptr;
+    uint32_t k = ISX_RMARK_CHUNK, last = ISX_RMARK_NONE;
+    for (uint32_t i = 0; i < nh; i++) {
+        const uint32_t wi = hw[i];
+        if (wi == last) continue;
+        last = wi;
+        if (k == ISX_RMARK_CHUNK) {
+            const int64_t ci = M.next.fetch_add(1, std::memory_order_relaxed);
+            if (ci >= M.cap_chunks) { M.overflow.store(true, std::memory_order_relaxed); return; }
+            c = M.buf + (size_t)ci * ISX_RMARK_BYTES(with_n);
+            k = 0;
+        }
+        uint64_t v2 = 0;
+        uint32_t vn = 0;
+        if (__builtin_expect(wi < safe, 1)) {
+            memcpy(&v2, ref2 + (size_t)wi * 8, 8);
+            if (with_n) memcpy(&vn, refn + (size_t)wi * 4, 4);
+        } else {
+            const int64_t o2 = (int64_t)wi * 8, on = (int64_t)wi * 4;
+            if (o2 < b2) memcpy(&v2, ref2 + o2, (size_t)std::min<int64_t>(8, b2 - o2));
+            if (with_n && on < bn) memcpy(&vn, refn + on, (size_t)std::min<int64_t>(4, bn - on));
+        }
+        memcpy(c + 4 * (size_t)k, &wi, 4);
+        memcpy(c + (size_t)ISX_RMARK_CHUNK * 4 + 8 * (size_t)k, &v2, 8);
+        if (with_n) memcpy(c + (size_t)ISX_RMARK_CHUNK * 12 + 4 * (size_t)k, &vn, 4);
+        k++;
+    }
+    M.unused.fetch_add(ISX_RMARK_CHUNK - k, std::memory_order_relaxed);
+    for (; k < ISX_RMARK_CHUNK; k++) reinterpret_cast<uint32_t *>(c)[k] = ISX_RMARK_NONE;
 }
 
 struct PlaneScratch {
@@ -656,6 +694,10 @@
     constexpr size_t group_words = (size_t)ISX_DREC_GROUP * ISX_DREC_WORDS;
     const bool fast_store = cpu_has_avx512() && (reinterpret_cast<uintptr_t>(J.rec) & 63) == 0;
     const int variant = planes_variant();
+    if (RefMarks *M = J.marks) {
+        M->next.store(0); M->unused.store(0); M->overflow.store(false);
+        M->n_chunks = 0; M->entries = 0; M->whole = J.n_mm_bins != 1;
+    }
     if (n == 0) {
         if (RG) J.wave_begin(0);
         for (int r = 0; r < ISX_DREC_GROUP; r++) put_empty_drec(J.rec + (size_t)r * ISX_DREC_WORDS);
@@ -723,6 +765,11 @@
     }
     J.need_slack = fits ? slack : std::max<int64_t>(worst, slack + 1);
     if (!fits) return SEG_CAPACITY;
+    if (RefMarks *M = J.marks) {
+        M->n_chunks = std::min(M->next.load(), M->cap_chunks);
+        M->entries = M->n_chunks * ISX_RMARK_CHUNK - M->unused.load();
+        M->whole = M->whole || M->overflow.load() || 2 * M->entries > (J.n_pos + 31) / 32;
+    }
     return SEG_OK;
 }
 
@@ -1054,8 +1101,8 @@
     return isx_encode_planes_mm(reads, ref, n_pos, 1, host_threads, slack_groups, cap_rec, ring_records, rec, gbase, n_rec, need_slack);
 }
 
-int isx_encode_planes_mm(const isx_read_planes *reads, const isx_ref_planes *ref, int64_t n_pos, int32_t n_mm_bins, int32_t host_threads, int32_t slack_groups,
-                         int64_t cap_rec, int64_t ring_records, uint32_t *rec, uint32_t *gbase, int64_t *n_rec, int64_t *need_slack)
+static int encode_planes_entry(const isx_read_planes *reads, const isx_ref_planes *ref, int64_t n_pos, int32_t n_mm_bins, int32_t host_threads, int32_t slack_groups,
+                               int64_t cap_rec, int64_t ring_records, uint32_t *rec, uint32_t *gbase, int64_t *n_rec, int64_t *need_slack, isxenc::RefMarks *marks)
 {
     if (n_mm_bins < 1 || n_mm_bins > 128) { isx_set_error("isx_encode_planes: n_mm_bins must be in [1, 128]"); return ISX_ERR_ARG; }
     if (!reads || !ref || !ref->plane2 || !rec || !gbase || !n_rec || reads->n_seg < 0 || cap_rec < ISX_DREC_GROUP || (cap_rec % ISX_DREC_GROUP) || n_pos <= 0 ||
@@ -1071,6 +1118,7 @@
     isxenc::SegJob J;
     J.in2 = *reads; J.n_seg = reads->n_seg; J.n_pos = n_pos; J.n_mm_bins = n_mm_bins;
     J.ref2 = ref->plane2; J.refn = ref->nplane; J.slack_groups = std::max(1, slack_groups);
+    J.marks = marks;
     J.rec = rec; J.gbase = gbase; J.pair_out = nullptr;
     J.cmin = cmin.data(); J.cmax = cmax.data(); J.cany = cany.data(); J.cap_rec = cap_rec;
     if (ring_records) {
@@ -1097,6 +1145,45 @@
     if (rc == isxenc::SEG_BAD_POS) { isx_set_error("a segment reaches beyond n_pos"); return ISX_ERR_ARG; }
     if (rc == isxenc::SEG_BAD_LEN) { isx_set_error("a segment's length is not in [1, 150]"); return ISX_ERR_ARG; }
     if (rc == isxenc::SEG_MM_RANGE) { isx_set_error("a segment has mm >= n_mm_bins"); return ISX_ERR_MM_RANGE; }
+    return ISX_OK;
+}
+
+int isx_encode_planes_mm(const isx_read_planes *reads, const isx_ref_planes *ref, int64_t n_pos, int32_t n_mm_bins, int32_t host_threads, int32_t slack_groups,
+                         int64_t cap_rec, int64_t ring_records, uint32_t *rec, uint32_t *gbase, int64_t *n_rec, int64_t *need_slack)
+{
+    return encode_planes_entry(reads, ref, n_pos, n_mm_bins, host_threads, slack_groups, cap_rec, ring_records, rec, gbase, n_rec, need_slack, nullptr);
+}
+
+int isx_encode_planes_marked(const isx_read_planes *reads, const isx_ref_planes *ref, int64_t n_pos, int32_t host_threads, int32_t slack_groups,
+                             int64_t cap_rec, int64_t ring_records, uint32_t *rec, uint32_t *gbase, int64_t *n_rec, int64_t *need_slack,
+                             int64_t cap_entries, uint32_t *word_idx, uint64_t *word2, uint32_t *wordn, int64_t *n_entries, int32_t *whole)
+{
+    if (cap_entries < 0 || !n_entries || !whole || (cap_entries && (!word_idx || !word2 || (ref && ref->nplane && !wordn)))) {
+        isx_set_error("isx_encode_planes_marked: bad argument");
+        return ISX_ERR_ARG;
+    }
+    const bool with_n = ref && ref->nplane;
+    isxenc::RefMarks M;
+    M.cap_chunks = cap_entries / ISX_RMARK_CHUNK;
+    std::vector<uint64_t> buf((size_t)M.cap_chunks * ISX_RMARK_BYTES(with_n) / 8 + 1);
+    M.buf = reinterpret_cast<uint8_t *>(buf.data());
+    const int rc = encode_planes_entry(reads, ref, n_pos, 1, host_threads, slack_groups, cap_rec, ring_records, rec, gbase, n_rec, need_slack, &M);
+    if (rc != ISX_OK) return rc;
+    int64_t n = 0;
+    for (int64_t c = 0; c < M.n_chunks; c++) {
+        const uint8_t *b = M.buf + (size_t)c * ISX_RMARK_BYTES(with_n);
+        for (int k = 0; k < ISX_RMARK_CHUNK; k++) {
+            uint32_t wi;
+            memcpy(&wi, b + 4 * k, 4);
+            if (wi == ISX_RMARK_NONE) continue;
+            word_idx[n] = wi;
+            memcpy(word2 + n, b + (size_t)ISX_RMARK_CHUNK * 4 + 8 * k, 8);
+            if (with_n) memcpy(wordn + n, b + (size_t)ISX_RMARK_CHUNK * 12 + 4 * k, 4);
+            n++;
+        }
+    }
+    *n_entries = n;
+    *whole = M.whole ? 1 : 0;
     return ISX_OK;
 }
 
diff --git a/instrain_amd/csrc/seg_encode.h b/instrain_amd/csrc/seg_encode.h
--- a/instrain_amd/csrc/seg_encode.h
+++ b/instrain_amd/csrc/seg_encode.h
@@ -1,6 +1,7 @@
 #pragma once
 #include <stdint.h>
 
+#include <atomic>
 #include <functional>
 #include <vector>
 
@@ -11,7 +12,22 @@
 #define ISX_SEG_REC_WORDS 16
 #define ISX_DREC_GROUP 32
 
+#define ISX_RMARK_CHUNK 64
+#define ISX_RMARK_BYTES(with_n) ((size_t)ISX_RMARK_CHUNK * ((with_n) ? 16 : 12))
+#define ISX_RMARK_NONE 0xFFFFFFFFu
+
 namespace isxenc {
+
+struct RefMarks {
+    uint8_t *buf = nullptr;
+    int64_t cap_chunks = 0;
+    std::atomic<int64_t> next{0};
+    std::atomic<int64_t> unused{0};
+    std::atomic<bool> overflow{false};
+    int64_t n_chunks = 0;
+    int64_t entries = 0;
+    bool whole = false;
+};
 
 struct SegJob {
     isx_segs in{};
@@ -20,6 +36,7 @@
     isx_read_planes in2{};
     std::function<void(int64_t first, int64_t count, uint32_t *gpos, uint8_t *len, uint8_t *mm, uint32_t *pair, uint64_t *planes)> produce_planes;
     const uint8_t *ref2 = nullptr, *refn = nullptr;
+    RefMarks *marks = nullptr;
     int64_t n_seg = 0, n_pos = 0;
     int n_mm_bins = 1;
     bool want_pairs = false;
diff --git a/instrain_amd/csrc/seg_planes.inc b/instrain_amd/csrc/seg_planes.inc
--- a/instrain_amd/csrc/seg_planes.inc
+++ b/instrain_amd/csrc/seg_planes.inc
@@ -90,6 +90,10 @@
         G.n++;
         return o;
     };
+    RefMarks *const MK = J.n_mm_bins == 1 ? J.marks : nullptr;
+    const bool m_on = MK && !MK->overflow.load(std::memory_order_relaxed);
+    uint32_t m_hw[m_on ? TASK * MARK_WORDS_PER_SEG + 1 : 1];
+    uint32_t m_nh = 0;
     uint32_t hdr_hi = 0;
     auto add_full = [&](uint32_t start, uint32_t len, uint32_t pid, uint64_t s0, uint64_t s1, uint64_t s2, uint32_t exc) __attribute__((always_inline)) {
         bool fill;
@@ -202,6 +206,7 @@
             const uint32_t col = t0 + (t1 & m0) + (t2 & m01);
             const uint32_t code = (uint32_t)(P[col >> 5] >> (2 * (col & 31u))) & 3u;
             const uint32_t w0 = 0x3FFFFC00u | ((col | (code << 8) | (0u - (uint32_t)(n_exc == 0))) & 0x3FFu);
+            if (m_on) { m_hw[m_nh] = (p + col) >> 5; m_nh += n_exc; }
             if (__builtin_expect(plain, 0)) { add_plain(p, L, pid, w0, ISX_DREC_NO_EXC); continue; }
 #if ISX_PLANES_VARIANT == 2
             if (__builtin_expect(in_regs, 1)) {
@@ -217,6 +222,12 @@
             add_full(p, L, pid, s0, s1, s2, w0);
             continue;
         }
+        if (m_on)
+            for (int k = 0; k < 3; k++)
+                for (uint64_t m = ex[k]; m; m &= m - 1) {
+                    const uint32_t wi = (p + (uint32_t)(64 * k + __builtin_ctzll(m))) >> 5;
+                    if (!m_nh || m_hw[m_nh - 1] != wi) m_hw[m_nh++] = wi;
+                }
         const uint32_t max_exc = plain ? ISX_DREC_EXC : ISX_DREC_EXC_FULL;
         if (__builtin_expect(n_exc <= max_exc, 1)) {
             uint64_t fields = 0;
@@ -267,6 +278,7 @@
         for (int r = 0; r < ISX_DREC_GROUP; r++) put_empty_drec(o + (size_t)r * ISX_DREC_WORDS);
         J.gbase[G.g] = 0; J.cmin[G.g] = 0xFFFFFFFFu; J.cmax[G.g] = 0; J.cany[G.g] = 0;
     }
+    if (m_on) marks_flush(*MK, ref2, refn, n_pos, m_hw, m_nh);
     if (K.fast_store) _mm_sfence();
     K.used = G.used; K.np = np; K.nb = nb; K.maxp = maxp;
 }
diff --git a/instrain_amd/engine.py b/instrain_amd/engine.py
--- a/instrain_amd/engine.py
+++ b/instrain_amd/engine.py
@@ -473,6 +473,11 @@
 
     def set_reference_budget(self, mib):
         check(self.lib.isx_pipe_set_reference_budget(self.h, int(mib)))
+
+    def reference_stats(self):
+        st = _lib.RefStats()
+        check(self.lib.isx_pipe_reference_stats(self.h, C.byref(st)))
+        return {k: int(getattr(st, k)) for k, _ in _lib.RefStats._fields_}
 
     def stage_planes(self, ref_planes, split_bounds, reads):
         split_bounds = np.ascontiguousarray(split_bounds, dtype=np.int64)
@@ -783,6 +788,31 @@
         return rec[:n], gbase[:n // 32], None, slack_groups
 
 
+def encode_planes_marked(reads, ref_planes, threads=1, slack_groups=1, cap_entries=None):
+    lib = _lib.load()
+    n_words = (ref_planes.n_pos + 31) // 32
+    if cap_entries is None:
+        cap_entries = n_words + 64 * (reads.n_seg // 4096 + 2)
+    while True:
+        cap = int(lib.isx_delta_records_needed(reads.gpos.ctypes.data if reads.n_seg else None, reads.n_seg, int(threads), int(slack_groups)))
+        rec = _aligned((cap, 8), np.uint32)
+        gbase = np.empty(cap // 32, dtype=np.uint32)
+        idx = np.empty(max(cap_entries, 1), dtype=np.uint32)
+        w2 = np.empty(max(cap_entries, 1), dtype=np.uint64)
+        wn = np.empty(max(cap_entries, 1), dtype=np.uint32) if ref_planes.nplane is not None else None
+        n_rec, need, n_ent, whole = C.c_int64(0), C.c_int64(0), C.c_int64(0), C.c_int32(0)
+        cr, cf = reads.c(), ref_planes.c()
+        rc = lib.isx_encode_planes_marked(C.byref(cr), C.byref(cf), ref_planes.n_pos, int(threads), int(slack_groups), cap, 0,
+                                          rec.ctypes.data, gbase.ctypes.data, C.byref(n_rec), C.byref(need),
+                                          int(cap_entries), idx.ctypes.data, w2.ctypes.data, None if wn is None else wn.ctypes.data, C.byref(n_ent), C.byref(whole))
+        if rc == _lib.ERR_CAPACITY and need.value > slack_groups:
+            slack_groups = int(need.value)
+            continue
+        check(rc)
+        n, k = n_rec.value, n_ent.value
+        return rec[:n], gbase[:n // 32], idx[:k], w2[:k], None if wn is None else wn[:k], bool(whole.value)
+
+
 def dense_cov(res, n_pos=None):
     if "cov16" in res:
         return res["cov16"]
```
